# lschoenm/MerKurio

Measured on AMD Instinct MI355X. Metric: Gbases/s scanned (150bp FASTQ, 10k 31-mers); % HBM roofline at 1/2/4/8 GPUs, higher is better.
Workload: dtype u8

## Files before the change

include/merkurio_hip.h:

```cpp
#ifndef MERKURIO_HIP_H
#define MERKURIO_HIP_H

#include <stddef.h>
#include <stdint.h>

#ifdef __cplusplus
extern "C" {
#endif

#define MK_ABI_VERSION 7

#define MK_OK 0
#define MK_E_EMPTY_PATTERN (-1)
#define MK_E_INVALID_Q (-2)
#define MK_E_PATTERN_TOO_LONG (-3)
#define MK_E_NO_PATTERNS (-4)
#define MK_E_NOMEM (-5)
#define MK_E_PAIR_MISMATCH (-6)
#define MK_E_HIP (-7)
#define MK_E_CAPACITY (-8)
#define MK_E_INVALID_ARG (-9)
#define MK_E_UNSUPPORTED (-10)
#define MK_E_RCCL (-11)
#define MK_E_CORRUPT (-12)

#define MK_ALGO_AUTO 0
#define MK_ALGO_AC 1
#define MK_ALGO_BNDMQ 2

#define MK_FLAG_ASCII_CASE_INSENSITIVE 1u

#define MK_MODE_ANY 0
#define MK_MODE_HITS 1

typedef struct mk_matcher mk_matcher;

typedef struct {
    uint64_t rec;
    uint32_t pat;
    uint32_t pos;
} mk_hit;

typedef struct {
    uint64_t rec;
    uint32_t pat;
    uint32_t pos;
    uint32_t file;
    uint32_t _pad;
} mk_row;

typedef struct {
    uint64_t nb_records_tot;
    uint64_t nb_bases;
    uint64_t nb_hits_tot[2];
    uint64_t nb_records_hit[2];
    uint64_t nb_records_extracted;
} mk_counters;

int mk_abi_version(void);
const char *mk_last_error(void);
int mk_device_count(void);

int mk_read_kmers_from_text(const uint8_t *content, size_t len, uint8_t **out_bytes, uint32_t **out_off,
                            uint32_t *out_n);
int mk_parse_pattern_list(const uint8_t *in_bytes, const uint32_t *in_off, uint32_t n_in, int reverse_complement,
                          int canonical, int lowercase, int uppercase, uint8_t **out_bytes, uint32_t **out_off,
                          uint32_t *out_n);
void mk_reverse_complement(const uint8_t *in, size_t n, uint8_t *out);
void mk_canonical(const uint8_t *in, size_t n, uint8_t *out);
int mk_recommend_aho_corasick(size_t num_patterns, size_t max_len);
size_t mk_tune_q_value(size_t pattern_len);
int mk_generate_masks(const uint8_t *pattern, size_t m, uint64_t masks[256], uint64_t *accept);
void mk_free(void *p);

int mk_matcher_create(const uint8_t *pat_bytes, const uint32_t *pat_off, uint32_t n_pat, uint32_t algo, uint32_t q,
                      uint32_t flags, int32_t device, mk_matcher **out);
typedef struct {
    uint32_t struct_size;
    uint32_t force_stride;
    uint32_t force_global_filter;
    uint32_t gbloom_log2_blocks;
    uint32_t tile_run;
    uint32_t gbloom_kib;
    uint32_t length_classes;
    uint32_t force_split_len;
    uint32_t force_stride2;
    uint32_t force_q2;
} mk_matcher_options;
int mk_matcher_create_ex(const uint8_t *pat_bytes, const uint32_t *pat_off, uint32_t n_pat, uint32_t algo, uint32_t q,
                         uint32_t flags, int32_t device, const mk_matcher_options *options, mk_matcher **out);
int mk_plan_geometry(const uint32_t *pat_len, uint32_t n_pat, const mk_matcher_options *options, uint32_t *q_gram, uint32_t *stride,
                     uint32_t *in_lds, uint32_t *split_len, uint32_t *n_short, uint32_t *q_gram2, uint32_t *stride2);
void mk_matcher_destroy(mk_matcher *m);
uint32_t mk_matcher_algo(const mk_matcher *m);
uint32_t mk_matcher_num_patterns(const mk_matcher *m);
int mk_matcher_filter_info(const mk_matcher *m, uint32_t *q_gram, uint32_t *stride, uint64_t *entries,
                           uint64_t *table_bytes);
int mk_matcher_class_info(const mk_matcher *m, uint32_t *split_len, uint32_t *n_short, uint32_t *q_gram2, uint32_t *stride2);
int mk_matcher_filter_mode(const mk_matcher *m, uint32_t *in_lds, uint64_t *filter_bytes);

int mk_scan_batch(mk_matcher *m, const uint8_t *seq_bytes, const uint64_t *seq_off, uint64_t n_rec, uint32_t mode,
                  uint8_t *rec_flags, mk_hit *hits, uint64_t hits_cap, uint64_t *n_hits);

#define MK_NUM_SUMMARY 8
#define MK_SUM_HITS 0
#define MK_SUM_RECORDS_HIT 1
#define MK_SUM_RECORDS 2
#define MK_SUM_BASES 3
#define MK_SUM_CANDIDATES 4

int mk_scan_device(mk_matcher *m, const void *d_seq, uint64_t n_bytes, const void *d_seq_off, uint64_t n_rec,
                   uint32_t mode, void *d_rec_flags, void *d_hits, uint64_t hits_cap, void *d_n_hits,
                   void *d_counters, void *stream);

int mk_matcher_check_device(mk_matcher *m, void *stream);

int mk_matcher_hint_hit_density(mk_matcher *m, uint32_t records_hit_per_1000);

int mk_matcher_set_fixed_record_length(mk_matcher *m, uint32_t record_length);

int mk_matcher_hint_record_lengths(mk_matcher *m, int equal_lengths);

int mk_order_hits(const mk_matcher *m, mk_hit *hits, uint64_t n_hits);
int mk_order_hits_device(mk_matcher *m, void *d_hits, uint64_t n_hits, void *stream);
int mk_matcher_order_info(const mk_matcher *m, uint32_t *path, uint32_t *n_bins, uint32_t *max_bin);
int mk_matcher_order_stats(const mk_matcher *m, uint64_t calls[4]);

const char *mk_matcher_kernel_name(const mk_matcher *m);
int mk_matcher_launch_info(const mk_matcher *m, uint32_t *grid_blocks, uint32_t *block_threads, uint32_t *lds_bytes);
int mk_matcher_enable_timing(mk_matcher *m, uint32_t slots);
int mk_matcher_kernel_times(mk_matcher *m, float *ms, uint32_t cap, uint32_t *n_out);

int mk_extract_single(mk_matcher *m, const uint8_t *seq, const uint64_t *off, uint64_t n_rec, int logging,
                      int invert, uint8_t *keep, mk_row *rows, uint64_t rows_cap, uint64_t *n_rows,
                      mk_counters *counters, uint32_t *pattern_hit_counts);
int mk_extract_paired(mk_matcher *m, const uint8_t *seq1, const uint64_t *off1, uint64_t n_rec1,
                      const uint8_t *seq2, const uint64_t *off2, uint64_t n_rec2, int logging, int invert,
                      uint8_t *keep, mk_row *rows, uint64_t rows_cap, uint64_t *n_rows, mk_counters *counters,
                      uint32_t *pattern_hit_counts);
int mk_tag_records(mk_matcher *m, const uint8_t *seq, const uint64_t *off, uint64_t n_rec, int logging,
                   int filter_matching, int invert, uint8_t *keep, mk_row *rows, uint64_t rows_cap, uint64_t *n_rows,
                   mk_counters *counters, uint32_t *pattern_hit_counts, uint64_t *found_off, uint32_t *found_pat,
                   uint64_t found_cap);
int mk_extract_fastq_text(mk_matcher *m, const uint8_t *text, uint64_t n_text, int logging, int invert, uint64_t rec_cap,
                          uint64_t *n_rec, uint64_t *rec_start, uint8_t *keep, mk_row *rows, uint64_t rows_cap, uint64_t *n_rows,
                          mk_counters *counters, uint32_t *pattern_hit_counts, uint32_t *status);
int mk_upload_text_ahead(mk_matcher *m, const uint8_t *text, uint64_t n_text);
int mk_host_alloc(size_t bytes, void **out);
void mk_host_free(void *p);
int mk_matcher_batch_times(const mk_matcher *m, float ms[4]);

int mk_tag_value(const mk_matcher *m, const uint32_t *found_pat, uint64_t n_found, const char *existing, char *out,
                 size_t cap, size_t *out_len);

int mk_synth_reads_device(mk_matcher *m, uint64_t seed, uint64_t n_rec, uint32_t read_len, uint32_t plant_every,
                          void *d_seq, void *d_seq_off, void *stream);
int mk_synth_reads_host(const mk_matcher *m, uint64_t seed, uint64_t rec0, uint64_t n_rec, uint32_t read_len,
                        uint32_t plant_every, uint8_t *seq, uint64_t *seq_off);
int mk_synth_reads_device_range(mk_matcher *m, uint64_t seed, uint64_t rec0, uint64_t n_rec, uint32_t read_len,
                                uint32_t plant_every, void *d_seq, void *d_seq_off, void *stream);

#define MK_COMM_ID_BYTES 128
int mk_reduce_counters(mk_matcher *const *per_gpu, int n, void *const *d_counters, size_t len, uint64_t *host_sum);
int mk_reduce_prepare(mk_matcher *const *per_gpu, int n);
int mk_comm_available(void);
int mk_comm_unique_id(uint8_t id[MK_COMM_ID_BYTES]);
int mk_comm_init(mk_matcher *m, const uint8_t id[MK_COMM_ID_BYTES], int rank, int n_ranks);
int mk_comm_reduce_counters(mk_matcher *m, void *d_counters, size_t len, void *stream);
int mk_comm_size(const mk_matcher *m, int *n_ranks);
int mk_comm_destroy(mk_matcher *m);

typedef struct mk_codec mk_codec;
typedef struct mk_bgzf_member {
    uint64_t data_off;
    uint64_t out_off;
    uint32_t data_len;
    uint32_t isize;
    uint32_t crc;
    uint32_t reserved;
} mk_bgzf_member;
int mk_codec_create(int device, mk_codec **out);
void mk_codec_destroy(mk_codec *c);
uint64_t mk_bgzf_deflate_bound(uint64_t n, uint32_t block_bytes);
int mk_bgzf_deflate(mk_codec *c, const uint8_t *in, uint64_t n, uint32_t block_bytes, uint8_t *out, uint64_t out_cap, uint64_t *out_len);
int mk_bgzf_deflate_pieces(mk_codec *c, const uint8_t *const *pieces, const uint64_t *sizes, uint64_t n_pieces, uint32_t block_bytes,
                           uint8_t *out, uint64_t out_cap, uint64_t *out_len);
int mk_bgzf_inflate(mk_codec *c, const uint8_t *in, uint64_t n_in, const mk_bgzf_member *members, uint64_t n_members, uint8_t *out,
                    uint64_t out_cap, uint64_t *bad_member);
typedef struct mk_window_text {
    uint8_t *text;
    uint64_t text_cap;
    uint8_t *tail;
    uint64_t tail_cap;
    uint8_t *kept;
    uint64_t kept_cap;
    uint64_t n_text, n_used, n_tail, n_kept_bytes;
} mk_window_text;
int mk_extract_fastq_bgzf(mk_matcher *m, mk_codec *codec, const uint8_t *head, uint64_t n_head, const uint8_t *bgzf, uint64_t n_bgzf,
                          const mk_bgzf_member *members, uint64_t n_members, int last, mk_window_text *io, int logging, int invert,
                          uint64_t rec_cap, uint64_t *n_rec, uint64_t *rec_start, uint8_t *keep, mk_row *rows, uint64_t rows_cap,
                          uint64_t *n_rows, mk_counters *c, uint32_t *pattern_hit_counts, uint32_t *status);
#define MK_TEXT_FASTQ 0
#define MK_TEXT_FASTA 1
typedef struct mk_window_source {
    const uint8_t *head;
    uint64_t n_head;
    const uint8_t *text;
    uint64_t n_text;
    const uint8_t *bgzf;
    uint64_t n_bgzf;
    const mk_bgzf_member *members;
    uint64_t n_members;
    const void *device_text;
    uint64_t n_device_text;
    uint32_t ends_at_record;
    uint32_t reserved;
    uint64_t *rec_start;
    uint8_t *tail;
    uint64_t tail_cap;
    uint8_t *kept;
    uint64_t kept_cap;
    uint8_t *all;
    uint64_t all_cap;
    uint64_t n_window, n_used, n_tail, n_kept_bytes, n_rec_seen;
} mk_window_source;
int mk_extract_window(mk_matcher *m, mk_codec *codec, uint32_t format, uint32_t n_sources, mk_window_source *sources, int logging, int invert,
                      uint64_t rec_cap, uint64_t *n_rec, uint8_t *keep, mk_row *rows, uint64_t rows_cap, uint64_t *n_rows, mk_counters *counters,
                      uint32_t *pattern_hit_counts, uint32_t *status);

int mk_gzip_inflate_device(mk_codec *c, const uint8_t *gz, uint64_t n, uint64_t *text_bytes, uint32_t *taken);
int mk_gzip_text_read(mk_codec *c, uint64_t offset, uint8_t *out, uint64_t len);
const void *mk_gzip_text_device(const mk_codec *c, uint64_t *text_bytes);
int mk_gzip_text_release(mk_codec *c);
int mk_gzip_info(const mk_codec *c, uint32_t *segments, float ms[5]);

typedef struct mk_bam_window {
    const uint8_t *head;
    uint64_t n_head;
    const uint8_t *bgzf;
    uint64_t n_bgzf;
    const mk_bgzf_member *members;
    uint64_t n_members;
    uint32_t last;
    uint32_t filter_matching, invert;
    uint8_t tag[2];
    uint8_t reserved[2];
    uint32_t block_bytes;
    uint8_t *tail;
    uint64_t tail_cap;
    uint8_t *out;
    uint64_t out_cap;
    mk_row *rows;
    uint64_t rows_cap;
    uint64_t *row_name;
    uint8_t *names;
    uint64_t names_cap;
    void (*on_tail)(void *ctx, const uint8_t *tail, uint64_t n_tail);
    void *on_tail_ctx;
    uint64_t n_window, n_used, n_tail, n_rec, n_kept, out_text_bytes, out_len, n_rows, n_names_bytes;
    float ms[8];
} mk_bam_window;
int mk_tag_bam_window(mk_matcher *m, mk_codec *codec, mk_bam_window *w, int logging, mk_counters *counters, uint32_t *pattern_hit_counts,
                      uint32_t *status);
int mk_matcher_set_bam_piece(mk_matcher *m, uint32_t piece_bytes);

typedef struct mk_sam_window {
    const uint8_t *head;
    uint64_t n_head;
    const uint8_t *text;
    uint64_t n_text;
    uint32_t last;
    uint32_t filter_matching, invert;
    uint8_t tag[2];
    uint8_t reserved[2];
    uint8_t *tail;
    uint64_t tail_cap;
    uint8_t *out;
    uint64_t out_cap;
    mk_row *rows;
    uint64_t rows_cap;
    uint64_t *row_name;
    uint8_t *names;
    uint64_t names_cap;
    uint64_t n_window, n_used, n_tail, n_rec, n_kept, out_len, n_rows, n_names_bytes;
    float ms[8];
} mk_sam_window;
int mk_tag_sam_window(mk_matcher *m, mk_sam_window *w, int logging, mk_counters *counters, uint32_t *pattern_hit_counts, uint32_t *status);

typedef struct mk_sam_bam_window {
    const uint8_t *head;
    uint64_t n_head;
    const uint8_t *text;
    uint64_t n_text;
    uint32_t last;
    uint32_t filter_matching, invert;
    uint8_t tag[2];
    uint8_t reserved[2];
    const uint8_t *ref_names;
    const uint64_t *ref_off;
    uint64_t n_refs;
    uint32_t block_bytes;
    uint32_t reserved2;
    uint8_t *tail;
    uint64_t tail_cap;
    uint8_t *out;
    uint64_t out_cap;
    mk_row *rows;
    uint64_t rows_cap;
    uint64_t *row_name;
    uint8_t *names;
    uint64_t names_cap;
    uint64_t n_window, n_used, n_tail, n_rec, n_kept, out_text_bytes, out_len, n_rows, n_names_bytes;
    float ms[8];
} mk_sam_bam_window;
int mk_tag_sam_bam_window(mk_matcher *m, mk_codec *codec, mk_sam_bam_window *w, int logging, mk_counters *counters, uint32_t *pattern_hit_counts,
                          uint32_t *status);

typedef struct mk_bam_sam_window {
    const uint8_t *head;
    uint64_t n_head;
    const uint8_t *bgzf;
    uint64_t n_bgzf;
    const mk_bgzf_member *members;
    uint64_t n_members;
    uint32_t last;
    uint32_t filter_matching, invert;
    uint8_t tag[2];
    uint8_t reserved[2];
    const uint8_t *ref_names;
    const uint64_t *ref_off;
    uint64_t n_refs;
    uint8_t *tail;
    uint64_t tail_cap;
    uint8_t *out;
    uint64_t out_cap;
    mk_row *rows;
    uint64_t rows_cap;
    uint64_t *row_name;
    uint8_t *names;
    uint64_t names_cap;
    void (*on_tail)(void *ctx, const uint8_t *tail, uint64_t n_tail);
    void *on_tail_ctx;
    uint64_t n_window, n_used, n_tail, n_rec, n_kept, out_len, n_rows, n_names_bytes;
    float ms[8];
} mk_bam_sam_window;
int mk_tag_bam_sam_window(mk_matcher *m, mk_codec *codec, mk_bam_sam_window *w, int logging, mk_counters *counters, uint32_t *pattern_hit_counts,
                          uint32_t *status);

int mk_bgzf_members(const uint8_t *in, uint64_t n, mk_bgzf_member *members, uint64_t cap, uint64_t *n_members, uint64_t *consumed,
                    uint64_t *text_bytes);
const uint8_t *mk_bgzf_eof(void);
int mk_codec_set_pass_limits(mk_codec *c, uint64_t deflate_members, uint64_t inflate_text_bytes);
int mk_codec_set_inflate_kernel(mk_codec *c, int which);
int mk_codec_set_gzip_chunk(mk_codec *c, uint64_t chunk_bytes);
int mk_codec_times(const mk_codec *c, float ms[3]);

#ifdef __cplusplus
}
#endif
#endif
```

merkurio_amd/build.py:

```python
import os
import subprocess
import sys
from concurrent.futures import ThreadPoolExecutor

HERE = os.path.dirname(os.path.abspath(__file__))
CSRC = os.path.join(HERE, "csrc")
LIB_DIR = os.path.join(HERE, "lib")
LIB_PATH = os.path.join(LIB_DIR, "libmerkurio_hip.so")
CLI_PATH = os.path.join(LIB_DIR, "merkurio")

N_VARIANT_TUS = 17
HOST_SOURCES = ["matcher.cpp", "host_patterns.cpp", "host_loops.cpp", "reduce.cpp"]
HIPCC = os.environ.get("HIPCC", "/opt/rocm/bin/hipcc")
FLAGS = ["--offload-arch=gfx950", "-O3", "-std=c++17", "-fPIC", "-Wall", "-Wno-unused-result"]
FLAGS += os.environ.get("MERKURIO_HIPCC_FLAGS", "").split()
JOBS = int(os.environ.get("MERKURIO_BUILD_JOBS", str(min(8, os.cpu_count() or 1))))


def _stale(target, deps):
    if not os.path.exists(target):
        return True
    t = os.path.getmtime(target)
    return any(os.path.getmtime(d) > t for d in deps)


def _headers():
    hs = [os.path.join(CSRC, f) for f in os.listdir(CSRC) if f.endswith((".h", ".hpp"))]
    hs += [os.path.join(CSRC, "codec", f) for f in os.listdir(os.path.join(CSRC, "codec")) if f.endswith((".h", ".hpp"))]
    hs.append(os.path.join(os.path.dirname(HERE), "include", "merkurio_hip.h"))
    return hs


def _units():
    units = [("scan_tu%d.o" % n, "scan_variants.hip", ["-DMK_TU=%d" % n]) for n in range(N_VARIANT_TUS)]
    units.append(("scan_kernel.o", "scan_kernel.hip", []))
    units.append(("order_hits.o", "order_hits.hip", []))
    units.append(("order_hits_fallback.o", "order_hits_fallback.hip", []))
    units.append(("sets.o", "sets.hip", []))
    units.append(("build_tables.o", "build_tables.hip", []))
    units.append(("ingest.o", "ingest.hip", []))
    units.append(("bam.o", "bam.hip", []))
    units.append(("sam.o", "sam.hip", []))
    units.append(("codec_bgzf_deflate.o", "codec/bgzf_deflate.hip", []))
    units.append(("codec_bgzf_inflate.o", "codec/bgzf_inflate.hip", []))
    units.append(("codec_bgzf_inflate_wave.o", "codec/bgzf_inflate_wave.hip", []))
    units.append(("codec_gzip_inflate.o", "codec/gzip_inflate.hip", []))
    units.append(("codec_gzip_segments_wave.o", "codec/gzip_segments_wave.hip", []))
    units.append(("codec_host.o", "codec/codec_host.cpp", []))
    units += [(s.replace(".cpp", ".o"), s, []) for s in HOST_SOURCES if os.path.exists(os.path.join(CSRC, s))]
    return units


def _deps():
    srcs = [os.path.join(CSRC, f) for f in os.listdir(CSRC) if os.path.isfile(os.path.join(CSRC, f))]
    srcs += [os.path.join(CSRC, "codec", f) for f in os.listdir(os.path.join(CSRC, "codec"))]
    return srcs + _headers()


def _parse_resource_remarks(stderr):
    import re
    rows, cur, rest = [], None, []
    for line in stderr.splitlines():
        if "[-Rpass-analysis=kernel-resource-usage]" not in line:
            rest.append(line)
            continue
        m = re.search(r"remark:\s+(.*?)\s*\[-Rpass", line)
        if not m:
            continue
        k, _, v = m.group(1).partition(":")
        k, v = k.strip(), v.strip()
        if k == "Function Name":
            cur = {"name": v}
            rows.append(cur)
        elif cur is not None:
            cur[k] = v
    out = []
    for r in rows:
        name = r["name"]
        for tool in ("c++filt", "/opt/rocm/lib/llvm/bin/llvm-cxxfilt"):
            try:
                name = subprocess.run([tool, name], capture_output=True, text=True).stdout.strip() or name
                break
            except OSError:
                continue
        out.append((name, r.get("VGPRs", "?"), r.get("AGPRs", "?"), r.get("TotalSGPRs", r.get("SGPRs", "?")),
                    r.get("ScratchSize [bytes/lane]", "?"), r.get("LDS Size [bytes/block]", "?"), r.get("Occupancy [waves/SIMD]", "?")))
    return out, "\n".join(rest) + ("\n" if rest else "")


def isa_resources(obj_dir, out_file, strict=True):
    rows = []
    for f in sorted(os.listdir(obj_dir)):
        if f.endswith(".isa.txt"):
            with open(os.path.join(obj_dir, f)) as fh:
                rows += [line.rstrip("\n").split("\t") for line in fh if line.strip()]
    if not rows:
        return None
    rows.sort(key=lambda r: r[0])
    with open(out_file, "w") as f:
        f.write("# kernel\tVGPRs\tAGPRs\tSGPRs\tscratch bytes/lane\tLDS bytes/block (static)\twaves/SIMD\n")
        for r in rows:
            f.write("\t".join(r) + "\n")
    spilled = [r[0] for r in rows if r[4] not in ("0", "?") and "rocprim" not in r[0]]
    if spilled and strict:
        raise RuntimeError("kernels with scratch memory (register spills): " + "; ".join(spilled))
    if spilled:
        print("note: kernels with scratch memory in this tagged build: " + "; ".join(spilled), file=sys.stderr)
    return out_file


def _compile_lib(out_path, extra_flags, obj_dir, force, verbose):
    os.makedirs(obj_dir, exist_ok=True)
    headers = _headers()
    jobs = []
    objs = []
    for obj, src, fl in _units():
        o = os.path.join(obj_dir, obj)
        s = os.path.join(CSRC, src)
        objs.append(o)
        if force or _stale(o, [s] + headers):
            jobs.append([HIPCC, *FLAGS, *extra_flags, *fl, "-c", "-o", o, s])

    def run(cmd):
        if verbose:
            print(" ".join(cmd), flush=True)
        if cmd[-1].endswith(".hip") and "-c" in cmd:
            r = subprocess.run(cmd + ["-Rpass-analysis=kernel-resource-usage"], stderr=subprocess.PIPE, text=True)
            obj = cmd[cmd.index("-o") + 1]
            rows, rest = _parse_resource_remarks(r.stderr)
            if rest.strip():
                sys.stderr.write(rest)
            if r.returncode:
                raise subprocess.CalledProcessError(r.returncode, cmd)
            with open(obj + ".isa.txt", "w") as f:
                for row in rows:
                    f.write("\t".join(str(x) for x in row) + "\n")
            return
        subprocess.run(cmd, check=True)

    if jobs:
        with ThreadPoolExecutor(max(1, JOBS)) as ex:
            list(ex.map(run, jobs))
    for f in os.listdir(obj_dir):
        if (f.endswith(".o") or f.endswith(".isa.txt")) and os.path.join(obj_dir, f.replace(".isa.txt", "")) not in objs:
            os.remove(os.path.join(obj_dir, f))
    isa_resources(obj_dir, os.path.join(os.path.dirname(out_path), "isa_resources" + os.path.basename(out_path)[len("libmerkurio_hip"):-3] + ".txt"),
                  strict=not extra_flags)
    if jobs or force or _stale(out_path, objs):
        tmp = out_path + ".tmp.%d" % os.getpid()
        run([HIPCC, "--offload-arch=gfx950", "-shared", "-o", tmp, *objs, "-ldl", "-lpthread"])
        os.replace(tmp, out_path)
    return out_path


def build_lib(force=False, verbose=False):
    import fcntl
    os.makedirs(LIB_DIR, exist_ok=True)
    if not force and not _stale(LIB_PATH, _deps()):
        return LIB_PATH
    with open(os.path.join(LIB_DIR, ".build.lock"), "w") as lock:
        fcntl.flock(lock, fcntl.LOCK_EX)
        if force or _stale(LIB_PATH, _deps()):
            _compile_lib(LIB_PATH, [], os.path.join(LIB_DIR, "obj"), force, verbose)
    return LIB_PATH


def build_tagged(tag, flags, force=False, verbose=False, only_scan=True):
    out = os.path.join(LIB_DIR, "libmerkurio_hip_%s.so" % tag)
    return _compile_lib(out, list(flags), os.path.join(LIB_DIR, "obj_" + tag), force, verbose)


def build_cli(force=False, verbose=False):
    srcs = [os.path.join(CSRC, "cli", f) for f in sorted(os.listdir(os.path.join(CSRC, "cli")))
            if f.endswith(".cpp")] if os.path.isdir(os.path.join(CSRC, "cli")) else []
    if not srcs:
        return None
    deps = srcs + [os.path.join(CSRC, "cli", f) for f in os.listdir(os.path.join(CSRC, "cli"))] + [LIB_PATH]
    if not force and not _stale(CLI_PATH, deps):
        return CLI_PATH
    obj_dir = os.path.join(LIB_DIR, "obj_cli")
    os.makedirs(obj_dir, exist_ok=True)
    cli_hdrs = [os.path.join(CSRC, "cli", f) for f in os.listdir(os.path.join(CSRC, "cli")) if f.endswith(".hpp")] + _headers()
    jobs, objs = [], []
    for s in srcs:
        o = os.path.join(obj_dir, os.path.basename(s).replace(".cpp", ".o"))
        objs.append(o)
        if force or _stale(o, [s] + cli_hdrs):
            jobs.append([HIPCC, "--offload-arch=gfx950", "-O2", "-std=c++17", "-Wall", "-Wno-unused-result", "-c", "-o", o, s])

    def run(cmd):
        if verbose:
            print(" ".join(cmd), flush=True)
        subprocess.run(cmd, check=True)

    with ThreadPoolExecutor(max(1, JOBS)) as ex:
        list(ex.map(run, jobs))
    run([HIPCC, "-o", CLI_PATH, *objs, "-L" + LIB_DIR, "-lmerkurio_hip", "-lz", "-ldl", "-lpthread", "-Wl,-rpath,$ORIGIN"])
    return CLI_PATH


def build_all(force=False, verbose=False):
    lib = build_lib(force, verbose)
    cli = build_cli(force, verbose)
    return lib, cli


if __name__ == "__main__":
    if "--tag" in sys.argv:
        tag = sys.argv[sys.argv.index("--tag") + 1]
        fl = sys.argv[sys.argv.index("--flags") + 1].split() if "--flags" in sys.argv else []
        print(build_tagged(tag, fl, force="--force" in sys.argv, verbose=True))
    else:
        print(build_all(force="--force" in sys.argv, verbose=True))
```

merkurio_amd/csrc/matcher.cpp:

```cpp
#include <hip/hip_runtime.h>

#include <algorithm>
#include <chrono>
#include <cmath>
#include <cstdarg>
#include <cstdio>
#include <cstdlib>
#include <cstring>
#include <memory>
#include <string>
#include <vector>

#include "host_common.h"
#include "matcher_internal.h"
#include "scan_kernel.h"

namespace mk {

thread_local char g_last_error[512] = "";

int fail(int code, const char *fmt, ...) {
    va_list ap;
    va_start(ap, fmt);
    vsnprintf(g_last_error, sizeof(g_last_error), fmt, ap);
    va_end(ap);
    return code;
}

int hip_fail(hipError_t e, const char *what) {
    (void)hipGetLastError();
    return fail(e == hipErrorOutOfMemory ? MK_E_NOMEM : MK_E_HIP, "%s failed: %s", what, hipGetErrorString(e));
}

#define MK_HIP(call)                                       \
    do {                                                   \
        hipError_t e_ = (call);                            \
        if (e_ != hipSuccess) return hip_fail(e_, #call);  \
    } while (0)

constexpr uint64_t kMaxLdsEntries = 98304;
constexpr double kMCandPerLaunch = 15000.0;
static double bloom_fp(double entries) {
    const double lo = 1.0 - exp(-entries / (kBloomBlocks * 32.0)), hi = 1.0 - exp(-2.0 * entries / (kBloomBlocks * 32.0));
    return lo * hi * hi;
}
static double hashed_cost(uint64_t n, uint32_t S, uint32_t q, double per_mcand) {
    const double per_base = std::min(1.0 / S, (double)n / pow(4.0, (double)std::min(q, 30u))) + bloom_fp((double)n * S) / S;
    return 0.42 * (16.0 / S) + kMCandPerLaunch * per_mcand * per_base;
}
static void choose_geometry(uint32_t lmin, uint64_t n_pat, const mk_matcher_options &opt, uint32_t *q, uint32_t *S,
                            uint32_t *gblocks) {
    const int forced = (int)opt.force_stride;
    const bool force_global = opt.force_global_filter != 0;
    *gblocks = 0;
    if (n_pat <= kMaxLdsEntries && !force_global) {
        *q = std::min<uint32_t>(32, lmin);
        *S = 1;
        double best = 1e300;
        for (uint32_t s : {16u, 8u, 4u, 2u, 1u}) {
            if (s > lmin) continue;
            const uint32_t qq = std::min<uint32_t>(32, lmin - s + 1);
            if (forced) {
                if ((int)s != forced) continue;
                *q = qq;
                *S = s;
                return;
            }
            if (s > 1 && n_pat * s > kMaxLdsEntries) continue;
            if (s > 1 && qq < 16 && (double)n_pat * s > 2.0 * pow(4.0, (double)qq)) continue;
            const double c = hashed_cost(n_pat, s, qq, 0.0152);
            if (c < best) {
                best = c;
                *q = qq;
                *S = s;
            }
        }
        return;
    }
    *q = std::min<uint32_t>(32, lmin);
    *S = 1;
    bool chosen = false;
    for (uint32_t s : {16u, 8u, 4u, 2u}) {
        if (s > lmin) continue;
        const uint32_t qq = std::min<uint32_t>(32, lmin - s + 1);
        if (forced ? (int)s != forced : (qq < 14 || n_pat * s > (8ull << 19))) continue;
        *q = qq;
        *S = s;
        chosen = true;
        break;
    }
    if (!chosen && !forced)
        for (uint32_t s : {16u, 8u, 4u, 2u}) {
            if (s > lmin) continue;
            const uint32_t qq = std::min<uint32_t>(32, lmin - s + 1);
            if (qq < 16 || n_pat * s * 4 > (1ull << 25)) continue;
            *q = qq;
            *S = s;
            break;
        }
    uint64_t blocks = std::min<uint64_t>(std::max<uint64_t>(n_pat * *S / 8, 1ull << 17), 3ull << 17);
    if (opt.gbloom_log2_blocks) blocks = 1ull << opt.gbloom_log2_blocks;
    if (opt.gbloom_kib) blocks = (uint64_t)opt.gbloom_kib * 128;
    *gblocks = (uint32_t)blocks;
}

struct ClassPlan {
    uint32_t split = 0;
    uint32_t S2 = 0, q2 = 0;
    uint32_t lmin_main = 0;
    uint64_t n_main = 0, n_short = 0;
    double cost = 0;
};
static double main_cost(uint32_t lmin, uint64_t n, const mk_matcher_options &opt, bool two_class) {
    uint32_t q, S, gb;
    choose_geometry(lmin, n, opt, &q, &S, &gb);
    return hashed_cost(n, S, q, two_class ? 0.025 : 0.0152);
}
static double short_cost(uint32_t S2, uint32_t q2, uint64_t n) {
    const double per_sample = std::min(1.0, (double)n * S2 / pow(4.0, (double)q2));
    return (q2 <= kShortByteMaxQ ? 0.075 : 0.15) * (16.0 / S2) + kMCandPerLaunch * 0.025 * per_sample / S2;
}
static ClassPlan plan_classes(std::vector<uint32_t> lens, const mk_matcher_options &opt) {
    ClassPlan best;
    const uint64_t n = lens.size();
    const auto mm = std::minmax_element(lens.begin(), lens.end());
    best.n_main = n;
    best.lmin_main = *mm.first;
    if (opt.length_classes == 1 || *mm.first == *mm.second) return best;
    if (opt.force_global_filter || n > kMaxLdsEntries) {
        constexpr uint32_t kGfMinLen = 15;
        if (*mm.first >= kGfMinLen || *mm.second < kGfMinLen || (opt.force_stride && opt.length_classes != 2 && !opt.force_split_len)) return best;
        uint32_t split = 0xFFFFFFFFu;
        uint64_t n_short = 0;
        for (uint32_t l : lens) {
            if (l < kGfMinLen)
                ++n_short;
            else
                split = std::min(split, l);
        }
        if (opt.force_split_len) {
            split = opt.force_split_len;
            n_short = 0;
            for (uint32_t l : lens) n_short += l < split;
            if (n_short == 0 || n_short == n) return best;
        }
        uint32_t q, S, gb;
        choose_geometry(split, n - n_short, opt, &q, &S, &gb);
        if (S < 2) return best;
        for (uint32_t s2 : {8u, 4u, 2u, 1u}) {
            if (s2 > *mm.first || (opt.force_stride2 && s2 != opt.force_stride2)) continue;
            const uint32_t qmax = std::min<uint32_t>(kShortMaxQ, *mm.first - s2 + 1);
            for (uint32_t q2 : {qmax, std::min(qmax, kShortByteMaxQ)}) {
                if (opt.force_q2 && q2 != std::min<uint32_t>(opt.force_q2, qmax)) continue;
                const double c = short_cost(s2, q2, n_short);
                if (best.split == 0 || c < best.cost) {
                    best.split = split;
                    best.S2 = s2;
                    best.q2 = q2;
                    best.lmin_main = split;
                    best.n_main = n - n_short;
                    best.n_short = n_short;
                    best.cost = c;
                }
            }
        }
        return best;
    }
    std::sort(lens.begin(), lens.end());
    if (opt.force_stride && opt.length_classes != 2 && !opt.force_split_len) return best;
    best.cost = main_cost(lens[0], n, opt, false);
    const double single = best.cost;
    for (uint64_t i = 1; i < n; ++i) {
        if (lens[i] == lens[i - 1]) continue;
        const uint32_t split = lens[i];
        if (opt.force_split_len && split != opt.force_split_len) continue;
        if (lens[0] > 64 && !opt.force_split_len) break;
        {
            uint32_t q, S, gb;
            choose_geometry(split, n - i, opt, &q, &S, &gb);
            if (S < 2) continue;
        }
        const double mc = main_cost(split, n - i, opt, true);
        for (uint32_t s2 : {8u, 4u, 2u, 1u}) {
            if (s2 > lens[0] || (opt.force_stride2 && s2 != opt.force_stride2)) continue;
            const uint32_t qmax = std::min<uint32_t>(kShortMaxQ, lens[0] - s2 + 1);
            for (uint32_t q2 : {qmax, std::min(qmax, kShortByteMaxQ)}) {
                if (opt.force_q2 && q2 != std::min<uint32_t>(opt.force_q2, qmax)) continue;
                if (!opt.force_stride2 && !opt.force_q2 && s2 > 1 && (double)i * s2 > 2.0 * pow(4.0, (double)q2)) continue;
                const double c = mc + short_cost(s2, q2, i);
                const bool forced = opt.length_classes == 2 || opt.force_split_len;
                if ((best.split == 0 && (forced || c < 0.9 * single)) || (best.split != 0 && c < best.cost)) {
                    best.split = split;
                    best.S2 = s2;
                    best.q2 = q2;
                    best.lmin_main = split;
                    best.n_main = n - i;
                    best.n_short = i;
                    best.cost = c;
                }
            }
        }
    }
    return best;
}

}

using namespace mk;

thread_local double mk::g_free_ms = 0;
thread_local double mk::g_alloc_ms = 0;

int mk::ensure_device(void **p, size_t *cap, size_t need) {
    if (need <= *cap) return MK_OK;
    const auto t0 = std::chrono::steady_clock::now();
    auto ms_since = [](std::chrono::steady_clock::time_point a) { return std::chrono::duration<double, std::milli>(std::chrono::steady_clock::now() - a).count(); };
    double free_ms = 0;
    if (*p) {
        (void)hipFree(*p);
        free_ms = ms_since(t0);
        g_free_ms += free_ms;
    }
    *p = nullptr;
    *cap = 0;
    size_t want = need + (need < (64u << 20) ? need / 4 : need / 16) + 4096;
    hipError_t e = hipMalloc(p, want);
    g_alloc_ms += ms_since(t0);
#ifdef MK_ALLOC_LOG
    fprintf(stderr, "[alloc] %8.1f MiB: hipFree %7.2f ms, hipMalloc %7.2f ms\n", want / 1048576.0, free_ms, ms_since(t0) - free_ms);
#endif
    if (e != hipSuccess) return hip_fail(e, "hipMalloc");
    *cap = want;
    return MK_OK;
}

static int ensure(void **p, size_t *cap, size_t need) { return ensure_device(p, cap, need); }

static int read_options(const mk_matcher_options *options, mk_matcher_options *out) {
    mk_matcher_options opt;
    memset(&opt, 0, sizeof(opt));
    if (options) {
        if (options->struct_size < sizeof(uint32_t) || options->struct_size > 4096)
            return fail(MK_E_INVALID_ARG, "mk_matcher_options.struct_size %u is not plausible", options->struct_size);
        memcpy(&opt, options, std::min<size_t>(options->struct_size, sizeof(opt)));
        const uint32_t fs = opt.force_stride;
        if (fs != 0 && fs != 1 && fs != 2 && fs != 4 && fs != 8 && fs != 16)
            return fail(MK_E_INVALID_ARG, "force_stride %u: must be 0, 1, 2, 4, 8 or 16", fs);
        if (opt.gbloom_log2_blocks != 0 && (opt.gbloom_log2_blocks < 10 || opt.gbloom_log2_blocks > 25))
            return fail(MK_E_INVALID_ARG, "gbloom_log2_blocks %u out of range (10..25)", opt.gbloom_log2_blocks);
        if (opt.tile_run > 8) return fail(MK_E_INVALID_ARG, "tile_run %u out of range (0..8)", opt.tile_run);
        if (opt.gbloom_kib > (1u << 18)) return fail(MK_E_INVALID_ARG, "gbloom_kib %u out of range (<= 256 MiB)", opt.gbloom_kib);
        if (opt.length_classes > 2) return fail(MK_E_INVALID_ARG, "length_classes %u: must be 0 (rule), 1 or 2", opt.length_classes);
        const uint32_t f2 = opt.force_stride2;
        if (f2 != 0 && f2 != 1 && f2 != 2 && f2 != 4 && f2 != 8)
            return fail(MK_E_INVALID_ARG, "force_stride2 %u: must be 0, 1, 2, 4 or 8", f2);
        if (opt.force_q2 > kShortMaxQ) return fail(MK_E_INVALID_ARG, "force_q2 %u: must be 0..%u", opt.force_q2, kShortMaxQ);
    }
    *out = opt;
    return MK_OK;
}

extern "C" {

int mk_abi_version(void) { return MK_ABI_VERSION; }
const char *mk_last_error(void) { return g_last_error; }

int mk_device_count(void) {
    int n = 0;
    if (hipGetDeviceCount(&n) != hipSuccess) return 0;
    return n;
}

void mk_free(void *p) { free(p); }

int mk_plan_geometry(const uint32_t *pat_len, uint32_t n_pat, const mk_matcher_options *options, uint32_t *q_gram, uint32_t *stride,
                     uint32_t *in_lds, uint32_t *split_len, uint32_t *n_short, uint32_t *q_gram2, uint32_t *stride2) {
    if (!pat_len || n_pat == 0) return fail(MK_E_NO_PATTERNS, "No k-mers found in file or provided sequence.");
    mk_matcher_options opt;
    int rc = read_options(options, &opt);
    if (rc) return rc;
    MK_ABI_BEGIN
    std::vector<uint32_t> lens(pat_len, pat_len + n_pat);
    if (*std::min_element(lens.begin(), lens.end()) == 0) return fail(MK_E_EMPTY_PATTERN, "Pattern is empty.");
    const ClassPlan plan = plan_classes(std::move(lens), opt);
    uint32_t q = 0, S = 1, gb = 0;
    choose_geometry(plan.lmin_main, plan.n_main, opt, &q, &S, &gb);
    if (q_gram) *q_gram = q;
    if (stride) *stride = S;
    if (in_lds) *in_lds = gb ? 0 : 1;
    if (split_len) *split_len = plan.split;
    if (n_short) *n_short = (uint32_t)plan.n_short;
    if (q_gram2) *q_gram2 = plan.q2;
    if (stride2) *stride2 = plan.S2;
    return MK_OK;
    MK_ABI_END
}

int mk_matcher_create(const uint8_t *pat_bytes, const uint32_t *pat_off, uint32_t n_pat, uint32_t algo, uint32_t q,
                      uint32_t flags, int32_t device, mk_matcher **out) {
    return mk_matcher_create_ex(pat_bytes, pat_off, n_pat, algo, q, flags, device, nullptr, out);
}

int mk_matcher_create_ex(const uint8_t *pat_bytes, const uint32_t *pat_off, uint32_t n_pat, uint32_t algo, uint32_t q,
                         uint32_t flags, int32_t device, const mk_matcher_options *options, mk_matcher **out) {
    if (!out) return fail(MK_E_INVALID_ARG, "out is null");
    *out = nullptr;
    mk_matcher_options opt;
    int rc_opt = read_options(options, &opt);
    if (rc_opt) return rc_opt;
    MK_ABI_BEGIN
    if (n_pat == 0 || !pat_off || !pat_bytes) return fail(MK_E_NO_PATTERNS, "No k-mers found in file or provided sequence.");
    if (algo > MK_ALGO_BNDMQ) return fail(MK_E_INVALID_ARG, "unknown algo %u", algo);
    if (n_pat > kMaxPatterns) return fail(MK_E_UNSUPPORTED, "too many patterns (%u)", n_pat);
    const bool ci = flags & MK_FLAG_ASCII_CASE_INSENSITIVE;
    uint32_t lmin = 0xFFFFFFFFu, lmax = 0;
    for (uint32_t i = 0; i < n_pat; ++i) {
        if (pat_off[i + 1] < pat_off[i]) return fail(MK_E_INVALID_ARG, "pattern offsets not monotone");
        uint32_t len = pat_off[i + 1] - pat_off[i];
        lmin = std::min(lmin, len);
        lmax = std::max(lmax, len);
    }
    uint32_t use = algo;
    if (ci)
        use = MK_ALGO_AC;
    else if (algo == MK_ALGO_AUTO)
        use = (q == 0 && mk_recommend_aho_corasick(n_pat, lmax)) ? MK_ALGO_AC : MK_ALGO_BNDMQ;
    if (use == MK_ALGO_BNDMQ) {
        for (uint32_t i = 0; i < n_pat; ++i) {
            size_t len = pat_off[i + 1] - pat_off[i];
            size_t qq = q ? q : mk_tune_q_value(len);
            if (!q && len >= 65) return fail(MK_E_PATTERN_TOO_LONG, "Pattern length is too long for BNDMq.");
            if (len == 0) return fail(MK_E_EMPTY_PATTERN, "Pattern is empty.");
            if (qq == 0 || qq > len)
                return fail(MK_E_INVALID_Q, "Invalid q-gram length: %zu. Must be between 1 and pattern length.", qq);
            if (len > 64)
                return fail(MK_E_PATTERN_TOO_LONG,
                            "Pattern length %zu is too large for this architecture when using BNDM (max 64).", len);
        }
    } else if (lmin == 0) {
        return fail(MK_E_EMPTY_PATTERN, "Pattern is empty.");
    }

    int ndev = 0;
    if (hipGetDeviceCount(&ndev) != hipSuccess || ndev <= 0)
        return fail(MK_E_HIP, "no HIP device available: the MI355X scan path has no CPU fallback");
    if (device < 0 || device >= ndev) return fail(MK_E_INVALID_ARG, "device %d out of range (%d devices)", device, ndev);
    MK_HIP(hipSetDevice(device));

    struct Deleter {
        void operator()(mk_matcher *p) const { mk_matcher_destroy(p); }
    };
    std::unique_ptr<mk_matcher, Deleter> owner(new mk_matcher());
    mk_matcher *m = owner.get();
    m->device = device;
    m->algo = use;
    m->flags = flags;
    m->n_pat = n_pat;
    m->pat_bytes.assign(pat_bytes, pat_bytes + pat_off[n_pat]);
    m->pat_off.assign(pat_off, pat_off + n_pat + 1);
    hipDeviceProp_t prop;
    if (hipGetDeviceProperties(&prop, device) == hipSuccess && prop.multiProcessorCount > 0)
        m->num_cus = prop.multiProcessorCount;

    m->uniform_len = (lmin == lmax) ? lmin : 0;
    m->tile_run = opt.tile_run;
    ClassPlan plan;
    {
        std::vector<uint32_t> lens(n_pat);
        for (uint32_t i = 0; i < n_pat; ++i) lens[i] = pat_off[i + 1] - pat_off[i];
        plan = plan_classes(std::move(lens), opt);
    }
    if ((opt.length_classes == 2 || opt.force_split_len) && !plan.split)
        return fail(MK_E_INVALID_ARG, "the pattern set cannot be split into two length classes as the options ask "
                                      "(split length %u, stride %u, shortest pattern %u, longest %u)",
                    opt.force_split_len, opt.force_stride2, lmin, lmax);
    m->split_len = plan.split;
    m->S2 = plan.S2;
    m->q2 = plan.q2;
    m->n_short = (uint32_t)plan.n_short;
    choose_geometry(plan.lmin_main, plan.n_main, opt, &m->q, &m->S, &m->gbloom_blocks);
    if (opt.force_stride && m->S != opt.force_stride)
        return fail(MK_E_INVALID_ARG, "force_stride %u is longer than the shortest pattern (%u)", opt.force_stride, plan.lmin_main);
    const uint32_t q_f = m->q, S = m->S;
    m->entries = plan.n_main * S + plan.n_short * plan.S2;
    uint64_t slots = 64;
    while (slots < (m->gbloom_blocks ? 4 : 2) * m->entries) slots <<= 1;
    if (slots > (1ull << 27) && m->gbloom_blocks) {
        slots = 64;
        while (slots < 2 * m->entries) slots <<= 1;
    }
    if (slots > (1ull << 27))
        return fail(MK_E_UNSUPPORTED, "pattern set too large (%llu table entries)", (unsigned long long)m->entries);
    m->table_slots = (uint32_t)slots;
    const bool two = plan.split != 0;
    const bool gf_ctx = m->gbloom_blocks != 0 && gf_has_ctx(S, q_f) && !two;
    const size_t bloom_words = m->gbloom_blocks ? (size_t)m->gbloom_blocks * 2 : (size_t)kBloomWords;
    MK_HIP(hipStreamCreateWithFlags(&m->stream, hipStreamNonBlocking));
    MK_HIP(hipMalloc((void **)&m->d_bloom, bloom_words * sizeof(uint32_t)));
    MK_HIP(hipMalloc((void **)&m->d_table, slots * sizeof(TableEntry)));
    MK_HIP(hipMalloc((void **)&m->d_pat_bytes, m->pat_bytes.size() + 16));
    MK_HIP(hipMalloc((void **)&m->d_pat_off, (n_pat + 1) * sizeof(uint32_t)));
    MK_HIP(hipMalloc((void **)&m->d_nhits, sizeof(unsigned long long)));
    MK_HIP(hipMalloc((void **)&m->d_error, 16));
    MK_HIP(hipMemset(m->d_error, 0, 16));
    MK_HIP(hipMalloc((void **)&m->d_stage, (size_t)m->num_cus * (kBlockThreads / 64) * kHitStage * sizeof(mk_hit)));
    MK_HIP(hipMalloc((void **)&m->d_flag_list, (size_t)m->num_cus * (kBlockThreads / 64) * kFlagListCap * sizeof(uint32_t)));
    MK_HIP(hipMalloc((void **)&m->d_flag_counts, (size_t)m->num_cus * (kBlockThreads / 64) * sizeof(uint32_t)));
    MK_HIP(hipMemcpy(m->d_pat_bytes, m->pat_bytes.data(), m->pat_bytes.size(), hipMemcpyHostToDevice));
    MK_HIP(hipMemsetAsync(m->d_pat_bytes + m->pat_bytes.size(), 0, 16, m->stream));
    MK_HIP(hipMemcpy(m->d_pat_off, m->pat_off.data(), (n_pat + 1) * sizeof(uint32_t), hipMemcpyHostToDevice));
    MK_HIP(hipMemsetAsync(m->d_bloom, 0, bloom_words * sizeof(uint32_t), m->stream));
    if (two) {
        MK_HIP(hipMalloc((void **)&m->d_short_table, kShortBitmapWords * sizeof(uint32_t)));
        MK_HIP(hipMemsetAsync(m->d_short_table, 0, kShortBitmapWords * sizeof(uint32_t), m->stream));
    }
    {
        BuildParams B;
        memset(&B, 0, sizeof(B));
        B.pat_bytes = m->d_pat_bytes;
        B.pat_off = m->d_pat_off;
        B.n_pat = n_pat;
        B.S = S;
        B.q = q_f;
        B.split = plan.split;
        B.S2 = plan.S2;
        B.q2 = plan.q2;
        B.gbloom_blocks = m->gbloom_blocks;
        B.gf_ctx = gf_ctx ? 1 : 0;
        B.bloom = m->d_bloom;
        B.table = m->d_table;
        B.bucket_mask = m->table_slots / kBucketEntries - 1;
        B.short_table = m->d_short_table;
        launch_build_tables(B, slots, m->stream);
        MK_HIP(hipGetLastError());
        MK_HIP(hipStreamSynchronize(m->stream));
    }
    if (use == MK_ALGO_AC && !m->uniform_len) {
        std::vector<uint32_t> unrank(n_pat), rank(n_pat);
        if (lmax <= (1u << 20)) {
            std::vector<uint32_t> start((size_t)lmax + 2, 0);
            for (uint32_t i = 0; i < n_pat; ++i) start[lmax - (pat_off[i + 1] - pat_off[i]) + 1]++;
            for (uint32_t l = 0; l <= lmax; ++l) start[l + 1] += start[l];
            for (uint32_t i = 0; i < n_pat; ++i) unrank[start[lmax - (pat_off[i + 1] - pat_off[i])]++] = i;
        } else {
            for (uint32_t i = 0; i < n_pat; ++i) unrank[i] = i;
            std::stable_sort(unrank.begin(), unrank.end(), [pat_off](uint32_t a, uint32_t b) {
                return pat_off[a + 1] - pat_off[a] > pat_off[b + 1] - pat_off[b];
            });
        }
        for (uint32_t r = 0; r < n_pat; ++r) rank[unrank[r]] = r;
        MK_HIP(hipMalloc((void **)&m->d_pat_rank, n_pat * sizeof(uint32_t)));
        MK_HIP(hipMalloc((void **)&m->d_pat_unrank, n_pat * sizeof(uint32_t)));
        MK_HIP(hipMemcpy(m->d_pat_rank, rank.data(), n_pat * sizeof(uint32_t), hipMemcpyHostToDevice));
        MK_HIP(hipMemcpy(m->d_pat_unrank, unrank.data(), n_pat * sizeof(uint32_t), hipMemcpyHostToDevice));
    }
    *out = owner.release();
    return MK_OK;
    MK_ABI_END
}

void mk_matcher_destroy(mk_matcher *m) {
    if (!m) return;
    (void)hipSetDevice(m->device);
    if (m->comm) (void)mk_comm_destroy(m);
    if (m->stream) (void)hipStreamDestroy(m->stream);
    if (m->stream_ahead) {
        (void)hipStreamSynchronize(m->stream_ahead);
        (void)hipStreamDestroy(m->stream_ahead);
        for (auto &a : m->ahead)
            if (a.ev) (void)hipEventDestroy(a.ev);
    }
    for (auto e : m->ev_start) (void)hipEventDestroy(e);
    for (auto e : m->ev_stop) (void)hipEventDestroy(e);
    for (void *p : {(void *)m->d_bloom, (void *)m->d_table, (void *)m->d_pat_bytes, (void *)m->d_pat_off,
                    (void *)m->d_seq, (void *)m->d_off, (void *)m->d_flags, (void *)m->d_hits, (void *)m->d_nhits,
                    (void *)m->d_stage, (void *)m->d_rec_index, (void *)m->d_flag_list, (void *)m->d_flag_counts, m->d_sort_tmp,
                    (void *)m->d_pat_rank, (void *)m->d_pat_unrank, (void *)m->d_error, m->d_aux, m->d_pair, (void *)m->d_short_table, m->d_refs, m->txt[0].d_text, m->txt[0].d_ing_a, m->txt[0].d_ing_b, m->txt[1].d_text, m->txt[1].d_ing_a, m->txt[1].d_ing_b, m->txt[0].d_fa_seq, m->txt[1].d_fa_seq, (void *)m->d_flags2, m->ahead[0].d, m->ahead[1].d, m->ahead[2].d, m->ahead[3].d})
        if (p) (void)hipFree(p);
    delete m;
}

uint32_t mk_matcher_algo(const mk_matcher *m) { return m ? m->algo : 0; }
uint32_t mk_matcher_num_patterns(const mk_matcher *m) { return m ? m->n_pat : 0; }
const char *mk_matcher_kernel_name(const mk_matcher *m) { return m ? m->kernel_name : ""; }

int mk_matcher_filter_info(const mk_matcher *m, uint32_t *q_gram, uint32_t *stride, uint64_t *entries,
                           uint64_t *table_bytes) {
    if (!m) return fail(MK_E_INVALID_ARG, "null matcher");
    if (q_gram) *q_gram = m->q;
    if (stride) *stride = m->S;
    if (entries) *entries = m->entries;
    if (table_bytes) *table_bytes = (uint64_t)m->table_slots * sizeof(TableEntry);
    return MK_OK;
}

int mk_matcher_class_info(const mk_matcher *m, uint32_t *split_len, uint32_t *n_short, uint32_t *q_gram2, uint32_t *stride2) {
    if (!m) return fail(MK_E_INVALID_ARG, "null matcher");
    if (split_len) *split_len = m->split_len;
    if (n_short) *n_short = m->n_short;
    if (q_gram2) *q_gram2 = m->q2;
    if (stride2) *stride2 = m->S2;
    return MK_OK;
}

int mk_matcher_filter_mode(const mk_matcher *m, uint32_t *in_lds, uint64_t *filter_bytes) {
    if (!m) return fail(MK_E_INVALID_ARG, "null matcher");
    if (in_lds) *in_lds = m->gbloom_blocks ? 0 : 1;
    if (filter_bytes) *filter_bytes = m->gbloom_blocks ? (uint64_t)m->gbloom_blocks * 8 : (uint64_t)kBloomBytes;
    return MK_OK;
}

int mk_scan_device(mk_matcher *m, const void *d_seq, uint64_t n_bytes, const void *d_seq_off, uint64_t n_rec,
                   uint32_t mode, void *d_rec_flags, void *d_hits, uint64_t hits_cap, void *d_n_hits,
                   void *d_counters, void *stream) {
    if (!m) return fail(MK_E_INVALID_ARG, "null matcher");
    if (mode > MK_MODE_HITS) return fail(MK_E_INVALID_ARG, "unknown mode %u", mode);
    if (((uintptr_t)d_seq & 15) != 0) return fail(MK_E_INVALID_ARG, "d_seq must be 16-byte aligned");
    if (((uintptr_t)d_rec_flags & 3) != 0) return fail(MK_E_INVALID_ARG, "d_rec_flags must be 4-byte aligned");
    const uint32_t rec_len = m->batch_rec_len ? m->batch_rec_len : m->fixed_rec_len;
    if (rec_len && n_bytes != n_rec * (uint64_t)rec_len)
        return fail(MK_E_INVALID_ARG, "fixed record length %u: %llu records are not %llu bytes", rec_len, (unsigned long long)n_rec,
                    (unsigned long long)n_bytes);
    if (!d_n_hits || !d_rec_flags || (!d_seq_off && n_rec && !rec_len)) return fail(MK_E_INVALID_ARG, "null device buffer");
    if (mode == MK_MODE_HITS && !d_hits && hits_cap) return fail(MK_E_INVALID_ARG, "d_hits is null");
    hipStream_t st = (hipStream_t)stream;
    MK_HIP(hipSetDevice(m->device));
    launch_clear((uint32_t *)d_rec_flags, (n_rec + 3) / 4, (unsigned long long *)d_n_hits, st);
    MK_HIP(hipGetLastError());
    if (mode == MK_MODE_HITS) MK_HIP(hipMemsetAsync(m->d_error, 0, sizeof(uint32_t), st));
    m->last_n_rec = n_rec;
    if (n_rec == 0 || n_bytes == 0) return MK_OK;
    ScanParams p;
    memset(&p, 0, sizeof(p));
    p.seq = (const uint8_t *)d_seq;
    p.n_bytes = n_bytes;
    p.rec_off = (const uint64_t *)d_seq_off;
    p.n_rec = n_rec;
    const uint64_t tile_bytes = (uint64_t)kTileChunks * kChunkBytes;
    const uint64_t n_tiles = (n_bytes + tile_bytes - 1) / tile_bytes;
    p.bloom = m->d_bloom;
    p.gbloom_blocks = m->gbloom_blocks;
    p.table = m->d_table;
    p.table_mask = m->table_slots / kBucketEntries - 1;
    p.pat_bytes = m->d_pat_bytes;
    p.pat_off = m->d_pat_off;
    p.n_pat = m->n_pat;
    p.q = m->q;
    const uint64_t kmask = m->q >= 32 ? ~0ull : ((1ull << (2 * m->q)) - 1);
    p.key_mask_lo = (uint32_t)kmask;
    p.key_mask_hi = (uint32_t)(kmask >> 32);
    p.case_insensitive = (m->flags & MK_FLAG_ASCII_CASE_INSENSITIVE) ? 1 : 0;
    p.s2 = m->split_len ? m->S2 : 0;
    p.s2_log2 = m->S2 >= 8 ? 3 : m->S2 >= 4 ? 2 : m->S2 >= 2 ? 1 : 0;
    p.key2_mask = (1u << (2 * m->q2)) - 1u;
    p.short_bytes = m->q2 <= kShortByteMaxQ;
    p.short_bitmap = m->d_short_table;
    p.uniform_len = m->uniform_len;
    p.rec_flags32 = (uint32_t *)d_rec_flags;
    p.hits = (mk_hit *)d_hits;
    p.hits_cap = (mode == MK_MODE_HITS) ? hits_cap : 0;
    p.n_hits = (unsigned long long *)d_n_hits;
    p.counters = (unsigned long long *)d_counters;
    p.error_word = m->d_error;
    const uint64_t waves_per_block = kBlockThreads / 64;
    uint64_t blocks = (n_tiles + waves_per_block - 1) / waves_per_block;
    if (blocks > (uint64_t)m->num_cus) blocks = m->num_cus;
    p.stage = m->d_stage;
    p.rec_per_byte = (double)n_rec / (double)n_bytes;
    const uint64_t tiles_per_wave = n_tiles / (blocks * waves_per_block);
    p.tile_run = m->tile_run ? m->tile_run : tiles_per_wave >= 16 ? 4 : tiles_per_wave >= 8 ? 2 : 1;
    p.rec_index = nullptr;
    p.rec_len = rec_len;
    p.inv_rec_len = rec_len ? 1.0 / (double)rec_len : 0.0;
    if (m->ragged && !rec_len && n_rec < (1ull << 32)) {
        int rc_i = ensure((void **)&m->d_rec_index, &m->d_rec_index_cap, ((n_bytes >> kRecIndexShift) + 2) * sizeof(uint32_t));
        if (rc_i) return rc_i;
        launch_rec_index(p.rec_off, n_rec, n_bytes, m->d_rec_index, st);
        p.rec_index = m->d_rec_index;
    }
    const size_t slots = m->ev_start.size();
    const size_t slot = slots ? (size_t)(m->timed_launches % slots) : 0;
    if (slots) MK_HIP(hipEventRecord(m->ev_start[slot], st));
    const uint32_t kDensePerMille = mode == MK_MODE_HITS ? 95 : 145;
    const bool plain_loads = m->hit_density_pm >= kDensePerMille && !m->split_len;
    const int flavour = plain_loads ? 0 : 1;
    const bool listed = !(plain_loads && m->gbloom_blocks == 0) && mode != MK_MODE_HITS && n_rec < (1ull << 32);
    p.flag_list = listed ? m->d_flag_list : nullptr;
    p.flag_counts = m->d_flag_counts;
    p.flag_cap = kFlagListCap;
    const char *name = launch_scan(p, (int)m->S, m->q > 16, mode == MK_MODE_HITS, m->gbloom_blocks != 0, flavour, (int)blocks, st);
    if (!name) return fail(MK_E_UNSUPPORTED, "no kernel for stride %u", m->S);
    if (slots) {
        MK_HIP(hipEventRecord(m->ev_stop[slot], st));
        m->timed_launches++;
    }
    if (listed)
        launch_flag_scatter(m->d_flag_list, m->d_flag_counts, kFlagListCap, (uint32_t)(blocks * waves_per_block), (uint8_t *)d_rec_flags, st);
    if (d_counters) {
        launch_count_flags(p, st);
        if (mode == MK_MODE_HITS && p.hits && p.hits_cap) launch_hist_hits(p, m->num_cus, st);
    }
    m->kernel_name = name;
    m->last_grid = (int)blocks;
    MK_HIP(hipGetLastError());
    return MK_OK;
}

static int take_device_errors(mk_matcher *m, hipStream_t st) {
    uint32_t w = 0;
    MK_HIP(hipMemcpyAsync(&w, m->d_error, sizeof(w), hipMemcpyDeviceToHost, st));
    MK_HIP(hipStreamSynchronize(st));
    if (!w) return MK_OK;
    MK_HIP(hipMemsetAsync(m->d_error, 0, sizeof(w), st));
    return fail(MK_E_UNSUPPORTED, "an occurrence lies 4 GiB or more into its record: a single record must be shorter than 4 GiB "
                                  "(mk_hit.pos is 32 bits); the tuples of that scan are not usable");
}

int mk_matcher_check_device(mk_matcher *m, void *stream) {
    if (!m) return fail(MK_E_INVALID_ARG, "null matcher");
    MK_HIP(hipSetDevice(m->device));
    return take_device_errors(m, (hipStream_t)stream);
}

int mk_matcher_hint_hit_density(mk_matcher *m, uint32_t records_hit_per_1000) {
    if (!m) return fail(MK_E_INVALID_ARG, "null matcher");
    m->hit_density_pm = records_hit_per_1000 > 1000 ? 1000 : records_hit_per_1000;
    return MK_OK;
}

int mk_matcher_set_fixed_record_length(mk_matcher *m, uint32_t record_length) {
    if (!m) return fail(MK_E_INVALID_ARG, "null matcher");
    m->fixed_rec_len = record_length;
    return MK_OK;
}

int mk_matcher_hint_record_lengths(mk_matcher *m, int equal_lengths) {
    if (!m) return fail(MK_E_INVALID_ARG, "null matcher");
    m->ragged = !equal_lengths;
    return MK_OK;
}

int mk_matcher_enable_timing(mk_matcher *m, uint32_t slots) {
    if (!m) return fail(MK_E_INVALID_ARG, "null matcher");
    MK_ABI_BEGIN
    MK_HIP(hipSetDevice(m->device));
    for (auto e : m->ev_start) (void)hipEventDestroy(e);
    for (auto e : m->ev_stop) (void)hipEventDestroy(e);
    m->ev_start.assign(slots, nullptr);
    m->ev_stop.assign(slots, nullptr);
    m->timed_launches = 0;
    for (uint32_t i = 0; i < slots; ++i) {
        MK_HIP(hipEventCreate(&m->ev_start[i]));
        MK_HIP(hipEventCreate(&m->ev_stop[i]));
    }
    return MK_OK;
    MK_ABI_END
}

int mk_matcher_kernel_times(mk_matcher *m, float *ms, uint32_t cap, uint32_t *n_out) {
    if (!m || !n_out) return fail(MK_E_INVALID_ARG, "null argument");
    const uint64_t slots = m->ev_start.size();
    const uint64_t n = std::min<uint64_t>(m->timed_launches, slots);
    *n_out = (uint32_t)n;
    if (n > cap) return fail(MK_E_CAPACITY, "need room for %llu timings", (unsigned long long)n);
    MK_HIP(hipSetDevice(m->device));
    const uint64_t first = m->timed_launches - n;
    for (uint64_t i = 0; i < n; ++i) {
        const size_t slot = (size_t)((first + i) % slots);
        MK_HIP(hipEventSynchronize(m->ev_stop[slot]));
        MK_HIP(hipEventElapsedTime(&ms[i], m->ev_start[slot], m->ev_stop[slot]));
    }
    m->timed_launches = 0;
    return MK_OK;
}

int mk_matcher_launch_info(const mk_matcher *m, uint32_t *grid_blocks, uint32_t *block_threads, uint32_t *lds_bytes) {
    if (!m) return fail(MK_E_INVALID_ARG, "null matcher");
    if (grid_blocks) *grid_blocks = (uint32_t)m->last_grid;
    if (block_threads) *block_threads = kBlockThreads;
    if (lds_bytes) *lds_bytes = scan_lds_bytes();
    return MK_OK;
}

static uint32_t bits_of(uint64_t v) { return v ? 64u - (uint32_t)__builtin_clzll(v) : 0u; }

static int order_library(mk_matcher *m, mk_hit *d_hits, uint64_t n, bool ac, hipStream_t st) {
    size_t need = 0;
    MK_HIP(order_hits_library(d_hits, n, ac, m->d_pat_off, m->uniform_len, nullptr, &need, st));
    int rc = ensure(&m->d_sort_tmp, &m->d_sort_tmp_cap, need ? need : 16);
    if (rc) return rc;
    MK_HIP(order_hits_library(d_hits, n, ac, m->d_pat_off, m->uniform_len, m->d_sort_tmp, &need, st));
    m->order_path = 3;
    return MK_OK;
}

int mk_order_hits_device(mk_matcher *m, void *d_hits, uint64_t n_hits, void *stream) {
    if (!m) return fail(MK_E_INVALID_ARG, "null matcher");
    return mk::order_hits_on_device(m, d_hits, n_hits, m->algo == MK_ALGO_AC, m->last_n_rec, stream);
}

}

static int order_hits_on_device_impl(mk_matcher *m, void *d_hits, uint64_t n_hits, bool ac_order, uint64_t rec_bound, void *stream);
int mk::order_hits_on_device(mk_matcher *m, void *d_hits, uint64_t n_hits, bool ac_order, uint64_t rec_bound, void *stream) {
    const int rc = order_hits_on_device_impl(m, d_hits, n_hits, ac_order, rec_bound, stream);
    if (rc == MK_OK) ++m->order_path_calls[m->order_path & 3];
    return rc;
}
static int order_hits_on_device_impl(mk_matcher *m, void *d_hits, uint64_t n_hits, bool ac_order, uint64_t rec_bound, void *stream) {
    using namespace mk;
    m->order_path = 0;
    if (n_hits < 2) return MK_OK;
    if (!d_hits) return fail(MK_E_INVALID_ARG, "null buffer");
    if (((uintptr_t)d_hits & 15) != 0) return fail(MK_E_INVALID_ARG, "d_hits must be 16-byte aligned");
    MK_ABI_BEGIN
    MK_HIP(hipSetDevice(m->device));
    hipStream_t st = (hipStream_t)stream;
    mk_hit *hits = (mk_hit *)d_hits;
    const uint64_t n = n_hits;
    if (n >= (1ull << 32)) return order_library(m, hits, n, ac_order, st);
    if (!m->order_prepared) {
        MK_HIP(order_kernels_prepare());
        m->order_prepared = true;
    }
    uint32_t log_bins = 0;
    while (log_bins < 15 && ((uint64_t)2048 << log_bins) < n) ++log_bins;
    const size_t head = 64 + (size_t)(4 * kOrderMaxBins + 16) * sizeof(uint32_t);
    int rc = ensure(&m->d_sort_tmp, &m->d_sort_tmp_cap, head + n * sizeof(uint64_t));
    if (rc) return rc;
    OrderScratch S;
    S.stats = (unsigned long long *)m->d_sort_tmp;
    S.g_cnt = (uint32_t *)((char *)m->d_sort_tmp + 64);
    S.bin_start = S.g_cnt + kOrderMaxBins;
    S.cursor = S.bin_start + kOrderMaxBins + 8;
    S.big_list = S.cursor + kOrderMaxBins;
    S.keys = (uint64_t *)((char *)m->d_sort_tmp + head);
    OrderKey L;
    memset(&L, 0, sizeof(L));
    L.pat_off = m->d_pat_off;
    L.uniform_len = m->uniform_len;
    L.rank = ac_order ? m->d_pat_rank : nullptr;
    L.unrank = ac_order ? m->d_pat_unrank : nullptr;
    L.ac = ac_order ? 1 : 0;
    if (!rec_bound) rec_bound = 1ull << 32;
    unsigned long long stats[6] = {0, 0, 0, 0, 0, 0};
    uint32_t s = 0;
    for (int attempt = 0; attempt < 2; ++attempt) {
        s = bits_of(rec_bound - 1) > log_bins ? bits_of(rec_bound - 1) - log_bins : 0;
        L.bits_a = 0;
        L.bits_b = 1;
        L.b_hi = 0;
        L.b_lo = 63;
        L.shift = s;
        L.n_bins = 1u << log_bins;
        MK_HIP(hipMemsetAsync(m->d_sort_tmp, 0, 64 + (size_t)L.n_bins * sizeof(uint32_t), st));
        launch_order_hist(hits, n, L, S, m->num_cus, st);
        MK_HIP(hipGetLastError());
        MK_HIP(hipMemcpyAsync(stats, S.stats, sizeof(stats), hipMemcpyDeviceToHost, st));
        uint32_t err_word = 0;
        MK_HIP(hipMemcpyAsync(&err_word, m->d_error, sizeof(err_word), hipMemcpyDeviceToHost, st));
        MK_HIP(hipStreamSynchronize(st));
        if (err_word) return take_device_errors(m, st);
        const bool beyond = (stats[0] >> s) >= L.n_bins;
        const bool loose = stats[3] > kOrderLeafMax && bits_of(stats[0]) < bits_of(rec_bound - 1);
        if (!beyond && !loose) break;
        rec_bound = stats[0] + 1;
    }
    uint32_t bits_rec = bits_of(stats[0]);
    const uint32_t bits_a = std::max(1u, bits_of(stats[1])), bits_b = std::max(1u, bits_of(stats[2]));
    if (bits_rec + bits_a + bits_b > 64) return order_library(m, hits, n, ac_order, st);
    if (s + bits_a > 63) return order_library(m, hits, n, ac_order, st);
    L.bits_a = bits_a;
    L.bits_b = bits_b;
    L.b_hi = 0;
    L.b_lo = bits_b;
    m->order_path = 1;
    if (stats[3] > kOrderLeafMax || (stats[0] >> s) >= L.n_bins) {
        L.rec_base = ~stats[4];
        bits_rec = bits_of(stats[0] - L.rec_base);
        const uint32_t total = bits_rec + bits_a + bits_b;
        const uint32_t lb = std::min(15u, std::max(log_bins + 3, total > 14 ? total - 14 : 0u));
        const uint32_t drop = total > lb ? total - lb : 0;
        if (drop >= bits_b) {
            L.b_hi = 0;
            L.b_lo = bits_b;
            L.shift = drop - bits_b;
        } else {
            L.b_hi = bits_b - drop;
            L.b_lo = drop;
            L.shift = 0;
        }
        L.n_bins = 1u << std::min(lb, total);
        MK_HIP(hipMemsetAsync(m->d_sort_tmp, 0, 64 + (size_t)L.n_bins * sizeof(uint32_t), st));
        launch_order_hist(hits, n, L, S, m->num_cus, st);
        MK_HIP(hipGetLastError());
        MK_HIP(hipMemcpyAsync(stats, S.stats, sizeof(stats), hipMemcpyDeviceToHost, st));
        MK_HIP(hipStreamSynchronize(st));
        if (stats[3] > kOrderLeafMax) return order_library(m, hits, n, ac_order, st);
        m->order_path = 2;
    } else {
        L.shift = s + bits_a;
    }
    m->order_bins = L.n_bins;
    m->order_max_bin = (uint32_t)stats[3];
    launch_order_scatter_leaf(hits, n, L, S, (uint32_t)stats[3], (uint32_t)stats[5], m->num_cus, st);
    MK_HIP(hipGetLastError());
    return MK_OK;
    MK_ABI_END
}

extern "C" {

int mk_matcher_order_stats(const mk_matcher *m, uint64_t calls[4]) {
    if (!m || !calls) return fail(MK_E_INVALID_ARG, "null argument");
    for (int i = 0; i < 4; ++i) calls[i] = m->order_path_calls[i];
    return MK_OK;
}

int mk_matcher_order_info(const mk_matcher *m, uint32_t *path, uint32_t *n_bins, uint32_t *max_bin) {
    if (!m) return fail(MK_E_INVALID_ARG, "null matcher");
    if (path) *path = m->order_path;
    if (n_bins) *n_bins = m->order_bins;
    if (max_bin) *max_bin = m->order_max_bin;
    return MK_OK;
}

int mk_order_hits(const mk_matcher *m, mk_hit *hits, uint64_t n_hits) {
    if (!m) return fail(MK_E_INVALID_ARG, "null matcher");
    if (m->algo == MK_ALGO_AC) {
        const uint32_t *off = m->pat_off.data();
        std::sort(hits, hits + n_hits, [off](const mk_hit &a, const mk_hit &b) {
            if (a.rec != b.rec) return a.rec < b.rec;
            uint64_t ea = (uint64_t)a.pos + (off[a.pat + 1] - off[a.pat]);
            uint64_t eb = (uint64_t)b.pos + (off[b.pat + 1] - off[b.pat]);
            if (ea != eb) return ea < eb;
            if (a.pos != b.pos) return a.pos < b.pos;
            return a.pat < b.pat;
        });
    } else {
        std::sort(hits, hits + n_hits, [](const mk_hit &a, const mk_hit &b) {
            if (a.rec != b.rec) return a.rec < b.rec;
            if (a.pat != b.pat) return a.pat < b.pat;
            return a.pos < b.pos;
        });
    }
    return MK_OK;
}

}

namespace mk {

int batch_check(const uint8_t *seq_bytes, const uint64_t *seq_off, uint64_t n_rec, uint64_t *n_bytes) {
    if (!seq_off) return fail(MK_E_INVALID_ARG, "null buffer");
    *n_bytes = seq_off[n_rec] - seq_off[0];
    if (*n_bytes && !seq_bytes) return fail(MK_E_INVALID_ARG, "null sequence buffer");
    if (*n_bytes >= (1ull << 32))
        for (uint64_t i = 0; i < n_rec; ++i)
            if (seq_off[i + 1] - seq_off[i] >= (1ull << 32))
                return fail(MK_E_UNSUPPORTED, "record %llu is %llu bytes long: a single record must be shorter than 4 GiB",
                            (unsigned long long)i, (unsigned long long)(seq_off[i + 1] - seq_off[i]));
    return MK_OK;
}

int batch_upload(mk_matcher *m, const uint8_t *seq_bytes, const uint64_t *seq_off, uint64_t n_rec, uint64_t n_bytes, uint32_t *batch_len) {
    MK_HIP(hipSetDevice(m->device));
    int rc;
    if ((rc = ensure((void **)&m->d_seq, &m->d_seq_cap, n_bytes + 64))) return rc;
    if ((rc = ensure((void **)&m->d_off, &m->d_off_cap, (n_rec + 1) * sizeof(uint64_t)))) return rc;
    if ((rc = ensure((void **)&m->d_flags, &m->d_flags_cap, n_rec + 8))) return rc;
    const uint64_t base = seq_off[0];
    const uint64_t len0 = seq_off[1] - seq_off[0];
    bool equal = true;
    for (uint64_t i = 1; i < n_rec && equal; ++i) equal = seq_off[i + 1] - seq_off[i] == len0;
    m->ragged = !equal;
    *batch_len = (equal && len0 > 0 && len0 < (1ull << 32)) ? (uint32_t)len0 : 0;
    std::vector<uint64_t> rel;
    const uint64_t *off_src = seq_off;
    if (base != 0) {
        rel.resize(n_rec + 1);
        for (uint64_t i = 0; i <= n_rec; ++i) rel[i] = seq_off[i] - base;
        off_src = rel.data();
    }
    if (n_bytes) MK_HIP(hipMemcpyAsync(m->d_seq, seq_bytes + base, n_bytes, hipMemcpyHostToDevice, m->stream));
    MK_HIP(hipMemcpyAsync(m->d_off, off_src, (n_rec + 1) * sizeof(uint64_t), hipMemcpyHostToDevice, m->stream));
    if (!rel.empty()) MK_HIP(hipStreamSynchronize(m->stream));
    return MK_OK;
}

int batch_scan(mk_matcher *m, uint64_t n_bytes, uint64_t n_rec, uint32_t mode, uint32_t batch_len, uint64_t cap, uint64_t limit,
               unsigned long long *found) {
    struct BatchLen {
        mk_matcher *m;
        uint32_t saved;
        ~BatchLen() {
            m->batch_rec_len = 0;
            m->fixed_rec_len = saved;
        }
    } guard{m, m->fixed_rec_len};
    m->fixed_rec_len = 0;
// ... 105 lines not shown
```

merkurio_amd/csrc/matcher_internal.h:

```cpp
#pragma once
#include <hip/hip_runtime.h>

#include <mutex>
#include <vector>

#include "filter.hpp"
#include "scan_kernel.h"
#include "host_common.h"

struct mk_matcher {
    int device = 0;
    int num_cus = 256;
    uint32_t algo = MK_ALGO_AC;
    uint32_t flags = 0;
    uint32_t n_pat = 0;
    std::vector<uint8_t> pat_bytes;
    std::vector<uint32_t> pat_off;
    uint32_t uniform_len = 0;
    uint32_t q = 0, S = 1;
    uint32_t split_len = 0, S2 = 0, q2 = 0, n_short = 0;
    uint32_t *d_short_table = nullptr;
    uint64_t entries = 0;
    uint32_t table_slots = 0;
    uint32_t *d_bloom = nullptr;
    uint32_t gbloom_blocks = 0;
    uint32_t tile_run = 0;
    uint32_t hit_density_pm = 0;
    bool ragged = false;
    uint32_t fixed_rec_len = 0, batch_rec_len = 0;
    uint32_t *d_rec_index = nullptr;
    size_t d_rec_index_cap = 0;
    mk::TableEntry *d_table = nullptr;
    uint8_t *d_pat_bytes = nullptr;
    uint32_t *d_pat_off = nullptr;
    hipStream_t stream = nullptr;
    uint8_t *d_seq = nullptr;
    size_t d_seq_cap = 0;
    uint64_t *d_off = nullptr;
    size_t d_off_cap = 0;
    uint8_t *d_flags = nullptr;
    size_t d_flags_cap = 0;
    mk_hit *d_hits = nullptr;
    size_t d_hits_cap = 0;
    unsigned long long *d_nhits = nullptr;
    uint32_t *d_error = nullptr;
    mk_hit *d_stage = nullptr;
    uint32_t *d_flag_list = nullptr;
    uint32_t *d_flag_counts = nullptr;
    void *d_sort_tmp = nullptr;
    size_t d_sort_tmp_cap = 0;
    uint32_t *d_pat_rank = nullptr;
    uint32_t *d_pat_unrank = nullptr;
    uint64_t last_n_rec = 0;
    uint32_t order_path = 0, order_bins = 0, order_max_bin = 0;
    uint64_t order_path_calls[4] = {0, 0, 0, 0};
    bool order_prepared = false;
    void *d_aux = nullptr;
    size_t d_aux_cap = 0;
    void *d_pair = nullptr;
    size_t d_pair_cap = 0;
    struct TextSlot {
        void *d_text = nullptr, *d_ing_a = nullptr, *d_ing_b = nullptr, *d_fa_seq = nullptr;
        size_t d_text_cap = 0, d_ing_a_cap = 0, d_ing_b_cap = 0, d_fa_seq_cap = 0;
    } txt[2];
    uint32_t bam_piece = 0;
    uint8_t *d_flags2 = nullptr;
    size_t d_flags2_cap = 0;
    void *d_refs = nullptr;
    size_t d_refs_cap = 0;
    std::vector<uint8_t> refs_names;
    std::vector<uint64_t> refs_off;
    uint32_t refs_slots = 0;
    bool refs_valid = false;
    struct AheadSlot {
        void *d = nullptr;
        size_t cap = 0;
        hipEvent_t ev = nullptr;
        const uint8_t *text = nullptr;
        uint64_t n = 0;
    } ahead[4];
    hipStream_t stream_ahead = nullptr;
    std::mutex ahead_mu;
    float batch_ms[4] = {0, 0, 0, 0};
    const char *kernel_name = "";
    int last_grid = 0;
    std::vector<hipEvent_t> ev_start, ev_stop;
    uint64_t timed_launches = 0;
    void *comm = nullptr;
    int comm_rank = 0, comm_size = 0;
};

namespace mk {
int ensure_device(void **p, size_t *cap, size_t need);
extern thread_local double g_alloc_ms, g_free_ms;
int batch_check(const uint8_t *seq_bytes, const uint64_t *seq_off, uint64_t n_rec, uint64_t *n_bytes);
int batch_upload(mk_matcher *m, const uint8_t *seq_bytes, const uint64_t *seq_off, uint64_t n_rec, uint64_t n_bytes, uint32_t *batch_len);
int batch_scan(mk_matcher *m, uint64_t n_bytes, uint64_t n_rec, uint32_t mode, uint32_t batch_len, uint64_t cap, uint64_t limit,
               unsigned long long *found);
int batch_flags(mk_matcher *m, uint64_t n_rec, uint8_t *rec_flags, uint64_t *flagged_out);
int order_hits_on_device(mk_matcher *m, void *d_hits, uint64_t n_hits, bool ac_order, uint64_t rec_bound, void *stream);
int hip_fail(hipError_t e, const char *what);
}
```

merkurio_amd/csrc/scan_kernel.h:

```cpp
#pragma once
#include <hip/hip_runtime.h>
#include <stdint.h>

#include "../../include/merkurio_hip.h"
#include "filter.hpp"

namespace mk {

constexpr uint32_t kHitStage = 1024;
constexpr uint32_t kFlagListCap = 2048;

struct ScanParams {
    const uint8_t *seq;
    uint64_t n_bytes;
    const uint64_t *rec_off;
    uint64_t n_rec;
    const uint32_t *bloom;
    uint32_t gbloom_blocks;
    const TableEntry *table;
    uint32_t table_mask;
    const uint8_t *pat_bytes;
    const uint32_t *pat_off;
    uint32_t n_pat;
    uint32_t q;
    uint32_t key_mask_lo;
    uint32_t key_mask_hi;
    uint32_t s2;
    uint32_t s2_log2;
    uint32_t key2_mask;
    uint32_t short_bytes;
    const uint32_t *short_bitmap;
    uint32_t case_insensitive;
    uint32_t uniform_len;
    double rec_per_byte;
    uint32_t tile_run;
    const uint32_t *rec_index;
    uint32_t rec_len;
    double inv_rec_len;
    mk_hit *stage;
    uint32_t *rec_flags32;
    uint32_t *flag_list;
    uint32_t *flag_counts;
    uint32_t flag_cap;
    mk_hit *hits;
    uint64_t hits_cap;
    unsigned long long *n_hits;
    unsigned long long *counters;
    uint32_t *error_word;
};

const char *launch_scan(const ScanParams &p, int S, bool wide, bool emit, bool global_filter, int flavour, int grid_blocks,
                        hipStream_t stream);

template <int S, int QC, bool EMIT, bool GF, int FL, int MC = 0>
void launch_variant(const ScanParams &p, int grid_blocks, hipStream_t stream);

uint32_t scan_lds_bytes();

void launch_hist_hits(const ScanParams &p, int grid_blocks, hipStream_t stream);

constexpr uint32_t kRecIndexShift = 16;
void launch_clear(uint32_t *flags32, uint64_t n_words, unsigned long long *n_hits, hipStream_t stream);
void launch_flag_scatter(const uint32_t *flag_list, const uint32_t *flag_counts, uint32_t flag_cap, uint32_t n_waves, uint8_t *rec_flags,
                         hipStream_t stream);
void launch_rec_index(const uint64_t *rec_off, uint64_t n_rec, uint64_t n_bytes, uint32_t *rec_index, hipStream_t stream);
struct OrderKey {
    const uint32_t *pat_off;
    uint32_t uniform_len;
    const uint32_t *rank;
    const uint32_t *unrank;
    uint64_t rec_base;
    uint32_t ac;
    uint32_t bits_a;
    uint32_t bits_b;
    uint32_t b_hi;
    uint32_t b_lo;
    uint32_t shift;
    uint32_t n_bins;
};
struct OrderScratch {
    unsigned long long *stats;
    uint32_t *g_cnt;
    uint32_t *bin_start;
    uint32_t *cursor;
    uint32_t *big_list;
    uint64_t *keys;
};
constexpr uint32_t kOrderMaxBins = 32768;
constexpr uint32_t kOrderLeafMax = 16384;
constexpr uint32_t kOrderLeafSmall = 4096;
void launch_order_hist(const mk_hit *d_hits, uint64_t n, const OrderKey &L, const OrderScratch &S, int num_cus, hipStream_t st);
void launch_order_scatter_leaf(mk_hit *d_hits, uint64_t n, const OrderKey &L, const OrderScratch &S, uint32_t max_bin, uint32_t n_big,
                               int num_cus, hipStream_t st);
hipError_t order_kernels_prepare();
hipError_t order_hits_library(mk_hit *d_hits, size_t n, bool ac, const uint32_t *d_pat_off, uint32_t uniform_len, void *tmp,
                              size_t *tmp_bytes, hipStream_t stream);

void launch_pattern_sets(const mk_hit *d_hits, uint64_t n, uint64_t n_rec, uint32_t *d_found_pat, unsigned long long *d_found_off,
                         unsigned long long *d_total, void *d_tile, hipStream_t st);
void launch_count_u32(const uint32_t *d_list, uint64_t n, uint32_t *d_counts, uint32_t n_bins, hipStream_t st);
void launch_rows(const mk_hit *d_hits, uint64_t n, uint32_t file, mk_row *d_rows, hipStream_t st);
void launch_pair_mark(mk_hit *d_hits, uint64_t n, uint32_t mate, bool ac, hipStream_t st);
void launch_rows_pair(const mk_hit *d_hits, uint64_t n, bool ac, mk_row *d_rows, hipStream_t st);
void launch_count_pair_heads(const mk_hit *d_hits, uint64_t n, uint32_t *d_counts, uint32_t n_bins, hipStream_t st);

void launch_ingest_count(const uint8_t *d_text, uint64_t n, uint32_t *d_block_cnt, uint32_t *d_total, hipStream_t st);
void launch_ingest_records(const uint8_t *d_text, uint64_t n, const uint32_t *d_block_off, const uint32_t *d_total, uint32_t *d_line_start,
                           uint64_t n_rec, uint32_t *d_rec_start, uint32_t *d_seq_start, uint32_t *d_seq_len, uint32_t *d_status, hipStream_t st);
void launch_ingest_lines(const uint8_t *d_text, uint64_t n, const uint32_t *d_block_off, const uint32_t *d_total, uint32_t *d_line_start, hipStream_t st);
void launch_ingest_offsets(const uint32_t *d_seq_len, uint64_t n_rec, unsigned long long *d_tile, unsigned long long *d_off, hipStream_t st);
void launch_ingest_gather(const uint8_t *d_text, const uint32_t *d_seq_start, const uint32_t *d_seq_len, const unsigned long long *d_off,
                          uint32_t fixed_len, uint64_t n_rec, uint8_t *d_seq, hipStream_t st, uint32_t skip_from = 0xFFFFFFFFu);
void launch_ingest_select(const uint8_t *d_flags, uint32_t invert, const uint32_t *d_rec_start, uint64_t n_rec, uint32_t n_text, uint32_t *d_sel_len,
                          hipStream_t st);
void launch_ingest_fasta_count(const uint8_t *d_text, uint64_t n, const uint32_t *d_nl_block_off, const uint32_t *d_line_start,
                               unsigned long long *d_block64, hipStream_t st);
void launch_ingest_fasta_emit(const uint8_t *d_text, uint64_t n, const uint32_t *d_nl_block_off, const uint32_t *d_line_start,
                              unsigned long long *d_block64, uint8_t *d_seq, uint32_t *d_rec_start, unsigned long long *d_off, hipStream_t st);
uint32_t ingest_block_bytes();
uint32_t ingest_scan_tile();
void launch_bam_find(const uint8_t *d_text, uint64_t n, uint32_t piece, uint32_t n_pieces, uint32_t *d_start, hipStream_t st);
void launch_bam_walk_count(const uint8_t *d_text, uint64_t n, uint32_t piece, uint32_t n_pieces, const uint32_t *d_start, uint32_t *d_land,
                           uint32_t *d_count, hipStream_t st);
void launch_bam_walk_emit(const uint8_t *d_text, uint64_t n, uint32_t piece, uint32_t n_pieces, const uint32_t *d_start, const uint32_t *d_base,
                          uint32_t *d_rec_off, uint32_t *d_rec_len, uint32_t *d_seq_start, uint32_t *d_seq_len, uint32_t *d_st, hipStream_t st);
void launch_bam_unpack(const uint8_t *d_text, const uint32_t *d_seq_start, const uint32_t *d_seq_len, const unsigned long long *d_off, uint32_t fixed_len,
                       uint64_t n_rec, uint8_t *d_seq, hipStream_t st);
void launch_bam_taglen(const uint8_t *d_text, const uint32_t *d_rec_off, const uint32_t *d_rec_len, const uint32_t *d_seq_start, const uint32_t *d_seq_len,
                       const unsigned long long *d_found_off, const uint32_t *d_found_pat, const uint32_t *d_pat_off, const uint8_t *d_pat_bytes, uint64_t n_rec,
                       uint32_t filter_matching, uint32_t invert, uint32_t tag0, uint32_t tag1, uint8_t *d_keep, uint32_t *d_out_len, uint32_t *d_ex_off,
                       uint32_t *d_st, hipStream_t st);
void launch_bam_emit(const uint8_t *d_text, const uint32_t *d_rec_off, const uint32_t *d_rec_len, const uint32_t *d_out_len, const unsigned long long *d_out_off,
                     const unsigned long long *d_found_off, const uint32_t *d_found_pat, const uint8_t *d_pat_bytes, const uint32_t *d_pat_off,
                     const uint32_t *d_ex_off, uint64_t n_rec, uint32_t tag0, uint32_t tag1, uint8_t *d_out, hipStream_t st);
void launch_bam_names(const uint8_t *d_text, const uint32_t *d_rec_off, const uint8_t *d_flags, uint64_t n_rec, uint32_t *d_name_start, uint32_t *d_name_len,
                      hipStream_t st);
void launch_bam_sam_len(const uint8_t *d_text, const uint32_t *d_rec_off, const uint32_t *d_rec_len, const uint8_t *d_keep, uint64_t n_rec,
                        const uint8_t *d_ref_bytes, const uint32_t *d_ref_off, uint32_t n_refs, uint32_t *d_out_len, uint32_t *d_seq_at, uint32_t *d_st, hipStream_t st);
void launch_bam_sam_emit(const uint8_t *d_text, const uint32_t *d_rec_off, const uint32_t *d_rec_len, const uint32_t *d_seq_start, const uint32_t *d_seq_len,
                         const uint32_t *d_out_len, const unsigned long long *d_out_off, const uint32_t *d_seq_at, const unsigned long long *d_found_off,
                         const uint32_t *d_found_pat, const uint8_t *d_pat_bytes, const uint32_t *d_pat_off, const uint32_t *d_ex_off, const uint8_t *d_ref_bytes,
                         const uint32_t *d_ref_off, uint32_t n_refs, uint64_t n_rec, uint32_t tag0, uint32_t tag1, uint8_t *d_out, hipStream_t st);
struct SamTables {
    uint32_t *rec_start, *rec_len, *name_len, *seq_start, *seq_len, *aux_start;
};
void launch_sam_fields(const uint8_t *d_text, const uint32_t *d_line_start, uint64_t n_lines, uint32_t *d_is_rec, const SamTables &L, uint32_t *d_st,
                       hipStream_t st);
void launch_sam_compact(const uint32_t *d_is_rec, const unsigned long long *d_rec_index, uint64_t n_lines, const SamTables &L, const SamTables &R,
                        hipStream_t st);
void launch_sam_gather(const uint8_t *d_text, const uint32_t *d_seq_start, const uint32_t *d_seq_len, const unsigned long long *d_off, uint32_t fixed_len,
                       uint64_t n_rec, uint8_t *d_seq, hipStream_t st);
void launch_sam_names(const uint32_t *d_name_len, const uint8_t *d_flags, uint64_t n_rec, uint32_t *d_name_len_out, hipStream_t st);
void launch_sam_name_ends(const uint32_t *d_name_len_out, const unsigned long long *d_name_off, uint64_t n_rec, uint8_t *d_names, hipStream_t st);
void launch_sam_taglen(const uint8_t *d_text, const SamTables &R, const unsigned long long *d_found_off, const uint32_t *d_found_pat, const uint32_t *d_pat_off,
                       const uint8_t *d_pat_bytes, uint64_t n_rec, uint32_t filter_matching, uint32_t invert, uint32_t tag0, uint32_t tag1, uint8_t *d_keep,
                       uint32_t *d_out_len, uint32_t *d_ex_off, uint32_t *d_st, hipStream_t st);
void launch_sam_emit(const uint8_t *d_text, const SamTables &R, const uint32_t *d_out_len, const unsigned long long *d_out_off,
                     const unsigned long long *d_found_off, const uint32_t *d_found_pat, const uint8_t *d_pat_bytes, const uint32_t *d_pat_off,
                     const uint32_t *d_ex_off, uint64_t n_rec, uint32_t tag0, uint32_t tag1, uint8_t *d_out, hipStream_t st);
void launch_sam_bam_len(const uint8_t *d_text, const SamTables &R, const uint8_t *d_keep, uint64_t n_rec, uint32_t *d_out_len, uint32_t *d_n_cig, uint32_t *d_st,
                        hipStream_t st);
void launch_sam_bam_encode(const uint8_t *d_text, const SamTables &R, const uint8_t *d_keep, const uint32_t *d_out_len, const unsigned long long *d_out_off,
                           const uint32_t *d_n_cig, const unsigned long long *d_found_off, const uint32_t *d_found_pat, const uint8_t *d_pat_bytes,
                           const uint32_t *d_pat_off, const uint32_t *d_ex_off, const uint8_t *d_ref_bytes, const uint32_t *d_ref_off, const uint32_t *d_ref_table,
                           uint32_t ref_table_mask, uint64_t n_rec, uint32_t tag0, uint32_t tag1, uint8_t *d_out, hipStream_t st);

struct BuildParams {
    const uint8_t *pat_bytes;
    const uint32_t *pat_off;
    uint32_t n_pat;
    uint32_t S, q;
    uint32_t split, S2, q2;
    uint32_t gbloom_blocks;
    uint32_t gf_ctx;
    uint32_t *bloom;
    TableEntry *table;
    uint32_t bucket_mask;
    uint32_t *short_table;
};
void launch_build_tables(const BuildParams &B, uint64_t n_slots, hipStream_t st);

void launch_count_flags(const ScanParams &p, hipStream_t stream);

void launch_synth(uint64_t seed, uint64_t rec0, uint64_t n_rec, uint32_t read_len, uint32_t plant_every, const uint8_t *d_pat_bytes,
                  const uint32_t *d_pat_off, uint32_t n_pat, uint8_t *d_seq, uint64_t *d_seq_off, hipStream_t stream);

}
```

merkurio_amd/csrc/scan_kernel.hip:

```cpp
#include <algorithm>

#include "scan_kernel.h"

namespace mk {

__global__ __launch_bounds__(1024) void mk_count_flags_kernel(const uint8_t *__restrict__ flags, uint64_t n_rec,
                                                             unsigned long long *__restrict__ out) {
    const uint64_t head = std::min<uint64_t>(n_rec, (16 - ((uintptr_t)flags & 15)) & 15);
    const uint64_t n16 = (n_rec - head) / 16;
    const uint4 *__restrict__ v = reinterpret_cast<const uint4 *>(flags + head);
    unsigned long long c = 0;
    const uint64_t stride = (uint64_t)gridDim.x * blockDim.x;
    uint64_t i = (uint64_t)blockIdx.x * blockDim.x + threadIdx.x;
    for (; i + 3 * stride < n16; i += 4 * stride) {
        const uint4 a = v[i], b = v[i + stride], d = v[i + 2 * stride], e = v[i + 3 * stride];
        c += __popc(a.x) + __popc(a.y) + __popc(a.z) + __popc(a.w) + __popc(b.x) + __popc(b.y) + __popc(b.z) + __popc(b.w) +
             __popc(d.x) + __popc(d.y) + __popc(d.z) + __popc(d.w) + __popc(e.x) + __popc(e.y) + __popc(e.z) + __popc(e.w);
    }
    for (; i < n16; i += stride) {
        const uint4 a = v[i];
        c += __popc(a.x) + __popc(a.y) + __popc(a.z) + __popc(a.w);
    }
    if (blockIdx.x == 0 && threadIdx.x == 0) {
        for (uint64_t r = 0; r < head; ++r) c += flags[r] != 0;
        for (uint64_t r = head + n16 * 16; r < n_rec; ++r) c += flags[r] != 0;
    }
    __shared__ unsigned long long part[16];
    for (int o = 32; o > 0; o >>= 1) c += __shfl_down(c, o);
    if ((threadIdx.x & 63) == 0) part[threadIdx.x >> 6] = c;
    __syncthreads();
    if (threadIdx.x == 0) {
        unsigned long long t = 0;
        for (unsigned w = 0; w < blockDim.x / 64; ++w) t += part[w];
        if (t) atomicAdd(out, t);
    }
}

void launch_count_flags(const ScanParams &p, hipStream_t st) {
    const uint64_t n16 = p.n_rec / 16;
    const int blocks = (int)std::min<uint64_t>(256, std::max<uint64_t>(1, (n16 + 4095) / 4096));
    hipLaunchKernelGGL(mk_count_flags_kernel, dim3(blocks), dim3(1024), 0, st, reinterpret_cast<const uint8_t *>(p.rec_flags32),
                       p.n_rec, p.counters + p.n_pat + MK_SUM_RECORDS_HIT);
}

__global__ __launch_bounds__(1024) void mk_clear_kernel(uint32_t *__restrict__ flags32, uint64_t n_words,
                                                       unsigned long long *__restrict__ n_hits) {
    if (blockIdx.x == 0 && threadIdx.x == 0) *n_hits = 0;
    const uint64_t head = std::min<uint64_t>(n_words, ((16 - ((uintptr_t)flags32 & 15)) & 15) / 4);
    const uint64_t n16 = (n_words - head) / 4;
    uint4 *__restrict__ v = reinterpret_cast<uint4 *>(flags32 + head);
    const uint64_t stride = (uint64_t)gridDim.x * blockDim.x;
    for (uint64_t i = (uint64_t)blockIdx.x * blockDim.x + threadIdx.x; i < n16; i += stride) v[i] = make_uint4(0, 0, 0, 0);
    if (blockIdx.x == 0 && threadIdx.x < 8) {
        if (threadIdx.x < head) flags32[threadIdx.x] = 0;
        const uint64_t t = head + n16 * 4 + threadIdx.x;
        if (threadIdx.x < 4 && t < n_words) flags32[t] = 0;
    }
}

void launch_clear(uint32_t *flags32, uint64_t n_words, unsigned long long *n_hits, hipStream_t st) {
    const int blocks = (int)std::min<uint64_t>(512, std::max<uint64_t>(1, (n_words / 4 + 1023) / 1024));
    hipLaunchKernelGGL(mk_clear_kernel, dim3(blocks), dim3(1024), 0, st, flags32, n_words, n_hits);
}

__global__ __launch_bounds__(1024) void mk_flag_scatter_kernel(const uint32_t *__restrict__ list, const uint32_t *__restrict__ counts,
                                                              uint32_t cap, uint32_t n_waves, uint8_t *__restrict__ flags) {
    const uint32_t w = blockIdx.x * (blockDim.x / 64) + threadIdx.x / 64;
    if (w >= n_waves) return;
    const uint32_t n = counts[w] < cap ? counts[w] : cap;
    const uint32_t *__restrict__ l = list + (uint64_t)w * cap;
    for (uint32_t i = threadIdx.x & 63; i < n; i += 64) flags[l[i]] = 1;
}

void launch_flag_scatter(const uint32_t *flag_list, const uint32_t *flag_counts, uint32_t flag_cap, uint32_t n_waves, uint8_t *rec_flags,
                         hipStream_t st) {
    hipLaunchKernelGGL(mk_flag_scatter_kernel, dim3((n_waves + 15) / 16), dim3(1024), 0, st, flag_list, flag_counts, flag_cap, n_waves,
                       rec_flags);
}

constexpr uint32_t kHistLdsBins = 36864;
__global__ __launch_bounds__(1024) void mk_hist_hits_kernel(const mk_hit *__restrict__ hits, const unsigned long long *__restrict__ n_hits,
                                                            uint64_t cap, unsigned long long *__restrict__ counters, uint32_t n_pat) {
    __shared__ uint32_t bins[kHistLdsBins];
    const uint64_t n = std::min<uint64_t>(*n_hits, cap);
    const uint64_t per = std::max<uint64_t>(65536, (n + gridDim.x - 1) / gridDim.x);
    const uint64_t lo = (uint64_t)blockIdx.x * per;
    if (lo >= n) return;
    const uint64_t hi = std::min(n, lo + per);
    const bool in_lds = n_pat <= kHistLdsBins;
    if (in_lds) {
        for (uint32_t i = threadIdx.x; i < n_pat; i += blockDim.x) bins[i] = 0;
        __syncthreads();
    }
    for (uint64_t i = lo + threadIdx.x; i < hi; i += blockDim.x) {
        const uint32_t pat = hits[i].pat;
        if (pat >= n_pat) continue;
        if (in_lds)
            atomicAdd(&bins[pat], 1u);
        else
            atomicAdd(&counters[pat], 1ull);
    }
    if (in_lds) {
        __syncthreads();
        for (uint32_t i = threadIdx.x; i < n_pat; i += blockDim.x)
            if (bins[i]) atomicAdd(&counters[i], (unsigned long long)bins[i]);
    }
}

void launch_hist_hits(const ScanParams &p, int grid_blocks, hipStream_t st) {
    hipLaunchKernelGGL(mk_hist_hits_kernel, dim3(grid_blocks), dim3(1024), 0, st, p.hits, p.n_hits, p.hits_cap, p.counters, p.n_pat);
}

__global__ void mk_rec_index_kernel(const uint64_t *__restrict__ rec_off, uint64_t n_rec, uint64_t n_entries, uint32_t *__restrict__ out) {
    for (uint64_t k = (uint64_t)blockIdx.x * blockDim.x + threadIdx.x; k < n_entries; k += (uint64_t)gridDim.x * blockDim.x) {
        const uint64_t p = k << kRecIndexShift;
        uint64_t lo = 0, hi = n_rec;
        while (hi - lo > 1) {
            const uint64_t mid = (lo + hi) >> 1;
            if (rec_off[mid] <= p)
                lo = mid;
            else
                hi = mid;
        }
        out[k] = (uint32_t)lo;
    }
}

void launch_rec_index(const uint64_t *rec_off, uint64_t n_rec, uint64_t n_bytes, uint32_t *rec_index, hipStream_t stream) {
    const uint64_t n_entries = (n_bytes >> kRecIndexShift) + 2;
    const int blocks = (int)std::min<uint64_t>(2048, (n_entries + 255) / 256);
    hipLaunchKernelGGL(mk_rec_index_kernel, dim3(blocks), dim3(256), 0, stream, rec_off, n_rec, n_entries, rec_index);
}

__global__ void mk_add_u64_kernel(unsigned long long *__restrict__ dst, const unsigned long long *__restrict__ src, size_t len) {
    for (size_t i = (size_t)blockIdx.x * blockDim.x + threadIdx.x; i < len; i += (size_t)gridDim.x * blockDim.x) dst[i] += src[i];
}

void launch_add_u64(unsigned long long *dst, const unsigned long long *src, size_t len, hipStream_t stream) {
    const int blocks = (int)std::min<size_t>(1024, (len + 255) / 256);
    hipLaunchKernelGGL(mk_add_u64_kernel, dim3(blocks ? blocks : 1), dim3(256), 0, stream, dst, src, len);
}

template <int S, int QC, bool EMIT, bool GF, int FL = 1, int MC = 0>
static const char *launch_one(const ScanParams &p, int grid, hipStream_t st, const char *name) {
    launch_variant<S, QC, EMIT, GF, FL, MC>(p, grid, st);
    return name;
}

#define MK_VARIANT(S_, QC_, GF_)                                                                                   \
    return emit ? launch_one<S_, QC_, true, GF_>(p, grid_blocks, stream, "mk_scan_kernel<" #S_ "," #QC_ ",true," #GF_ ">") \
                : launch_one<S_, QC_, false, GF_>(p, grid_blocks, stream, "mk_scan_kernel<" #S_ "," #QC_ ",false," #GF_ ">")

#define MK_VARIANT_PLAIN(S_, QC_)                                                                                       \
    return emit ? launch_one<S_, QC_, true, false, 0>(p, grid_blocks, stream, "mk_scan_kernel<" #S_ "," #QC_ ",true,false,plain>") \
                : launch_one<S_, QC_, false, false, 0>(p, grid_blocks, stream, "mk_scan_kernel<" #S_ "," #QC_ ",false,false,plain>")
#define MK_VARIANT_MC(S_, QC_)                                                                                              \
    return emit ? launch_one<S_, QC_, true, false, 1, 1>(p, grid_blocks, stream, "mk_scan_kernel<" #S_ "," #QC_ ",true,false,2-class>") \
                : launch_one<S_, QC_, false, false, 1, 1>(p, grid_blocks, stream, "mk_scan_kernel<" #S_ "," #QC_ ",false,false,2-class>")
#define MK_VARIANT_MCS(S_, QC_)                                                                                                         \
    do {                                                                                                                                \
        if (p.short_bytes && p.s2 == 2)                                                                                                 \
            return emit ? launch_one<S_, QC_, true, false, 1, 2>(p, grid_blocks, stream, "mk_scan_kernel<" #S_ "," #QC_ ",true,false,s2=2,2-class>") \
                        : launch_one<S_, QC_, false, false, 1, 2>(p, grid_blocks, stream, "mk_scan_kernel<" #S_ "," #QC_ ",false,false,s2=2,2-class>"); \
        if (p.short_bytes && p.s2 == 4)                                                                                                 \
            return emit ? launch_one<S_, QC_, true, false, 1, 4>(p, grid_blocks, stream, "mk_scan_kernel<" #S_ "," #QC_ ",true,false,s2=4,2-class>") \
                        : launch_one<S_, QC_, false, false, 1, 4>(p, grid_blocks, stream, "mk_scan_kernel<" #S_ "," #QC_ ",false,false,s2=4,2-class>"); \
        if (p.short_bytes && p.s2 == 8)                                                                                                 \
            return emit ? launch_one<S_, QC_, true, false, 1, 8>(p, grid_blocks, stream, "mk_scan_kernel<" #S_ "," #QC_ ",true,false,s2=8,2-class>") \
                        : launch_one<S_, QC_, false, false, 1, 8>(p, grid_blocks, stream, "mk_scan_kernel<" #S_ "," #QC_ ",false,false,s2=8,2-class>"); \
        MK_VARIANT_MC(S_, QC_);                                                                                                         \
    } while (0)

const char *launch_scan(const ScanParams &p, int S, bool wide, bool emit, bool global_filter, int flavour, int grid_blocks,
                        hipStream_t stream) {
    const bool plain_loads = flavour == 0;
#define MK_VARIANT_MC_GF(S_, QC_)                                                                                          \
    return emit ? launch_one<S_, QC_, true, true, 1, 1>(p, grid_blocks, stream, "mk_scan_kernel<" #S_ "," #QC_ ",true,true,2-class>") \
                : launch_one<S_, QC_, false, true, 1, 1>(p, grid_blocks, stream, "mk_scan_kernel<" #S_ "," #QC_ ",false,true,2-class>")
    if (p.s2 && global_filter) {
        if (wide) switch (S) {
                case 2: MK_VARIANT_MC_GF(2, -1);
                case 4: MK_VARIANT_MC_GF(4, -1);
                case 8: MK_VARIANT_MC_GF(8, -1);
                case 16: MK_VARIANT_MC_GF(16, -1);
                default: return nullptr;
            }
        switch (S) {
            case 2: MK_VARIANT_MC_GF(2, 0);
            case 4: MK_VARIANT_MC_GF(4, 0);
            case 8: MK_VARIANT_MC_GF(8, 0);
            case 16: MK_VARIANT_MC_GF(16, 0);
            default: return nullptr;
        }
    }
#undef MK_VARIANT_MC_GF
    if (p.s2) {
        if (S == 16 && p.q == 16) MK_VARIANT_MCS(16, 16);
        if (S == 8 && p.q == 24) MK_VARIANT_MCS(8, 24);
        if (S == 4 && p.q == 28) MK_VARIANT_MCS(4, 28);
        if (S == 4 && p.q == 18) MK_VARIANT_MCS(4, 18);
        if (wide) switch (S) {
                case 2: MK_VARIANT_MC(2, -1);
                case 4: MK_VARIANT_MC(4, -1);
                case 8: MK_VARIANT_MC(8, -1);
                case 16: MK_VARIANT_MC(16, -1);
                default: return nullptr;
            }
        switch (S) {
            case 2: MK_VARIANT_MC(2, 0);
            case 4: MK_VARIANT_MC(4, 0);
            case 8: MK_VARIANT_MC(8, 0);
            case 16: MK_VARIANT_MC(16, 0);
            default: return nullptr;
        }
    }
    if (global_filter) {
        if (S == 8 && p.q == 14) MK_VARIANT(8, 14, true);
        if (S == 4 && p.q == 18) MK_VARIANT(4, 18, true);
        if (S == 8 && p.q == 24) MK_VARIANT(8, 24, true);
        if (wide) switch (S) {
                case 1: MK_VARIANT(1, -1, true);
                case 2: MK_VARIANT(2, -1, true);
                case 4: MK_VARIANT(4, -1, true);
                case 8: MK_VARIANT(8, -1, true);
                case 16: MK_VARIANT(16, -1, true);
                default: return nullptr;
            }
        switch (S) {
            case 1: MK_VARIANT(1, 0, true);
            case 2: MK_VARIANT(2, 0, true);
            case 4: MK_VARIANT(4, 0, true);
            case 8: MK_VARIANT(8, 0, true);
            case 16: MK_VARIANT(16, 0, true);
            default: return nullptr;
        }
    }
    if (plain_loads) {
        if (S == 16 && p.q == 16) MK_VARIANT_PLAIN(16, 16);
        if (S == 8 && p.q == 24) MK_VARIANT_PLAIN(8, 24);
        if (S == 4 && p.q == 28) MK_VARIANT_PLAIN(4, 28);
        if (S == 4 && p.q == 18) MK_VARIANT_PLAIN(4, 18);
        if (wide) switch (S) {
                case 1: MK_VARIANT_PLAIN(1, -1);
                case 2: MK_VARIANT_PLAIN(2, -1);
                case 4: MK_VARIANT_PLAIN(4, -1);
                case 8: MK_VARIANT_PLAIN(8, -1);
                case 16: MK_VARIANT_PLAIN(16, -1);
                default: return nullptr;
            }
        switch (S) {
            case 1: MK_VARIANT_PLAIN(1, 0);
            case 2: MK_VARIANT_PLAIN(2, 0);
            case 4: MK_VARIANT_PLAIN(4, 0);
            case 8: MK_VARIANT_PLAIN(8, 0);
            case 16: MK_VARIANT_PLAIN(16, 0);
            default: return nullptr;
        }
    }
    if (S == 16 && p.q == 16) MK_VARIANT(16, 16, false);
    if (S == 8 && p.q == 24) MK_VARIANT(8, 24, false);
    if (S == 4 && p.q == 28) MK_VARIANT(4, 28, false);
    if (S == 4 && p.q == 18) MK_VARIANT(4, 18, false);
    if (wide) switch (S) {
            case 1: MK_VARIANT(1, -1, false);
            case 2: MK_VARIANT(2, -1, false);
            case 4: MK_VARIANT(4, -1, false);
            case 8: MK_VARIANT(8, -1, false);
            case 16: MK_VARIANT(16, -1, false);
            default: return nullptr;
        }
    switch (S) {
        case 1: MK_VARIANT(1, 0, false);
        case 2: MK_VARIANT(2, 0, false);
        case 4: MK_VARIANT(4, 0, false);
        case 8: MK_VARIANT(8, 0, false);
        case 16: MK_VARIANT(16, 0, false);
        default: return nullptr;
    }
}
#undef MK_VARIANT
#undef MK_VARIANT_PLAIN
#undef MK_VARIANT_MC
#undef MK_VARIANT_MCS

__global__ void mk_synth_fill_kernel(uint64_t seed, uint64_t byte0, uint64_t n_bytes, uint8_t *__restrict__ seq) {
    const uint64_t n16 = (n_bytes + 15) / 16;
    const uint64_t blk0 = byte0 >> 5;
    for (uint64_t i = (uint64_t)blockIdx.x * blockDim.x + threadIdx.x; i < n16; i += (uint64_t)gridDim.x * blockDim.x) {
        const uint64_t bits = synth_block(seed, blk0 + (i >> 1)) >> (32 * (i & 1));
        uint32_t w[4];
#pragma unroll
        for (int k = 0; k < 4; ++k) {
            uint32_t v = 0;
#pragma unroll
            for (int b = 0; b < 4; ++b) v |= (uint32_t)synth_base(bits, 4 * k + b) << (8 * b);
            w[k] = v;
        }
        const uint64_t pos = i * 16;
        if (pos + 16 <= n_bytes) {
            *reinterpret_cast<uint4 *>(seq + pos) = make_uint4(w[0], w[1], w[2], w[3]);
        } else {
            for (uint64_t k = 0; pos + k < n_bytes; ++k) seq[pos + k] = (uint8_t)(w[k >> 2] >> (8 * (k & 3)));
        }
    }
}

__global__ void mk_synth_off_plant_kernel(uint64_t seed, uint64_t rec0, uint64_t n_rec, uint32_t read_len, uint32_t plant_every,
                                          const uint8_t *__restrict__ pat_bytes, const uint32_t *__restrict__ pat_off,
                                          uint32_t n_pat, uint8_t *__restrict__ seq, uint64_t *__restrict__ seq_off) {
    for (uint64_t r = (uint64_t)blockIdx.x * blockDim.x + threadIdx.x; r <= n_rec; r += (uint64_t)gridDim.x * blockDim.x) {
        seq_off[r] = r * read_len;
        if (r == n_rec || plant_every == 0) continue;
        const uint64_t gr = rec0 + r;
        const uint64_t h = synth_rec_hash(seed, gr);
        if (h % plant_every != 0) continue;
        const uint32_t pat = (uint32_t)((gr * 2654435761ull) % n_pat);
        const uint32_t a = pat_off[pat], len = pat_off[pat + 1] - a;
        if (len > read_len) continue;
        const uint32_t o = (uint32_t)((h >> 32) % (read_len - len + 1));
        for (uint32_t i = 0; i < len; ++i) seq[r * read_len + o + i] = pat_bytes[a + i];
    }
}

void launch_synth(uint64_t seed, uint64_t rec0, uint64_t n_rec, uint32_t read_len, uint32_t plant_every, const uint8_t *d_pat_bytes,
                  const uint32_t *d_pat_off, uint32_t n_pat, uint8_t *d_seq, uint64_t *d_seq_off, hipStream_t stream) {
    const uint64_t n_bytes = n_rec * read_len;
    hipLaunchKernelGGL(mk_synth_fill_kernel, dim3(2048), dim3(256), 0, stream, seed, rec0 * read_len, n_bytes, d_seq);
    hipLaunchKernelGGL(mk_synth_off_plant_kernel, dim3(2048), dim3(256), 0, stream, seed, rec0, n_rec, read_len, plant_every,
                       d_pat_bytes, d_pat_off, n_pat, d_seq, d_seq_off);
}

}
```

merkurio_amd/csrc/scan_kernel_impl.hpp:

```cpp
#pragma once
#include <algorithm>

#include "scan_kernel.h"

namespace mk {

typedef uint32_t u32x4 __attribute__((ext_vector_type(4)));

__device__ __forceinline__ uint32_t pack4_top(uint32_t d) { return (d & 0x06060606u) * 0x00820820u; }
__device__ __forceinline__ uint32_t pack16(uint4 v) {
    const uint32_t u0 = pack4_top(v.x), u1 = pack4_top(v.y), u2 = pack4_top(v.z), u3 = pack4_top(v.w);
    const uint32_t lo16 = __builtin_amdgcn_perm(u1, u0, 0x0c0c0703u);
    const uint32_t hi16 = __builtin_amdgcn_perm(u3, u2, 0x07030c0cu);
    return lo16 | hi16;
}

__device__ __forceinline__ uint4 load16(const uint8_t *__restrict__ seq, uint64_t pos, uint64_t n) {
    if (pos + 16 <= n) return *reinterpret_cast<const uint4 *>(seq + pos);
    uint32_t w[4] = {0, 0, 0, 0};
    if (pos < n) {
        uint32_t rem = (uint32_t)(n - pos);
        for (uint32_t i = 0; i < rem; ++i) w[i >> 2] |= (uint32_t)seq[pos + i] << (8 * (i & 3));
    }
    return make_uint4(w[0], w[1], w[2], w[3]);
}

struct alignas(8) CandEntry {
    uint32_t h;
    uint32_t t_lo;
};
constexpr uint32_t kRingEntries = 128;
constexpr uint32_t kHitSlots = 64;
constexpr uint32_t kLdsSumWords = 4;
constexpr uint32_t kLdsBytes = kBloomBytes + (kBlockThreads / 64) * kRingEntries * sizeof(CandEntry) +
                               (kBlockThreads / 64) * kHitSlots * 8;
constexpr uint32_t kShortBitmapBytes = kShortBitmapWords * 4;
static_assert(kLdsBytes + kShortBitmapBytes <= 160 * 1024, "one workgroup per CU");

#ifndef MK_ABLATE
#define MK_ABLATE 0
#endif

template <bool EMIT, int FL>
__device__ __forceinline__ bool resolve_one(const ScanParams &P, uint32_t pat, uint64_t p, uint32_t &n_true, mk_hit &out) {
    if constexpr ((MK_ABLATE & 16) != 0) return false;
    const uint32_t a = P.uniform_len ? pat * P.uniform_len : P.pat_off[pat];
    const uint32_t len = P.uniform_len ? P.uniform_len : P.pat_off[pat + 1] - a;
    if (p + len > P.n_bytes) return false;
    const uint8_t *__restrict__ tx = P.seq + p;
    const uint8_t *__restrict__ pt = P.pat_bytes + a;
    constexpr bool WIDE = FL != 1;
    const uint64_t n = P.n_rec;
    uint64_t rstart, rend, lo;
    if (P.rec_len) {
        lo = (uint64_t)((double)p * P.inv_rec_len);
        rstart = lo * P.rec_len;
        if (rstart > p) {
            --lo;
            rstart -= P.rec_len;
        } else if (p - rstart >= P.rec_len) {
            ++lo;
            rstart += P.rec_len;
        }
        rend = rstart + P.rec_len;
    } else {
        lo = (uint64_t)((double)p * P.rec_per_byte + 1e-6);
        if (P.rec_index) {
            const uint32_t k = (uint32_t)(p >> kRecIndexShift);
            const uint32_t r0 = P.rec_index[k], r1 = P.rec_index[k + 1];
            lo = r0 + ((((uint32_t)p & ((1u << kRecIndexShift) - 1u)) * (uint64_t)(r1 - r0 + 1)) >> kRecIndexShift);
            if (lo > r1) lo = r1;
        }
        if (lo >= n) lo = n - 1;
        if constexpr (WIDE) {
            uint64_t rpair[2];
            __builtin_memcpy(rpair, P.rec_off + lo, 16);
            rstart = rpair[0], rend = rpair[1];
        } else {
            rstart = P.rec_off[lo], rend = P.rec_off[lo + 1];
        }
    }
    if (P.case_insensitive) {
        for (uint32_t i = 0; i < len; ++i)
            if (fold_ascii(tx[i]) != fold_ascii(pt[i])) return false;
    } else {
        uint64_t diff = 0;
        if (WIDE && len >= 16) {
            const uint32_t last = len - 16;
            uint64_t x[2], y[2], u[2], v[2];
            __builtin_memcpy(x, tx, 16);
            __builtin_memcpy(y, pt, 16);
            __builtin_memcpy(u, tx + last, 16);
            __builtin_memcpy(v, pt + last, 16);
            diff = (x[0] ^ y[0]) | (x[1] ^ y[1]) | (u[0] ^ v[0]) | (u[1] ^ v[1]);
            for (uint32_t o = 16; o < last; o += 16) {
                __builtin_memcpy(x, tx + o, 16);
                __builtin_memcpy(y, pt + o, 16);
                diff |= (x[0] ^ y[0]) | (x[1] ^ y[1]);
            }
        } else if (len >= 8) {
            const uint32_t last = len - 8;
#pragma unroll
            for (uint32_t i = 0; i < 4; ++i) {
                const uint32_t o = 8 * i < last ? 8 * i : last;
                uint64_t x, y;
                __builtin_memcpy(&x, tx + o, 8);
                __builtin_memcpy(&y, pt + o, 8);
                diff |= x ^ y;
            }
            for (uint32_t o = 32; o < len; o += 8) {
                const uint32_t oo = o < last ? o : last;
                uint64_t x, y;
                __builtin_memcpy(&x, tx + oo, 8);
                __builtin_memcpy(&y, pt + oo, 8);
                diff |= x ^ y;
            }
        } else {
            for (uint32_t i = 0; i < len; ++i) diff |= (uint64_t)(tx[i] ^ pt[i]);
        }
        if (diff) return false;
    }
    if (!(rstart <= p && p < rend)) {
        uint64_t hi;
        if (rstart <= p) {
            hi = lo + 1;
            uint64_t step = 1;
            while (hi < n && P.rec_off[hi] <= p) {
                lo = hi;
                step <<= 1;
                hi = (n - hi > step) ? hi + step : n;
            }
        } else {
            hi = lo;
            uint64_t step = 1;
            lo = lo - 1;
            while (P.rec_off[lo] > p) {
                hi = lo;
                step <<= 1;
                lo = lo > step ? lo - step : 0;
            }
        }
        while (hi - lo > 1) {
            const uint64_t mid = (lo + hi) >> 1;
            if (P.rec_off[mid] <= p)
                lo = mid;
            else
                hi = mid;
        }
        rstart = P.rec_off[lo];
        rend = P.rec_off[lo + 1];
    }
    if (p + len > rend) return false;
    if constexpr ((MK_ABLATE & 32) != 0) {
        n_true++;
        return false;
    }
    n_true++;
    out.rec = lo;
    if (EMIT) {
        out.pat = pat;
        out.pos = (uint32_t)(p - rstart);
        if (p - rstart > 0xFFFFFFFFull) atomicOr(P.error_word, 1u);
    }
    return true;
}

struct HitRing {
    uint2 *q;
    uint32_t count;
    mk_hit *stage;
    uint32_t staged;
    uint32_t *flist;
    uint32_t nflag;
};

template <bool FLAGS>
__device__ __forceinline__ void flush_stage(const ScanParams &P, HitRing &hr, uint32_t lane) {
    const uint32_t n = hr.staged;
    if (n == 0) return;
    unsigned long long base = 0;
    if (lane == 0) base = atomicAdd(P.n_hits, (unsigned long long)n);
    const uint32_t blo = __builtin_amdgcn_readfirstlane((uint32_t)base);
    const uint32_t bhi = __builtin_amdgcn_readfirstlane((uint32_t)(base >> 32));
    base = ((unsigned long long)bhi << 32) | blo;
    __builtin_amdgcn_fence(__ATOMIC_RELEASE, "workgroup");
    __builtin_amdgcn_fence(__ATOMIC_ACQUIRE, "workgroup");
    for (uint32_t i = lane; i < n; i += 64) {
        const uint4 v = reinterpret_cast<const uint4 *>(hr.stage)[i];
        if (base + i < P.hits_cap) reinterpret_cast<uint4 *>(P.hits)[base + i] = v;
        if constexpr (FLAGS && (MK_ABLATE & 256) == 0)
            reinterpret_cast<uint8_t *>(P.rec_flags32)[((uint64_t)v.y << 32) | v.x] = 1;
    }
    __builtin_amdgcn_fence(__ATOMIC_RELEASE, "workgroup");
    hr.staged = 0;
}

template <bool EMIT, int FL>
__device__ __forceinline__ void drain_hits(const ScanParams &P, HitRing &hr, uint64_t newest_end, uint32_t lane, uint32_t &n_true) {
    constexpr bool WIDE = FL == 0;
    const uint32_t n = hr.count;
    __builtin_amdgcn_fence(__ATOMIC_RELEASE, "wavefront");
    __builtin_amdgcn_wave_barrier();
    const uint2 e = hr.q[lane & (kHitSlots - 1)];
    __builtin_amdgcn_wave_barrier();
    bool hit = false;
    mk_hit out;
    if (lane < n) {
        uint64_t p = (newest_end & 0xFFFFFFFF00000000ull) | e.x;
        if (p >= newest_end) p -= 1ull << 32;
        hit = resolve_one<EMIT, FL>(P, e.y, p, n_true, out);
    }
    hr.count = 0;
    const uint64_t mm = __ballot(hit);
    if (mm == 0) return;
    const uint32_t below = __builtin_amdgcn_mbcnt_hi((uint32_t)(mm >> 32), __builtin_amdgcn_mbcnt_lo((uint32_t)mm, 0u));
    const uint32_t n_hit = (uint32_t)__popcll(mm);
    if constexpr (EMIT) {
        if constexpr (WIDE && (MK_ABLATE & 256) == 0)
            if (hit) reinterpret_cast<uint8_t *>(P.rec_flags32)[out.rec] = 1;
        if (hit) hr.stage[hr.staged + below] = out;
        hr.staged += n_hit;
        if (hr.staged > kHitStage - 64) flush_stage<!WIDE>(P, hr, lane);
    } else if constexpr ((MK_ABLATE & 256) == 0) {
        if (!WIDE && hr.flist && hr.nflag + n_hit <= P.flag_cap) {
            if (hit) hr.flist[hr.nflag + below] = (uint32_t)out.rec;
            hr.nflag += n_hit;
        } else if (hit) {
            reinterpret_cast<uint8_t *>(P.rec_flags32)[out.rec] = 1;
        }
    }
}

template <bool EMIT, int CS, int FL>
__device__ __forceinline__ bool probe_round(const ScanParams &P, bool active, uint32_t fp, uint32_t ctx, uint64_t t, uint4 v0, uint4 v1,
                                            uint32_t lane, HitRing &hr, uint64_t newest_end, uint32_t &n_true) {
    const uint32_t efp[4] = {v0.x, v0.z, v1.x, v1.z};
    const uint32_t epo[4] = {v0.y, v0.w, v1.y, v1.w};
#pragma unroll
    for (int k = 0; k < 4; ++k) {
        const uint32_t e_off = epo[k] & 15u, e_pat = (epo[k] & ~kBucketOverflow) >> 4;
        uint32_t want = fp;
        if constexpr (CS > 0) want = ctx_fp(fp, ctx & ctx_mask(e_off & (uint32_t)(CS - 1), (uint32_t)CS));
        const bool match = active && epo[k] != kEmptyPat && efp[k] == want && t >= e_off;
        const uint64_t mm = (MK_ABLATE & 64) ? 0ull : __ballot(match);
        if (mm) {
            const uint32_t cnt = (uint32_t)__popcll(mm);
            if (hr.count + cnt > kHitSlots) drain_hits<EMIT, FL>(P, hr, newest_end, lane, n_true);
            if (match) {
                const uint32_t below =
                    __builtin_amdgcn_mbcnt_hi((uint32_t)(mm >> 32), __builtin_amdgcn_mbcnt_lo((uint32_t)mm, 0u));
                hr.q[hr.count + below] = make_uint2((uint32_t)(t - e_off), e_pat);
            }
            hr.count += cnt;
        }
    }
    return active && epo[0] != kEmptyPat && (epo[0] & kBucketOverflow) != 0;
}

__device__ __forceinline__ void load_bucket(const ScanParams &P, bool active, uint32_t b, uint4 &v0, uint4 &v1) {
    v0 = make_uint4(0, kEmptyPat, 0, kEmptyPat);
    v1 = v0;
    if (active) {
        const uint4 *bp = reinterpret_cast<const uint4 *>(P.table + (size_t)b * kBucketEntries);
        v0 = bp[0];
        v1 = bp[1];
    }
}

template <bool EMIT, int CS, int FL>
__device__ __forceinline__ void probe_chain(const ScanParams &P, bool active, uint32_t b, uint32_t fp, uint32_t ctx, uint64_t t,
                                            uint32_t lane, HitRing &hr, uint64_t newest_end, uint32_t &n_true) {
    while (__ballot(active)) {
        uint4 v0, v1;
        load_bucket(P, active, b, v0, v1);
        active = probe_round<EMIT, CS, FL>(P, active, fp, ctx, t, v0, v1, lane, hr, newest_end, n_true);
        b = (b + 1) & P.table_mask;
    }
}

#ifndef MK_ISSUE_AT
#define MK_ISSUE_AT 56
#endif
#ifndef MK_ISSUE_AT_DENSE
#define MK_ISSUE_AT_DENSE 16
#endif
#ifndef MK_DRAIN_AT_DENSE
#define MK_DRAIN_AT_DENSE 16
#endif

template <int S, int QC, bool CTX, int MC = 0>
struct Geo {
    static constexpr bool kFixed = QC > 0;
    static constexpr int kNS = 16 / S;
    static constexpr int kSpan = kFixed ? (kNS - 1) * S + QC + (CTX ? 7 : 0) : 48;
    static constexpr bool kNeedW1 = kSpan > 16 || MC != 0, kNeedW2 = kSpan > 32;
};

template <int S2, bool BYTES>
__device__ __forceinline__ uint32_t short_filter(const uint32_t *__restrict__ bm, uint32_t w0, uint32_t w1, uint32_t kmask) {
    uint32_t cand = 0;
#pragma unroll
    for (int j = 0; j < 16 / S2; ++j) {
        const int sh = 2 * j * S2;
        const uint32_t x = sh == 0 ? w0 : (BYTES && sh <= 20) ? (w0 >> sh) : __builtin_amdgcn_alignbit(w1, w0, sh);
        const uint32_t key = x & kmask;
        if constexpr (BYTES) {
            cand |= (uint32_t) reinterpret_cast<const uint8_t *>(bm)[key] << j;
        } else {
            const uint32_t word = bm[key >> 5];
            cand |= ((word >> (key & 31u)) & 1u) << j;
        }
    }
    return cand;
}

__device__ __forceinline__ uint32_t stream32_rt(uint32_t w0, uint32_t w1, uint32_t w2, uint32_t bit) {
    const uint32_t k = bit >> 5;
    const uint32_t a = k == 0 ? w0 : k == 1 ? w1 : w2;
    const uint32_t b = k == 0 ? w1 : k == 1 ? w2 : 0u;
    return __builtin_amdgcn_alignbit(b, a, bit & 31u);
}

__device__ __forceinline__ uint32_t stream32(uint32_t w0, uint32_t w1, uint32_t w2, int bit) {
    const int k = bit >> 5, r = bit & 31;
    const uint32_t a = k == 0 ? w0 : k == 1 ? w1 : k == 2 ? w2 : 0u;
    const uint32_t b = k == 0 ? w1 : k == 1 ? w2 : 0u;
    return r ? __builtin_amdgcn_alignbit(b, a, r) : a;
}

template <int S, int QC>
__device__ __forceinline__ uint32_t sample_hash(uint32_t w0, uint32_t w1, uint32_t w2, int sh, uint32_t mask_lo,
                                                uint32_t mask_hi) {
    constexpr uint32_t C1 = 0x9E3779u, C2 = 0x85EBCBu;
    if constexpr (QC > 0) {
        const uint32_t lo = stream32(w0, w1, w2, sh);
        if constexpr (QC <= 12) {
            return __umul24(lo & ((1u << (2 * QC)) - 1u), C1);
        } else if constexpr (QC < 16) {
            const uint32_t l = lo & ((1u << (2 * QC)) - 1u);
            return __umul24(l, C1) + __umul24(l >> 24, C2);
        } else if constexpr (QC == 16) {
            return __umul24(lo, C1) + __umul24(lo >> 24, C2);
        } else if constexpr (QC < 24) {
            const uint32_t t = stream32(w0, w1, w2, sh + 24) & ((1u << (2 * QC - 24)) - 1u);
            return __umul24(lo, C1) + __umul24(t, C2);
        } else if constexpr (QC == 24) {
            const uint32_t t = stream32(w0, w1, w2, sh + 24);
            return __umul24(lo, C1) + __umul24(t, C2);
        } else {
            const uint32_t t = stream32(w0, w1, w2, sh + 24);
            constexpr uint32_t top = QC >= 28 ? 0xFF000000u : (((1u << (2 * QC - 48)) - 1u) << 24);
            return __umul24(lo, C1) + __umul24(t, C2) + (t & top);
        }
    } else {
        const uint32_t lo = stream32(w0, w1, w2, sh) & mask_lo;
        const uint32_t hi = QC == 0 ? 0u : (stream32(w0, w1, w2, sh + 32) & mask_hi);
        const uint32_t t = __builtin_amdgcn_alignbit(hi, lo, 24);
        return __umul24(lo, C1) + __umul24(t, C2) + (t & 0xFF000000u);
    }
}

template <int S, int QC, bool EMIT, bool GF, int FL, int MC = 0>
__global__ __launch_bounds__(kBlockThreads) void mk_scan_kernel(const ScanParams P) {
    static_assert(!(MC != 0 && GF && QC > 0), "two length classes with the main filter in global memory: the runtime-q kernels only "
                                              "(the context fingerprints of the fixed-q ones cover the main class's geometry)");
    constexpr bool NTL = FL != 0;
    constexpr bool kCtx = GF && QC > 0;
    constexpr int CS = kCtx ? S : 0;
    using G = Geo<S, QC, kCtx, MC>;
    constexpr bool kPipe = kCtx && G::kNS <= 2 && (MK_ABLATE & 7) == 0;
    constexpr bool kWide = FL == 0;
    constexpr uint32_t kShortWords = MC != 0 ? kShortBitmapWords : 0;
    __shared__ __attribute__((aligned(16))) uint32_t lds_all[kShortWords + kLdsBytes / 4];
    uint32_t *const bloom = lds_all + kShortWords;
    uint32_t *lds_sums = bloom + kBloomWords;
    const uint32_t *short_bm = lds_all;
    if constexpr (!GF) {
        const uint4 *src = reinterpret_cast<const uint4 *>(P.bloom);
        uint4 *dst = reinterpret_cast<uint4 *>(bloom);
        for (uint32_t i = threadIdx.x; i < kBloomWords / 4; i += kBlockThreads) dst[i] = src[i];
    }
    if constexpr (MC != 0) {
        const uint4 *src2 = reinterpret_cast<const uint4 *>(P.short_bitmap);
        uint4 *dst2 = reinterpret_cast<uint4 *>(lds_all);
        for (uint32_t i = threadIdx.x; i < kShortBitmapWords / 4; i += kBlockThreads) dst2[i] = src2[i];
    }
    if constexpr (!GF || MC != 0) __syncthreads();
    const uint2 *__restrict__ gbloom = reinterpret_cast<const uint2 *>(P.bloom);
    const uint32_t gmask = P.gbloom_blocks;

    if (P.counters && blockIdx.x == 0 && threadIdx.x == 0) {
        atomicAdd(&P.counters[P.n_pat + MK_SUM_RECORDS], (unsigned long long)P.n_rec);
        atomicAdd(&P.counters[P.n_pat + MK_SUM_BASES], (unsigned long long)P.n_bytes);
    }
    const uint32_t lane = threadIdx.x & 63u;
    const uint32_t wave_in_block = __builtin_amdgcn_readfirstlane(threadIdx.x >> 6);
    const uint64_t wave_id = (uint64_t)blockIdx.x * (kBlockThreads / 64) + wave_in_block;
    const uint64_t n_waves = (uint64_t)gridDim.x * (kBlockThreads / 64);
    constexpr int NS = G::kNS;
    constexpr uint64_t kTileBytes = (uint64_t)kTileChunks * kChunkBytes;
    const uint32_t mask_lo = P.key_mask_lo, mask_hi = P.key_mask_hi;
    const uint8_t *__restrict__ seq = P.seq;
    const uint64_t n_bytes = P.n_bytes;
    CandEntry *ring = reinterpret_cast<CandEntry *>(bloom + kBloomWords) + wave_in_block * kRingEntries;
    uint32_t *ctx_ring = bloom + wave_in_block * kRingEntries;
    uint32_t q_head = 0, q_count = 0, n_cand = 0;
    HitRing hr;
    hr.q = reinterpret_cast<uint2 *>(bloom + kBloomWords + (kBlockThreads / 64) * kRingEntries * 2) + wave_in_block * kHitSlots;
    hr.count = 0;
    hr.stage = EMIT ? P.stage + wave_id * (uint64_t)kHitStage : nullptr;
    hr.staged = 0;
    hr.flist = (!kWide && !EMIT && P.flag_list) ? P.flag_list + wave_id * (uint64_t)P.flag_cap : nullptr;
    hr.nflag = 0;
    uint32_t n_true = 0;
    uint32_t abl_acc = 0;

    auto halo = [&](uint32_t pk_cur, uint32_t pk_nxt, uint32_t &w1, uint32_t &w2) __attribute__((always_inline)) {
        w1 = 0;
        w2 = 0;
        if constexpr (G::kNeedW1) {
            const uint32_t n0 = __builtin_amdgcn_readlane(pk_nxt, 0);
            w1 = __builtin_amdgcn_update_dpp(n0, pk_cur, 0x130, 0xf, 0xf, false);
        }
        if constexpr (G::kNeedW2) {
            const uint32_t n1 = __builtin_amdgcn_readlane(pk_nxt, 1);
            w2 = __builtin_amdgcn_update_dpp(n1, w1, 0x130, 0xf, 0xf, false);
        }
    };
    auto filter_chunk = [&](uint32_t pk_cur, uint32_t pk_nxt, uint32_t &h0, uint32_t &h1) __attribute__((always_inline)) -> uint32_t {
        const uint32_t w0 = pk_cur;
        uint32_t w1, w2;
        halo(pk_cur, pk_nxt, w1, w2);
        if constexpr ((MK_ABLATE & 4) != 0) return ((w0 ^ w1 ^ w2) == 0x12345678u) ? 1u : 0u;
        uint32_t cand = 0;
        const char *bloom_bytes = reinterpret_cast<const char *>(bloom);
#pragma unroll
        for (int j = 0; j < NS; ++j) {
            uint32_t h = sample_hash<S, QC>(w0, w1, w2, 2 * j * S, mask_lo, mask_hi);
            if (j == 0) h0 = h;
            if (j == 1) h1 = h;
            uint2 blk;
            if constexpr ((MK_ABLATE & 2) != 0) {
                blk = make_uint2(h & 0x10101010u, h);
            } else if constexpr (GF) {
                blk = gbloom[gbloom_block(h, gmask)];
                h = gbloom_bits(h);
            } else {
                blk = *reinterpret_cast<const uint2 *>(bloom_bytes + bloom_block_byte(h));
            }
            uint32_t m = (blk.x >> (h >> 27)) & (blk.y >> (h >> 22)) & (blk.y >> (h >> 17));
            if constexpr (GF) m &= blk.x >> (h >> 12);
            cand |= (m & 1u) << j;
        }
        if constexpr (MC != 0) {
            uint32_t c2;
#if defined(MK_MC_ABL) && MK_MC_ABL == 1
            c2 = 0;
#elif defined(MK_MC_ABL) && MK_MC_ABL == 2
            c2 = short_filter<4, true>(short_bm, w0, w1, P.key2_mask);
#else
            if constexpr (MC > 1) {
                c2 = short_filter<MC, true>(short_bm, w0, w1, P.key2_mask);
            } else if (P.short_bytes) {
                switch (P.s2) {
                    case 1: c2 = short_filter<1, true>(short_bm, w0, w1, P.key2_mask); break;
                    case 2: c2 = short_filter<2, true>(short_bm, w0, w1, P.key2_mask); break;
                    case 4: c2 = short_filter<4, true>(short_bm, w0, w1, P.key2_mask); break;
                    default: c2 = short_filter<8, true>(short_bm, w0, w1, P.key2_mask); break;
                }
            } else {
                switch (P.s2) {
                    case 1: c2 = short_filter<1, false>(short_bm, w0, w1, P.key2_mask); break;
                    case 2: c2 = short_filter<2, false>(short_bm, w0, w1, P.key2_mask); break;
                    case 4: c2 = short_filter<4, false>(short_bm, w0, w1, P.key2_mask); break;
                    default: c2 = short_filter<8, false>(short_bm, w0, w1, P.key2_mask); break;
                }
            }
#endif
            cand |= c2 << 16;
        }
        if constexpr ((MK_ABLATE & 1) != 0) {
            abl_acc += cand;
            cand = 0;
        }
        return cand;
    };

    bool pend_on = false;
    bool pend_active = false;
    uint32_t pend_fp = 0, pend_b = 0, pend_ctx = 0;
    uint64_t pend_t = 0;
    uint4 pend_v0 = make_uint4(0, 0, 0, 0), pend_v1 = pend_v0;
    uint64_t newest_end = 0;
    auto take_from_ring = [&](uint32_t n, bool &active, uint32_t &b, uint32_t &fp, uint32_t &ctx, uint64_t &t) __attribute__((always_inline)) {
        __builtin_amdgcn_fence(__ATOMIC_RELEASE, "wavefront");
        __builtin_amdgcn_wave_barrier();
        const CandEntry e = ring[(q_head + lane) & (kRingEntries - 1)];
        ctx = 0;
        if constexpr (kCtx) ctx = ctx_ring[(q_head + lane) & (kRingEntries - 1)];
        __builtin_amdgcn_wave_barrier();
        active = lane < n;
        b = table_bucket(e.h, P.table_mask);
        fp = e.h;
        t = (newest_end & 0xFFFFFFFF00000000ull) | e.t_lo;
        if (t >= newest_end) t -= 1ull << 32;
        q_head = (q_head + n) & (kRingEntries - 1);
        q_count -= n;
    };
    auto drain_ring = [&](uint32_t n) __attribute__((always_inline)) {
        bool active;
        uint32_t b, fp;
        uint64_t t;
        uint32_t ctx;
        take_from_ring(n, active, b, fp, ctx, t);
        probe_chain<EMIT, CS, FL>(P, active, b, fp, ctx, t, lane, hr, newest_end, n_true);
    };
    auto issue_probe = [&](uint32_t n) __attribute__((always_inline)) {
        take_from_ring(n, pend_active, pend_b, pend_fp, pend_ctx, pend_t);
        load_bucket(P, pend_active, pend_b, pend_v0, pend_v1);
        pend_on = true;
    };
    auto consume_probe = [&]() __attribute__((always_inline)) {
        const bool more = probe_round<EMIT, CS, FL>(P, pend_active, pend_fp, pend_ctx, pend_t, pend_v0, pend_v1, lane, hr, newest_end, n_true);
        if (__ballot(more))
            probe_chain<EMIT, CS, FL>(P, more, (pend_b + 1) & P.table_mask, pend_fp, pend_ctx, pend_t, lane, hr, newest_end, n_true);
        pend_on = false;
    };

    uint32_t slot_h = 0, slot_t = 0, slot_c = 0;
    bool slot_full = false;
    auto flush_slots = [&]() __attribute__((always_inline)) {
        const uint64_t full = __ballot(slot_full);
        if (!full) return;
        if (q_count > 64) drain_ring(64);
        if (slot_full) {
            const uint32_t below =
                __builtin_amdgcn_mbcnt_hi((uint32_t)(full >> 32), __builtin_amdgcn_mbcnt_lo((uint32_t)full, 0u));
            CandEntry e;
            e.h = slot_h;
            e.t_lo = slot_t;
            ring[(q_head + q_count + below) & (kRingEntries - 1)] = e;
            if constexpr (kCtx) ctx_ring[(q_head + q_count + below) & (kRingEntries - 1)] = slot_c;
        }
        q_count += (uint32_t)__popcll(full);
        n_cand += (uint32_t)__popcll(full);
        slot_full = false;
    };
    auto queue_candidates = [&](uint32_t pk_cur, uint32_t pk_nxt, uint32_t wm1, uint32_t cand, uint64_t cpos, uint32_t h0, uint32_t h1) __attribute__((always_inline)) {
        const uint32_t w0 = pk_cur;
        uint32_t w1 = 0, w2 = 0;
        if constexpr (NS > 2 || kCtx || MC != 0) halo(pk_cur, pk_nxt, w1, w2);
        newest_end = cpos + kChunkBytes;
        const uint32_t t_base = (uint32_t)cpos + lane * 16;
        do {
            if (__ballot(cand != 0 && slot_full)) flush_slots();
            if (cand != 0) {
                const uint32_t j = (uint32_t)__ffs(cand) - 1u;
                cand &= cand - 1;
                if constexpr (NS <= 2) {
                    slot_h = j ? h1 : h0;
                } else {
                    const uint32_t sh = 2u * j * S;
                    const uint32_t klo = __builtin_amdgcn_alignbit(w1, w0, sh) & mask_lo;
                    const uint32_t khi = __builtin_amdgcn_alignbit(w2, w1, sh) & mask_hi;
                    const uint32_t t = __builtin_amdgcn_alignbit(khi, klo, 24);
                    slot_h = __umul24(klo, 0x9E3779u) + __umul24(t, 0x85EBCBu) + (t & 0xFF000000u);
                }
                if constexpr (kCtx) {
                    const uint32_t pb = 2u * j * S;
                    const uint32_t prev7 = pb >= 14u ? (w0 >> (pb - 14u)) : __builtin_amdgcn_alignbit(w0, wm1, (pb + 18u) & 31u);
                    const uint32_t next7 = stream32_rt(w0, w1, w2, pb + 2u * (uint32_t)QC);
                    slot_c = (prev7 & 0x3FFFu) | ((next7 & 0x3FFFu) << 14);
                }
                slot_t = t_base + j * S;
                if constexpr (MC != 0) {
                    const uint32_t j2 = (j - 16u) << P.s2_log2;
                    const uint32_t fp2 = short_fp(__builtin_amdgcn_alignbit(w1, w0, 2u * j2) & P.key2_mask);
                    const bool is2 = j >= 16u;
                    slot_h = is2 ? fp2 : main_fp(slot_h);
                    slot_t = is2 ? t_base + j2 : slot_t;
                }
                slot_full = true;
            }
        } while (__ballot(cand != 0));
    };

    const uint64_t n_main_tiles = n_bytes >= kChunkBytes ? (n_bytes - kChunkBytes) / kTileBytes : 0;
    if (wave_id * (P.tile_run ? P.tile_run : 1u) < n_main_tiles) {
        const uint32_t run = P.tile_run ? P.tile_run : 1u;
        const uint64_t jump = (n_waves - 1) * (uint64_t)run + 1;
        uint64_t ld_tile = wave_id * run;
        uint32_t ld_run = 0;
        uint32_t ld_g = 0;
        const uint64_t last_tile = n_main_tiles - 1;
        const uint8_t *ld_ptr = seq + (ld_tile < last_tile ? ld_tile : last_tile) * kTileBytes + lane * 16;
        auto nt_load = [](const uint8_t *p) -> uint4 {
            if constexpr (NTL) {
                const u32x4 nv = __builtin_nontemporal_load(reinterpret_cast<const u32x4 *>(p));
                return make_uint4(nv.x, nv.y, nv.z, nv.w);
            } else {
                return *reinterpret_cast<const uint4 *>(p);
            }
        };
        auto load_group = [&](uint4 &a, uint4 &b, uint4 &c, uint4 &d) __attribute__((always_inline)) {
            a = nt_load(ld_ptr);
            b = nt_load(ld_ptr + kChunkBytes);
            c = nt_load(ld_ptr + 2 * kChunkBytes);
            d = nt_load(ld_ptr + 3 * kChunkBytes);
            ld_ptr += 4 * kChunkBytes;
            if (++ld_g == (uint32_t)(kTileChunks + 1) / 4) {
                ld_g = 0;
                if (++ld_run == run) {
                    ld_run = 0;
                    ld_tile += jump;
                } else {
                    ld_tile += 1;
                }
                const uint64_t t = ld_tile < last_tile ? ld_tile : last_tile;
                ld_ptr = seq + t * kTileBytes + lane * 16;
            }
        };
        uint4 r0, r1, r2, r3;
        load_group(r0, r1, r2, r3);
        uint32_t pk_prev = 0;
        uint32_t pk_pp = 0, pk_tile_prev = 0;
        bool pd_on = false;
        uint32_t pd_h0 = 0, pd_h1 = 0, pd_cur = 0, pd_nxt = 0, pd_wm1 = 0;
        uint2 pd_b0 = make_uint2(0, 0), pd_b1 = pd_b0;
        uint64_t pd_cpos = 0;
        auto test_pending = [&]() __attribute__((always_inline)) {
            auto pass = [](uint32_t h, uint2 blk) -> uint32_t {
                const uint32_t hb = gbloom_bits(h);
                return (blk.x >> (hb >> 27)) & (blk.x >> (hb >> 12)) & (blk.y >> (hb >> 22)) & (blk.y >> (hb >> 17)) & 1u;
            };
            uint32_t cand = pass(pd_h0, pd_b0);
            if constexpr (NS > 1) cand |= pass(pd_h1, pd_b1) << 1;
            if (__ballot(cand != 0)) queue_candidates(pd_cur, pd_nxt, pd_wm1, cand, pd_cpos, pd_h0, pd_h1);
        };
        uint64_t last_push_base = 0;
        uint32_t sc_run = 0;
        for (uint64_t tile = wave_id * run; tile < n_main_tiles;) {
            const uint64_t base = tile * kTileBytes;
            if constexpr (kCtx) {
                pk_tile_prev = 0;
                if (base >= 16) pk_tile_prev = pack16(*reinterpret_cast<const uint4 *>(seq + base - 16));
            }
            if (base - last_push_base >= (1ull << 30)) {
                last_push_base = base;
                flush_slots();
                if (hr.count) drain_hits<EMIT, FL>(P, hr, newest_end, lane, n_true);
                if (q_count && !pend_on) issue_probe(q_count < 64 ? q_count : 64);
            }
#pragma unroll 1
            for (int g = 0; g < (kTileChunks + 1) / 4; ++g) {
                const uint32_t p0 = pack16(r0), p1 = pack16(r1), p2 = pack16(r2), p3 = pack16(r3);
                asm volatile("" ::"v"(p0), "v"(p1), "v"(p2), "v"(p3) : "memory");
                if (pend_on) consume_probe();
                load_group(r0, r1, r2, r3);
                {
                    uint32_t q0 = p0, q1 = p1, q2 = p2;
#pragma unroll 1
                    for (int k = 0; k < 4; ++k) {
                        const int ci = 4 * g + k - 1;
                        if constexpr (kPipe) {
                            uint32_t nh0 = 0, nh1 = 0, nwm1 = 0;
                            uint2 nb0 = make_uint2(0, 0), nb1 = nb0;
                            if (ci >= 0) {
                                uint32_t w1, w2;
                                halo(pk_prev, q0, w1, w2);
                                nh0 = sample_hash<S, QC>(pk_prev, w1, w2, 0, mask_lo, mask_hi);
                                nb0 = gbloom[gbloom_block(nh0, gmask)];
                                if constexpr (NS > 1) {
                                    nh1 = sample_hash<S, QC>(pk_prev, w1, w2, 2 * S, mask_lo, mask_hi);
                                    nb1 = gbloom[gbloom_block(nh1, gmask)];
                                }
                                nwm1 = __builtin_amdgcn_update_dpp(__builtin_amdgcn_readlane(pk_pp, 63), pk_prev, 0x138, 0xf, 0xf, false);
                            }
                            if (pd_on) test_pending();
                            pd_on = ci >= 0;
                            pd_h0 = nh0;
                            pd_h1 = nh1;
                            pd_b0 = nb0;
                            pd_b1 = nb1;
                            pd_cur = pk_prev;
                            pd_nxt = q0;
                            pd_wm1 = nwm1;
                            pd_cpos = base + (uint64_t)(ci < 0 ? 0 : ci) * kChunkBytes;
                        } else if (ci >= 0) {
                            uint32_t h0 = 0, h1 = 0;
                            const uint32_t ck = filter_chunk(pk_prev, q0, h0, h1);
                            if constexpr ((MK_ABLATE & 4) != 0) n_cand += ck;
                            if (__ballot(ck != 0)) {
                                uint32_t wm1 = 0;
                                if constexpr (kCtx)
                                    wm1 = __builtin_amdgcn_update_dpp(__builtin_amdgcn_readlane(pk_pp, 63), pk_prev, 0x138, 0xf, 0xf, false);
                                queue_candidates(pk_prev, q0, wm1, ck, base + (uint64_t)ci * kChunkBytes, h0, h1);
                            }
                        }
                        if constexpr (kCtx) pk_pp = ci < 0 ? pk_tile_prev : pk_prev;
                        pk_prev = q0;
                        q0 = q1;
                        q1 = q2;
                        q2 = p3;
                    }
                }
                if constexpr ((MK_ABLATE & 8) != 0) {
                    if (q_count >= MK_ISSUE_AT) {
                        q_head = (q_head + q_count) & (kRingEntries - 1);
                        q_count = 0;
                    }
                } else if (!pend_on && q_count >= (FL == 0 ? MK_ISSUE_AT_DENSE : MK_ISSUE_AT)) {
                    issue_probe(q_count < 64 ? q_count : 64);
                }
                if constexpr (FL == 0 && MK_DRAIN_AT_DENSE <= 64) {
                    if (hr.count >= MK_DRAIN_AT_DENSE) drain_hits<EMIT, FL>(P, hr, newest_end, lane, n_true);
                }
                pk_prev = p3;
            }
            if (++sc_run == run) {
                sc_run = 0;
                tile += jump;
            } else {
                tile += 1;
            }
        }
        if constexpr (kPipe) {
            if (pd_on) test_pending();
        }
    }
    if (pend_on) consume_probe();

    {
        const uint64_t tail_rank = (wave_id + n_waves - (n_main_tiles / (P.tile_run ? P.tile_run : 1u)) % n_waves) % n_waves;
        for (uint64_t cpos = n_main_tiles * kTileBytes + tail_rank * kChunkBytes; cpos < n_bytes; cpos += n_waves * kChunkBytes) {
            const uint32_t pk_cur = pack16(load16(seq, cpos + lane * 16, n_bytes));
            const uint32_t pk_nxt = pack16(load16(seq, cpos + kChunkBytes + lane * 16, n_bytes));
            uint32_t h0 = 0, h1 = 0;
            const uint32_t ck = filter_chunk(pk_cur, pk_nxt, h0, h1);
            if constexpr ((MK_ABLATE & 4) != 0) n_cand += ck;
            if (__ballot(ck != 0)) {
                uint32_t wm1 = 0;
                if constexpr (kCtx) {
                    const uint64_t mine = cpos + lane * 16;
                    if (mine >= 16) wm1 = pack16(load16(seq, mine - 16, n_bytes));
                }
                queue_candidates(pk_cur, pk_nxt, wm1, ck, cpos, h0, h1);
            }
        }
    }

    flush_slots();
    while (q_count) drain_ring(q_count < 64 ? q_count : 64);
    if (hr.count) drain_hits<EMIT, FL>(P, hr, newest_end, lane, n_true);
    if constexpr (EMIT) flush_stage<!kWide>(P, hr, lane);
    if (hr.flist && lane == 0) P.flag_counts[wave_id] = hr.nflag;
    if ((MK_ABLATE & 1) != 0 && abl_acc == 0xFFFFFFFFu) n_cand++;
    if (P.counters) {
        __syncthreads();
        if (threadIdx.x < kLdsSumWords) lds_sums[threadIdx.x] = 0;
        __syncthreads();
        if (lane == 0 && n_cand) atomicAdd(&lds_sums[0], n_cand);
        if (n_true) atomicAdd(&lds_sums[1], n_true);
        __syncthreads();
        if (threadIdx.x == 0 && lds_sums[0]) atomicAdd(&P.counters[P.n_pat + MK_SUM_CANDIDATES], (unsigned long long)lds_sums[0]);
        if (threadIdx.x == 1 && lds_sums[1]) atomicAdd(&P.counters[P.n_pat + MK_SUM_HITS], (unsigned long long)lds_sums[1]);
    }
}

}
```

merkurio_amd/csrc/scan_variants.hip:

```cpp
#include "scan_kernel_impl.hpp"

#ifndef MK_TU
#error "compile with -DMK_TU=0..16"
#endif

namespace mk {

template <int S, int QC, bool EMIT, bool GF, int FL, int MC>
void launch_variant(const ScanParams &p, int grid_blocks, hipStream_t stream) {
    hipLaunchKernelGGL((mk_scan_kernel<S, QC, EMIT, GF, FL, MC>), dim3(grid_blocks), dim3(kBlockThreads), 0, stream, p);
}

#define MK_INST(S_, QC_, GF_)                                                                    \
    template void launch_variant<S_, QC_, false, GF_, 1, 0>(const ScanParams &, int, hipStream_t); \
    template void launch_variant<S_, QC_, true, GF_, 1, 0>(const ScanParams &, int, hipStream_t)
#define MK_INST_MC(S_, QC_, MC_)                                                                       \
    template void launch_variant<S_, QC_, false, false, 1, MC_>(const ScanParams &, int, hipStream_t); \
    template void launch_variant<S_, QC_, true, false, 1, MC_>(const ScanParams &, int, hipStream_t)
#define MK_INST_MC_GF(S_, QC_)                                                                       \
    template void launch_variant<S_, QC_, false, true, 1, 1>(const ScanParams &, int, hipStream_t); \
    template void launch_variant<S_, QC_, true, true, 1, 1>(const ScanParams &, int, hipStream_t)
#define MK_INST_PLAIN(S_, QC_, GF_)                                                               \
    template void launch_variant<S_, QC_, false, GF_, 0, 0>(const ScanParams &, int, hipStream_t); \
    template void launch_variant<S_, QC_, true, GF_, 0, 0>(const ScanParams &, int, hipStream_t)

#if MK_TU == 0
uint32_t scan_lds_bytes() { return kLdsBytes; }
MK_INST(16, 16, false);
MK_INST(8, 24, false);
MK_INST(4, 28, false);
MK_INST(4, 18, false);
#elif MK_TU == 6
MK_INST_PLAIN(16, 16, false);
MK_INST_PLAIN(8, 24, false);
MK_INST_PLAIN(4, 28, false);
MK_INST_PLAIN(4, 18, false);
#elif MK_TU == 7
MK_INST_PLAIN(1, 0, false);
MK_INST_PLAIN(2, 0, false);
MK_INST_PLAIN(4, 0, false);
MK_INST_PLAIN(8, 0, false);
MK_INST_PLAIN(16, 0, false);
#elif MK_TU == 8
MK_INST_PLAIN(1, -1, false);
MK_INST_PLAIN(2, -1, false);
MK_INST_PLAIN(4, -1, false);
MK_INST_PLAIN(8, -1, false);
MK_INST_PLAIN(16, -1, false);
#elif MK_TU == 1
MK_INST(1, 0, false);
MK_INST(2, 0, false);
MK_INST(4, 0, false);
MK_INST(8, 0, false);
MK_INST(16, 0, false);
#elif MK_TU == 2
MK_INST(1, -1, false);
MK_INST(2, -1, false);
MK_INST(4, -1, false);
MK_INST(8, -1, false);
MK_INST(16, -1, false);
#elif MK_TU == 3
MK_INST(8, 14, true);
MK_INST(4, 18, true);
MK_INST(8, 24, true);
#elif MK_TU == 4
MK_INST(1, 0, true);
MK_INST(2, 0, true);
MK_INST(4, 0, true);
MK_INST(8, 0, true);
MK_INST(16, 0, true);
#elif MK_TU == 5
MK_INST(1, -1, true);
MK_INST(2, -1, true);
MK_INST(4, -1, true);
MK_INST(8, -1, true);
MK_INST(16, -1, true);
#elif MK_TU == 9
MK_INST_MC(16, 16, 1);
MK_INST_MC(8, 24, 1);
MK_INST_MC(4, 28, 1);
MK_INST_MC(4, 18, 1);
#elif MK_TU == 10
MK_INST_MC(2, 0, 1);
MK_INST_MC(4, 0, 1);
MK_INST_MC(8, 0, 1);
MK_INST_MC(16, 0, 1);
#elif MK_TU == 11
MK_INST_MC(2, -1, 1);
MK_INST_MC(4, -1, 1);
MK_INST_MC(8, -1, 1);
MK_INST_MC(16, -1, 1);
#elif MK_TU == 12
MK_INST_MC(16, 16, 2);
MK_INST_MC(8, 24, 2);
MK_INST_MC(4, 28, 2);
MK_INST_MC(4, 18, 2);
#elif MK_TU == 13
MK_INST_MC(16, 16, 4);
MK_INST_MC(8, 24, 4);
MK_INST_MC(4, 28, 4);
MK_INST_MC(4, 18, 4);
#elif MK_TU == 14
MK_INST_MC(16, 16, 8);
MK_INST_MC(8, 24, 8);
MK_INST_MC(4, 28, 8);
MK_INST_MC(4, 18, 8);
#elif MK_TU == 15
MK_INST_MC_GF(2, 0);
MK_INST_MC_GF(4, 0);
MK_INST_MC_GF(8, 0);
MK_INST_MC_GF(16, 0);
#elif MK_TU == 16
MK_INST_MC_GF(2, -1);
MK_INST_MC_GF(4, -1);
MK_INST_MC_GF(8, -1);
MK_INST_MC_GF(16, -1);
#else
#error "unknown MK_TU"
#endif

}
```

merkurio_amd/native.py:

```python
import ctypes as C
import time
import importlib.util
import os

import numpy as np

from . import build as _build

MK_OK = 0
MK_E_EMPTY_PATTERN = -1
MK_E_INVALID_Q = -2
MK_E_PATTERN_TOO_LONG = -3
MK_E_NO_PATTERNS = -4
MK_E_NOMEM = -5
MK_E_PAIR_MISMATCH = -6
MK_E_HIP = -7
MK_E_CAPACITY = -8
MK_E_INVALID_ARG = -9
MK_E_UNSUPPORTED = -10
MK_E_RCCL = -11
MK_E_CORRUPT = -12
MK_COMM_ID_BYTES = 128

MK_ALGO_AUTO, MK_ALGO_AC, MK_ALGO_BNDMQ = 0, 1, 2
MK_FLAG_ASCII_CASE_INSENSITIVE = 1
MK_MODE_ANY, MK_MODE_HITS = 0, 1
MK_NUM_SUMMARY = 8
MK_SUM_HITS, MK_SUM_RECORDS_HIT, MK_SUM_RECORDS, MK_SUM_BASES, MK_SUM_CANDIDATES = 0, 1, 2, 3, 4

HIT_DTYPE = np.dtype([("rec", "<u8"), ("pat", "<u4"), ("pos", "<u4")])
ROW_DTYPE = np.dtype([("rec", "<u8"), ("pat", "<u4"), ("pos", "<u4"), ("file", "<u4"), ("_pad", "<u4")])

EXPORTS = [
    "mk_abi_version", "mk_last_error", "mk_device_count", "mk_read_kmers_from_text", "mk_parse_pattern_list",
    "mk_reverse_complement", "mk_canonical", "mk_recommend_aho_corasick", "mk_tune_q_value", "mk_generate_masks",
    "mk_free", "mk_matcher_create", "mk_matcher_create_ex", "mk_plan_geometry", "mk_matcher_destroy", "mk_matcher_algo", "mk_matcher_num_patterns",
    "mk_matcher_filter_info", "mk_matcher_class_info", "mk_matcher_filter_mode", "mk_scan_batch", "mk_scan_device", "mk_order_hits", "mk_order_hits_device", "mk_matcher_order_info", "mk_matcher_order_stats", "mk_matcher_kernel_name",
    "mk_matcher_launch_info", "mk_matcher_enable_timing", "mk_matcher_kernel_times", "mk_matcher_hint_hit_density", "mk_matcher_hint_record_lengths", "mk_matcher_set_fixed_record_length", "mk_matcher_check_device",
    "mk_extract_single", "mk_extract_fastq_text", "mk_upload_text_ahead", "mk_host_alloc", "mk_host_free", "mk_extract_paired", "mk_tag_records", "mk_tag_value", "mk_matcher_batch_times", "mk_synth_reads_device",
    "mk_synth_reads_host", "mk_synth_reads_device_range", "mk_reduce_counters", "mk_reduce_prepare", "mk_comm_available", "mk_comm_unique_id", "mk_comm_init",
    "mk_comm_reduce_counters", "mk_comm_size", "mk_comm_destroy",
    "mk_codec_create", "mk_codec_destroy", "mk_bgzf_deflate_bound", "mk_bgzf_deflate", "mk_bgzf_deflate_pieces", "mk_bgzf_inflate", "mk_bgzf_members", "mk_bgzf_eof",
    "mk_codec_times", "mk_codec_set_pass_limits", "mk_codec_set_inflate_kernel", "mk_codec_set_gzip_chunk", "mk_gzip_inflate_device", "mk_gzip_text_read", "mk_gzip_text_device", "mk_gzip_text_release", "mk_gzip_info", "mk_extract_fastq_bgzf", "mk_extract_window",
    "mk_tag_bam_window", "mk_matcher_set_bam_piece", "mk_tag_sam_window", "mk_tag_sam_bam_window", "mk_tag_bam_sam_window",
]


class MerkurioError(RuntimeError):
    def __init__(self, code, msg):
        super().__init__(f"[{code}] {msg}")
        self.code = code


class PatternError(MerkurioError):
    KINDS = {MK_E_EMPTY_PATTERN: "EmptyPattern", MK_E_INVALID_Q: "InvalidQGramLength",
             MK_E_PATTERN_TOO_LONG: "PatternTooLong"}

    @property
    def kind(self):
        return self.KINDS.get(self.code, "?")


class MatcherOptions(C.Structure):
    _fields_ = [("struct_size", C.c_uint32), ("force_stride", C.c_uint32), ("force_global_filter", C.c_uint32),
                ("gbloom_log2_blocks", C.c_uint32), ("tile_run", C.c_uint32), ("gbloom_kib", C.c_uint32),
                ("length_classes", C.c_uint32), ("force_split_len", C.c_uint32), ("force_stride2", C.c_uint32),
                ("force_q2", C.c_uint32)]

    def __init__(self, force_stride=0, force_global_filter=False, gbloom_log2_blocks=0, tile_run=0, gbloom_kib=0,
                 length_classes=0, force_split_len=0, force_stride2=0, force_q2=0, force_single_class=False):
        super().__init__(C.sizeof(MatcherOptions), int(force_stride), int(bool(force_global_filter)),
                         int(gbloom_log2_blocks), int(tile_run), int(gbloom_kib),
                         1 if force_single_class else int(length_classes), int(force_split_len), int(force_stride2), int(force_q2))


class WindowText(C.Structure):
    _fields_ = [("text", C.c_void_p), ("text_cap", C.c_uint64), ("tail", C.c_void_p), ("tail_cap", C.c_uint64), ("kept", C.c_void_p),
                ("kept_cap", C.c_uint64), ("n_text", C.c_uint64), ("n_used", C.c_uint64), ("n_tail", C.c_uint64), ("n_kept_bytes", C.c_uint64)]


class WindowSource(C.Structure):
    _fields_ = [("head", C.c_void_p), ("n_head", C.c_uint64), ("text", C.c_void_p), ("n_text", C.c_uint64), ("bgzf", C.c_void_p),
                ("n_bgzf", C.c_uint64), ("members", C.c_void_p), ("n_members", C.c_uint64), ("device_text", C.c_void_p), ("n_device_text", C.c_uint64), ("ends_at_record", C.c_uint32),
                ("reserved", C.c_uint32), ("rec_start", C.c_void_p), ("tail", C.c_void_p), ("tail_cap", C.c_uint64), ("kept", C.c_void_p),
                ("kept_cap", C.c_uint64), ("all", C.c_void_p), ("all_cap", C.c_uint64), ("n_window", C.c_uint64), ("n_used", C.c_uint64),
                ("n_tail", C.c_uint64), ("n_kept_bytes", C.c_uint64), ("n_rec_seen", C.c_uint64)]


MK_TEXT_FASTQ, MK_TEXT_FASTA = 0, 1


class BamWindow(C.Structure):
    _fields_ = [("head", C.c_void_p), ("n_head", C.c_uint64), ("bgzf", C.c_void_p), ("n_bgzf", C.c_uint64), ("members", C.c_void_p), ("n_members", C.c_uint64),
                ("last", C.c_uint32), ("filter_matching", C.c_uint32), ("invert", C.c_uint32), ("tag", C.c_uint8 * 2), ("reserved", C.c_uint8 * 2),
                ("block_bytes", C.c_uint32), ("tail", C.c_void_p), ("tail_cap", C.c_uint64), ("out", C.c_void_p), ("out_cap", C.c_uint64),
                ("rows", C.c_void_p), ("rows_cap", C.c_uint64), ("row_name", C.c_void_p), ("names", C.c_void_p), ("names_cap", C.c_uint64),
                ("on_tail", C.c_void_p), ("on_tail_ctx", C.c_void_p),
                ("n_window", C.c_uint64), ("n_used", C.c_uint64), ("n_tail", C.c_uint64), ("n_rec", C.c_uint64), ("n_kept", C.c_uint64),
                ("out_text_bytes", C.c_uint64), ("out_len", C.c_uint64), ("n_rows", C.c_uint64), ("n_names_bytes", C.c_uint64), ("ms", C.c_float * 8)]


class SamWindow(C.Structure):
    _fields_ = [("head", C.c_void_p), ("n_head", C.c_uint64), ("text", C.c_void_p), ("n_text", C.c_uint64),
                ("last", C.c_uint32), ("filter_matching", C.c_uint32), ("invert", C.c_uint32), ("tag", C.c_uint8 * 2), ("reserved", C.c_uint8 * 2),
                ("tail", C.c_void_p), ("tail_cap", C.c_uint64), ("out", C.c_void_p), ("out_cap", C.c_uint64),
                ("rows", C.c_void_p), ("rows_cap", C.c_uint64), ("row_name", C.c_void_p), ("names", C.c_void_p), ("names_cap", C.c_uint64),
                ("n_window", C.c_uint64), ("n_used", C.c_uint64), ("n_tail", C.c_uint64), ("n_rec", C.c_uint64), ("n_kept", C.c_uint64),
                ("out_len", C.c_uint64), ("n_rows", C.c_uint64), ("n_names_bytes", C.c_uint64), ("ms", C.c_float * 8)]


class SamBamWindow(C.Structure):
    _fields_ = [("head", C.c_void_p), ("n_head", C.c_uint64), ("text", C.c_void_p), ("n_text", C.c_uint64),
                ("last", C.c_uint32), ("filter_matching", C.c_uint32), ("invert", C.c_uint32), ("tag", C.c_uint8 * 2), ("reserved", C.c_uint8 * 2),
                ("ref_names", C.c_void_p), ("ref_off", C.c_void_p), ("n_refs", C.c_uint64), ("block_bytes", C.c_uint32), ("reserved2", C.c_uint32),
                ("tail", C.c_void_p), ("tail_cap", C.c_uint64), ("out", C.c_void_p), ("out_cap", C.c_uint64),
                ("rows", C.c_void_p), ("rows_cap", C.c_uint64), ("row_name", C.c_void_p), ("names", C.c_void_p), ("names_cap", C.c_uint64),
                ("n_window", C.c_uint64), ("n_used", C.c_uint64), ("n_tail", C.c_uint64), ("n_rec", C.c_uint64), ("n_kept", C.c_uint64),
                ("out_text_bytes", C.c_uint64), ("out_len", C.c_uint64), ("n_rows", C.c_uint64), ("n_names_bytes", C.c_uint64), ("ms", C.c_float * 8)]


class BamSamWindow(C.Structure):
    _fields_ = [("head", C.c_void_p), ("n_head", C.c_uint64), ("bgzf", C.c_void_p), ("n_bgzf", C.c_uint64), ("members", C.c_void_p), ("n_members", C.c_uint64),
                ("last", C.c_uint32), ("filter_matching", C.c_uint32), ("invert", C.c_uint32), ("tag", C.c_uint8 * 2), ("reserved", C.c_uint8 * 2),
                ("ref_names", C.c_void_p), ("ref_off", C.c_void_p), ("n_refs", C.c_uint64),
                ("tail", C.c_void_p), ("tail_cap", C.c_uint64), ("out", C.c_void_p), ("out_cap", C.c_uint64),
                ("rows", C.c_void_p), ("rows_cap", C.c_uint64), ("row_name", C.c_void_p), ("names", C.c_void_p), ("names_cap", C.c_uint64),
                ("on_tail", C.c_void_p), ("on_tail_ctx", C.c_void_p),
                ("n_window", C.c_uint64), ("n_used", C.c_uint64), ("n_tail", C.c_uint64), ("n_rec", C.c_uint64), ("n_kept", C.c_uint64),
                ("out_len", C.c_uint64), ("n_rows", C.c_uint64), ("n_names_bytes", C.c_uint64), ("ms", C.c_float * 8)]


class Counters(C.Structure):
    _fields_ = [("nb_records_tot", C.c_uint64), ("nb_bases", C.c_uint64), ("nb_hits_tot", C.c_uint64 * 2),
                ("nb_records_hit", C.c_uint64 * 2), ("nb_records_extracted", C.c_uint64)]

    def as_dict(self, counts):
        return {"records": self.nb_records_tot, "bases": self.nb_bases,
                "hits": (self.nb_hits_tot[0], self.nb_hits_tot[1]),
                "records_hit": (self.nb_records_hit[0], self.nb_records_hit[1]),
                "extracted": self.nb_records_extracted, "pattern_hit_counts": counts.tolist()}


_lib = None


def lib_path():
    return _build.LIB_PATH


def _bind_to_torch_hip_runtime():
    if os.environ.get("MERKURIO_SYSTEM_HIP") == "1":
        return None
    try:
        spec = importlib.util.find_spec("torch")
    except (ImportError, ValueError):
        spec = None
    if not spec or not spec.submodule_search_locations:
        return None
    path = os.path.join(list(spec.submodule_search_locations)[0], "lib", "libamdhip64.so")
    if not os.path.exists(path):
        return None
    return C.CDLL(path, mode=C.RTLD_GLOBAL)


def load(build_if_missing=True):
    global _lib
    if _lib is not None:
        return _lib
    _bind_to_torch_hip_runtime()
    path = os.environ.get("MERKURIO_LIB_PATH") or _build.LIB_PATH
    if path == _build.LIB_PATH and build_if_missing and (
            not os.path.exists(path) or os.environ.get("MERKURIO_REBUILD") == "1"):
        _build.build_lib()
    if not os.path.exists(path):
        raise MerkurioError(MK_E_HIP, f"{path} is missing: run `python -m merkurio_amd.build`")
    L = C.CDLL(path)
    L.mk_last_error.restype = C.c_char_p
    L.mk_matcher_kernel_name.restype = C.c_char_p
    L.mk_matcher_kernel_name.argtypes = [C.c_void_p]
    L.mk_tune_q_value.restype = C.c_size_t
    L.mk_tune_q_value.argtypes = [C.c_size_t]
    L.mk_recommend_aho_corasick.argtypes = [C.c_size_t, C.c_size_t]
    L.mk_free.argtypes = [C.c_void_p]
    L.mk_matcher_destroy.argtypes = [C.c_void_p]
    L.mk_matcher_algo.argtypes = [C.c_void_p]
    L.mk_matcher_algo.restype = C.c_uint32
    L.mk_matcher_num_patterns.argtypes = [C.c_void_p]
    L.mk_matcher_num_patterns.restype = C.c_uint32
    L.mk_matcher_create.argtypes = [C.c_void_p, C.c_void_p, C.c_uint32, C.c_uint32, C.c_uint32, C.c_uint32, C.c_int32,
                                    C.POINTER(C.c_void_p)]
    L.mk_matcher_create_ex.argtypes = [C.c_void_p, C.c_void_p, C.c_uint32, C.c_uint32, C.c_uint32, C.c_uint32, C.c_int32,
                                       C.POINTER(MatcherOptions), C.POINTER(C.c_void_p)]
    L.mk_synth_reads_device_range.argtypes = [C.c_void_p, C.c_uint64, C.c_uint64, C.c_uint64, C.c_uint32, C.c_uint32,
                                              C.c_void_p, C.c_void_p, C.c_void_p]
    L.mk_reduce_counters.argtypes = [C.POINTER(C.c_void_p), C.c_int, C.POINTER(C.c_void_p), C.c_size_t, C.c_void_p]
    L.mk_reduce_prepare.argtypes = [C.POINTER(C.c_void_p), C.c_int]
    L.mk_comm_unique_id.argtypes = [C.c_void_p]
    L.mk_comm_init.argtypes = [C.c_void_p, C.c_void_p, C.c_int, C.c_int]
    L.mk_comm_reduce_counters.argtypes = [C.c_void_p, C.c_void_p, C.c_size_t, C.c_void_p]
    L.mk_comm_destroy.argtypes = [C.c_void_p]
    L.mk_comm_size.argtypes = [C.c_void_p, C.POINTER(C.c_int)]
    L.mk_scan_batch.argtypes = [C.c_void_p, C.c_void_p, C.c_void_p, C.c_uint64, C.c_uint32, C.c_void_p, C.c_void_p,
                                C.c_uint64, C.POINTER(C.c_uint64)]
    L.mk_scan_device.argtypes = [C.c_void_p, C.c_void_p, C.c_uint64, C.c_void_p, C.c_uint64, C.c_uint32, C.c_void_p,
                                 C.c_void_p, C.c_uint64, C.c_void_p, C.c_void_p, C.c_void_p]
    L.mk_order_hits.argtypes = [C.c_void_p, C.c_void_p, C.c_uint64]
    L.mk_order_hits_device.argtypes = [C.c_void_p, C.c_void_p, C.c_uint64, C.c_void_p]
    L.mk_matcher_order_info.argtypes = [C.c_void_p, C.POINTER(C.c_uint32), C.POINTER(C.c_uint32), C.POINTER(C.c_uint32)]
    L.mk_matcher_launch_info.argtypes = [C.c_void_p, C.POINTER(C.c_uint32), C.POINTER(C.c_uint32), C.POINTER(C.c_uint32)]
    L.mk_matcher_enable_timing.argtypes = [C.c_void_p, C.c_uint32]
    L.mk_matcher_hint_hit_density.argtypes = [C.c_void_p, C.c_uint32]
    L.mk_matcher_hint_record_lengths.argtypes = [C.c_void_p, C.c_int]
    L.mk_matcher_set_fixed_record_length.argtypes = [C.c_void_p, C.c_uint32]
    L.mk_matcher_check_device.argtypes = [C.c_void_p, C.c_void_p]
    L.mk_matcher_batch_times.argtypes = [C.c_void_p, C.POINTER(C.c_float)]
    L.mk_matcher_kernel_times.argtypes = [C.c_void_p, C.c_void_p, C.c_uint32, C.POINTER(C.c_uint32)]
    L.mk_matcher_filter_info.argtypes = [C.c_void_p, C.POINTER(C.c_uint32), C.POINTER(C.c_uint32),
                                         C.POINTER(C.c_uint64), C.POINTER(C.c_uint64)]
    L.mk_matcher_filter_mode.argtypes = [C.c_void_p, C.POINTER(C.c_uint32), C.POINTER(C.c_uint64)]
    L.mk_plan_geometry.argtypes = [C.c_void_p, C.c_uint32, C.POINTER(MatcherOptions)] + [C.POINTER(C.c_uint32)] * 7
    L.mk_matcher_class_info.argtypes = [C.c_void_p, C.POINTER(C.c_uint32), C.POINTER(C.c_uint32), C.POINTER(C.c_uint32),
                                        C.POINTER(C.c_uint32)]
    L.mk_extract_single.argtypes = [C.c_void_p, C.c_void_p, C.c_void_p, C.c_uint64, C.c_int, C.c_int, C.c_void_p,
                                    C.c_void_p, C.c_uint64, C.POINTER(C.c_uint64), C.POINTER(Counters), C.c_void_p]
    L.mk_extract_fastq_text.argtypes = [C.c_void_p, C.c_void_p, C.c_uint64, C.c_int, C.c_int, C.c_uint64, C.POINTER(C.c_uint64), C.c_void_p,
                                        C.c_void_p, C.c_void_p, C.c_uint64, C.POINTER(C.c_uint64), C.POINTER(Counters), C.c_void_p,
                                        C.POINTER(C.c_uint32)]
    L.mk_upload_text_ahead.argtypes = [C.c_void_p, C.c_void_p, C.c_uint64]
    L.mk_host_alloc.argtypes = [C.c_size_t, C.POINTER(C.c_void_p)]
    L.mk_host_free.argtypes = [C.c_void_p]
    L.mk_host_free.restype = None
    L.mk_codec_create.argtypes = [C.c_int, C.POINTER(C.c_void_p)]
    L.mk_codec_destroy.argtypes = [C.c_void_p]
    L.mk_codec_destroy.restype = None
    L.mk_bgzf_deflate_bound.argtypes = [C.c_uint64, C.c_uint32]
    L.mk_bgzf_deflate_bound.restype = C.c_uint64
    L.mk_bgzf_deflate.argtypes = [C.c_void_p, C.c_void_p, C.c_uint64, C.c_uint32, C.c_void_p, C.c_uint64, C.POINTER(C.c_uint64)]
    L.mk_bgzf_deflate_pieces.argtypes = [C.c_void_p, C.c_void_p, C.c_void_p, C.c_uint64, C.c_uint32, C.c_void_p, C.c_uint64, C.POINTER(C.c_uint64)]
    L.mk_bgzf_inflate.argtypes = [C.c_void_p, C.c_void_p, C.c_uint64, C.c_void_p, C.c_uint64, C.c_void_p, C.c_uint64, C.POINTER(C.c_uint64)]
    L.mk_bgzf_members.argtypes = [C.c_void_p, C.c_uint64, C.c_void_p, C.c_uint64, C.POINTER(C.c_uint64), C.POINTER(C.c_uint64),
                                  C.POINTER(C.c_uint64)]
    L.mk_bgzf_eof.restype = C.POINTER(C.c_uint8 * 28)
    L.mk_codec_times.argtypes = [C.c_void_p, C.POINTER(C.c_float)]
    L.mk_codec_set_pass_limits.argtypes = [C.c_void_p, C.c_uint64, C.c_uint64]
    L.mk_codec_set_gzip_chunk.argtypes = [C.c_void_p, C.c_uint64]
    L.mk_codec_set_inflate_kernel.argtypes = [C.c_void_p, C.c_int]
    L.mk_gzip_inflate_device.argtypes = [C.c_void_p, C.c_void_p, C.c_uint64, C.POINTER(C.c_uint64), C.POINTER(C.c_uint32)]
    L.mk_gzip_text_read.argtypes = [C.c_void_p, C.c_uint64, C.c_void_p, C.c_uint64]
    L.mk_gzip_text_device.argtypes = [C.c_void_p, C.POINTER(C.c_uint64)]
    L.mk_gzip_text_device.restype = C.c_void_p
    L.mk_gzip_text_release.argtypes = [C.c_void_p]
    L.mk_gzip_info.argtypes = [C.c_void_p, C.POINTER(C.c_uint32), C.POINTER(C.c_float)]
    L.mk_extract_fastq_bgzf.argtypes = [C.c_void_p, C.c_void_p, C.c_void_p, C.c_uint64, C.c_void_p, C.c_uint64, C.c_void_p, C.c_uint64, C.c_int,
                                        C.POINTER(WindowText), C.c_int, C.c_int, C.c_uint64, C.POINTER(C.c_uint64), C.c_void_p, C.c_void_p, C.c_void_p,
                                        C.c_uint64, C.POINTER(C.c_uint64), C.POINTER(Counters), C.c_void_p, C.POINTER(C.c_uint32)]
    L.mk_extract_window.argtypes = [C.c_void_p, C.c_void_p, C.c_uint32, C.c_uint32, C.c_void_p, C.c_int, C.c_int, C.c_uint64, C.POINTER(C.c_uint64),
                                    C.c_void_p, C.c_void_p, C.c_uint64, C.POINTER(C.c_uint64), C.c_void_p, C.c_void_p, C.POINTER(C.c_uint32)]
    L.mk_matcher_order_stats.argtypes = [C.c_void_p, C.POINTER(C.c_uint64)]
    L.mk_tag_bam_window.argtypes = [C.c_void_p, C.c_void_p, C.POINTER(BamWindow), C.c_int, C.POINTER(Counters), C.c_void_p, C.POINTER(C.c_uint32)]
    L.mk_matcher_set_bam_piece.argtypes = [C.c_void_p, C.c_uint32]
    L.mk_tag_sam_window.argtypes = [C.c_void_p, C.POINTER(SamWindow), C.c_int, C.POINTER(Counters), C.c_void_p, C.POINTER(C.c_uint32)]
    L.mk_tag_sam_bam_window.argtypes = [C.c_void_p, C.c_void_p, C.POINTER(SamBamWindow), C.c_int, C.POINTER(Counters), C.c_void_p, C.POINTER(C.c_uint32)]
    L.mk_tag_bam_sam_window.argtypes = [C.c_void_p, C.c_void_p, C.POINTER(BamSamWindow), C.c_int, C.POINTER(Counters), C.c_void_p, C.POINTER(C.c_uint32)]
    L.mk_extract_paired.argtypes = [C.c_void_p, C.c_void_p, C.c_void_p, C.c_uint64, C.c_void_p, C.c_void_p, C.c_uint64,
                                    C.c_int, C.c_int, C.c_void_p, C.c_void_p, C.c_uint64, C.POINTER(C.c_uint64),
                                    C.POINTER(Counters), C.c_void_p]
    L.mk_tag_records.argtypes = [C.c_void_p, C.c_void_p, C.c_void_p, C.c_uint64, C.c_int, C.c_int, C.c_int, C.c_void_p,
                                 C.c_void_p, C.c_uint64, C.POINTER(C.c_uint64), C.POINTER(Counters), C.c_void_p,
                                 C.c_void_p, C.c_void_p, C.c_uint64]
    L.mk_tag_value.argtypes = [C.c_void_p, C.c_void_p, C.c_uint64, C.c_char_p, C.c_char_p, C.c_size_t,
                               C.POINTER(C.c_size_t)]
    L.mk_synth_reads_device.argtypes = [C.c_void_p, C.c_uint64, C.c_uint64, C.c_uint32, C.c_uint32, C.c_void_p,
                                        C.c_void_p, C.c_void_p]
    L.mk_synth_reads_host.argtypes = [C.c_void_p, C.c_uint64, C.c_uint64, C.c_uint64, C.c_uint32, C.c_uint32,
                                      C.c_void_p, C.c_void_p]
    L.mk_read_kmers_from_text.argtypes = [C.c_void_p, C.c_size_t, C.POINTER(C.c_void_p), C.POINTER(C.c_void_p),
                                          C.POINTER(C.c_uint32)]
    L.mk_parse_pattern_list.argtypes = [C.c_void_p, C.c_void_p, C.c_uint32, C.c_int, C.c_int, C.c_int, C.c_int,
                                        C.POINTER(C.c_void_p), C.POINTER(C.c_void_p), C.POINTER(C.c_uint32)]
    L.mk_reverse_complement.argtypes = [C.c_void_p, C.c_size_t, C.c_void_p]
    L.mk_canonical.argtypes = [C.c_void_p, C.c_size_t, C.c_void_p]
    L.mk_generate_masks.argtypes = [C.c_void_p, C.c_size_t, C.c_void_p, C.POINTER(C.c_uint64)]
    _lib = L
    return L


def _check(rc):
    if rc == MK_OK:
        return
    msg = load().mk_last_error().decode(errors="replace")
    if rc in PatternError.KINDS:
        raise PatternError(rc, msg)
    raise MerkurioError(rc, msg)


def device_count():
    return load().mk_device_count()


def pack_list(items):
    items = [bytes(x) for x in items]
    off = np.zeros(len(items) + 1, dtype=np.uint32)
    if items:
        off[1:] = np.cumsum([len(x) for x in items])
    data = np.frombuffer(b"".join(items) + b"\0", dtype=np.uint8).copy()
    return data, off


def pack_records(seqs):
    seqs = [bytes(x) for x in seqs]
    off = np.zeros(len(seqs) + 1, dtype=np.uint64)
    if seqs:
        off[1:] = np.cumsum([len(x) for x in seqs], dtype=np.uint64)
    data = np.frombuffer(b"".join(seqs) + b"\0", dtype=np.uint8).copy()
    return data, off


def _take_list(pb, po, n):
    L = load()
    off = np.ctypeslib.as_array(C.cast(po, C.POINTER(C.c_uint32)), shape=(n.value + 1,)).copy()
    total = int(off[-1])
    data = C.string_at(pb, total) if total else b""
    L.mk_free(pb)
    L.mk_free(po)
    return [data[off[i]:off[i + 1]] for i in range(n.value)]


def read_kmers_from_text(content: bytes):
    pb, po, n = C.c_void_p(), C.c_void_p(), C.c_uint32()
    buf = np.frombuffer(bytes(content) + b"\0", dtype=np.uint8)
    _check(load().mk_read_kmers_from_text(buf.ctypes.data, len(content), C.byref(pb), C.byref(po), C.byref(n)))
    return _take_list(pb, po, n)


def read_kmers_from_file(path):
    with open(path, "rb") as f:
        return read_kmers_from_text(f.read())


def parse_pattern_list(kmer_file=None, kmer_seq=None, reverse_complement=False, canonical=False, lowercase=False,
                       uppercase=False):
    if kmer_file is not None:
        raw = read_kmers_from_file(kmer_file)
    elif kmer_seq is not None:
        raw = [s.encode() if isinstance(s, str) else bytes(s) for s in kmer_seq]
    else:
        raise MerkurioError(MK_E_NO_PATTERNS, "No k-mer sequence provided.")
    data, off = pack_list(raw)
    pb, po, n = C.c_void_p(), C.c_void_p(), C.c_uint32()
    _check(load().mk_parse_pattern_list(data.ctypes.data, off.ctypes.data, len(raw), int(reverse_complement),
                                        int(canonical), int(lowercase), int(uppercase), C.byref(pb), C.byref(po),
                                        C.byref(n)))
    return _take_list(pb, po, n)


def reverse_complement(s: bytes) -> bytes:
    src = np.frombuffer(bytes(s) + b"\0", dtype=np.uint8)
    out = np.zeros(len(s) + 1, dtype=np.uint8)
    load().mk_reverse_complement(src.ctypes.data, len(s), out.ctypes.data)
    return out[:len(s)].tobytes()


def canonical(s: bytes) -> bytes:
    src = np.frombuffer(bytes(s) + b"\0", dtype=np.uint8)
    out = np.zeros(len(s) + 1, dtype=np.uint8)
    load().mk_canonical(src.ctypes.data, len(s), out.ctypes.data)
    return out[:len(s)].tobytes()


def recommend_aho_corasick(pattern_list) -> bool:
    return bool(load().mk_recommend_aho_corasick(len(pattern_list), max(len(p) for p in pattern_list)))


def tune_q_value(pattern) -> int:
    q = load().mk_tune_q_value(len(pattern))
    if q == 0:
# ... 599 lines not shown
```

Measured before the change: 6239.

## Fuse flag scatter into scan kernel and add optional two-group-deep load prefetch

Removes the separate flag-scatter kernel launch and its per-wave count buffer; each wave now writes its listed record flags directly at the end of the scan kernel after a workgroup fence. It also adds a depth-2 kernel variant that keeps two load groups in flight, selectable through a new force_depth option. Depth defaults to 1, so by default only the fused scatter and an added waitcnt in drain_hits take effect. The fused scatter saves a launch and a global round trip, at the cost of a tail loop inside the scan kernel.

```diff
diff --git a/include/merkurio_hip.h b/include/merkurio_hip.h
--- a/include/merkurio_hip.h
+++ b/include/merkurio_hip.h
@@ -86,6 +86,7 @@
     uint32_t force_split_len;
     uint32_t force_stride2;
     uint32_t force_q2;
+    uint32_t force_depth;
 } mk_matcher_options;
 int mk_matcher_create_ex(const uint8_t *pat_bytes, const uint32_t *pat_off, uint32_t n_pat, uint32_t algo, uint32_t q,
                          uint32_t flags, int32_t device, const mk_matcher_options *options, mk_matcher **out);
diff --git a/merkurio_amd/build.py b/merkurio_amd/build.py
--- a/merkurio_amd/build.py
+++ b/merkurio_amd/build.py
@@ -9,7 +9,7 @@
 LIB_PATH = os.path.join(LIB_DIR, "libmerkurio_hip.so")
 CLI_PATH = os.path.join(LIB_DIR, "merkurio")
 
-N_VARIANT_TUS = 17
+N_VARIANT_TUS = 19
 HOST_SOURCES = ["matcher.cpp", "host_patterns.cpp", "host_loops.cpp", "reduce.cpp"]
 HIPCC = os.environ.get("HIPCC", "/opt/rocm/bin/hipcc")
 FLAGS = ["--offload-arch=gfx950", "-O3", "-std=c++17", "-fPIC", "-Wall", "-Wno-unused-result"]
diff --git a/merkurio_amd/csrc/matcher.cpp b/merkurio_amd/csrc/matcher.cpp
--- a/merkurio_amd/csrc/matcher.cpp
+++ b/merkurio_amd/csrc/matcher.cpp
@@ -249,6 +249,7 @@
         if (opt.gbloom_log2_blocks != 0 && (opt.gbloom_log2_blocks < 10 || opt.gbloom_log2_blocks > 25))
             return fail(MK_E_INVALID_ARG, "gbloom_log2_blocks %u out of range (10..25)", opt.gbloom_log2_blocks);
         if (opt.tile_run > 8) return fail(MK_E_INVALID_ARG, "tile_run %u out of range (0..8)", opt.tile_run);
+        if (opt.force_depth > 2) return fail(MK_E_INVALID_ARG, "force_depth %u: must be 0 (rule), 1 or 2", opt.force_depth);
         if (opt.gbloom_kib > (1u << 18)) return fail(MK_E_INVALID_ARG, "gbloom_kib %u out of range (<= 256 MiB)", opt.gbloom_kib);
         if (opt.length_classes > 2) return fail(MK_E_INVALID_ARG, "length_classes %u: must be 0 (rule), 1 or 2", opt.length_classes);
         const uint32_t f2 = opt.force_stride2;
@@ -364,6 +365,7 @@
 
     m->uniform_len = (lmin == lmax) ? lmin : 0;
     m->tile_run = opt.tile_run;
+    m->force_depth = opt.force_depth;
     ClassPlan plan;
     {
         std::vector<uint32_t> lens(n_pat);
@@ -405,7 +407,6 @@
     MK_HIP(hipMemset(m->d_error, 0, 16));
     MK_HIP(hipMalloc((void **)&m->d_stage, (size_t)m->num_cus * (kBlockThreads / 64) * kHitStage * sizeof(mk_hit)));
     MK_HIP(hipMalloc((void **)&m->d_flag_list, (size_t)m->num_cus * (kBlockThreads / 64) * kFlagListCap * sizeof(uint32_t)));
-    MK_HIP(hipMalloc((void **)&m->d_flag_counts, (size_t)m->num_cus * (kBlockThreads / 64) * sizeof(uint32_t)));
     MK_HIP(hipMemcpy(m->d_pat_bytes, m->pat_bytes.data(), m->pat_bytes.size(), hipMemcpyHostToDevice));
     MK_HIP(hipMemsetAsync(m->d_pat_bytes + m->pat_bytes.size(), 0, 16, m->stream));
     MK_HIP(hipMemcpy(m->d_pat_off, m->pat_off.data(), (n_pat + 1) * sizeof(uint32_t), hipMemcpyHostToDevice));
@@ -474,7 +475,7 @@
     for (auto e : m->ev_stop) (void)hipEventDestroy(e);
     for (void *p : {(void *)m->d_bloom, (void *)m->d_table, (void *)m->d_pat_bytes, (void *)m->d_pat_off,
                     (void *)m->d_seq, (void *)m->d_off, (void *)m->d_flags, (void *)m->d_hits, (void *)m->d_nhits,
-                    (void *)m->d_stage, (void *)m->d_rec_index, (void *)m->d_flag_list, (void *)m->d_flag_counts, m->d_sort_tmp,
+                    (void *)m->d_stage, (void *)m->d_rec_index, (void *)m->d_flag_list, m->d_sort_tmp,
                     (void *)m->d_pat_rank, (void *)m->d_pat_unrank, (void *)m->d_error, m->d_aux, m->d_pair, (void *)m->d_short_table, m->d_refs, m->txt[0].d_text, m->txt[0].d_ing_a, m->txt[0].d_ing_b, m->txt[1].d_text, m->txt[1].d_ing_a, m->txt[1].d_ing_b, m->txt[0].d_fa_seq, m->txt[1].d_fa_seq, (void *)m->d_flags2, m->ahead[0].d, m->ahead[1].d, m->ahead[2].d, m->ahead[3].d})
         if (p) (void)hipFree(p);
     delete m;
@@ -569,6 +570,7 @@
     p.rec_per_byte = (double)n_rec / (double)n_bytes;
     const uint64_t tiles_per_wave = n_tiles / (blocks * waves_per_block);
     p.tile_run = m->tile_run ? m->tile_run : tiles_per_wave >= 16 ? 4 : tiles_per_wave >= 8 ? 2 : 1;
+    const int depth = m->force_depth ? (int)m->force_depth : 1;
     p.rec_index = nullptr;
     p.rec_len = rec_len;
     p.inv_rec_len = rec_len ? 1.0 / (double)rec_len : 0.0;
@@ -586,16 +588,13 @@
     const int flavour = plain_loads ? 0 : 1;
     const bool listed = !(plain_loads && m->gbloom_blocks == 0) && mode != MK_MODE_HITS && n_rec < (1ull << 32);
     p.flag_list = listed ? m->d_flag_list : nullptr;
-    p.flag_counts = m->d_flag_counts;
     p.flag_cap = kFlagListCap;
-    const char *name = launch_scan(p, (int)m->S, m->q > 16, mode == MK_MODE_HITS, m->gbloom_blocks != 0, flavour, (int)blocks, st);
+    const char *name = launch_scan(p, (int)m->S, m->q > 16, mode == MK_MODE_HITS, m->gbloom_blocks != 0, flavour, depth, (int)blocks, st);
     if (!name) return fail(MK_E_UNSUPPORTED, "no kernel for stride %u", m->S);
     if (slots) {
         MK_HIP(hipEventRecord(m->ev_stop[slot], st));
         m->timed_launches++;
     }
-    if (listed)
-        launch_flag_scatter(m->d_flag_list, m->d_flag_counts, kFlagListCap, (uint32_t)(blocks * waves_per_block), (uint8_t *)d_rec_flags, st);
     if (d_counters) {
         launch_count_flags(p, st);
         if (mode == MK_MODE_HITS && p.hits && p.hits_cap) launch_hist_hits(p, m->num_cus, st);
diff --git a/merkurio_amd/csrc/matcher_internal.h b/merkurio_amd/csrc/matcher_internal.h
--- a/merkurio_amd/csrc/matcher_internal.h
+++ b/merkurio_amd/csrc/matcher_internal.h
@@ -25,6 +25,7 @@
     uint32_t *d_bloom = nullptr;
     uint32_t gbloom_blocks = 0;
     uint32_t tile_run = 0;
+    uint32_t force_depth = 0;
     uint32_t hit_density_pm = 0;
     bool ragged = false;
     uint32_t fixed_rec_len = 0, batch_rec_len = 0;
@@ -46,7 +47,6 @@
     uint32_t *d_error = nullptr;
     mk_hit *d_stage = nullptr;
     uint32_t *d_flag_list = nullptr;
-    uint32_t *d_flag_counts = nullptr;
     void *d_sort_tmp = nullptr;
     size_t d_sort_tmp_cap = 0;
     uint32_t *d_pat_rank = nullptr;
diff --git a/merkurio_amd/csrc/scan_kernel.h b/merkurio_amd/csrc/scan_kernel.h
--- a/merkurio_amd/csrc/scan_kernel.h
+++ b/merkurio_amd/csrc/scan_kernel.h
@@ -40,7 +40,6 @@
     mk_hit *stage;
     uint32_t *rec_flags32;
     uint32_t *flag_list;
-    uint32_t *flag_counts;
     uint32_t flag_cap;
     mk_hit *hits;
     uint64_t hits_cap;
@@ -49,10 +48,13 @@
     uint32_t *error_word;
 };
 
-const char *launch_scan(const ScanParams &p, int S, bool wide, bool emit, bool global_filter, int flavour, int grid_blocks,
+const char *launch_scan(const ScanParams &p, int S, bool wide, bool emit, bool global_filter, int flavour, int depth, int grid_blocks,
                         hipStream_t stream);
 
-template <int S, int QC, bool EMIT, bool GF, int FL, int MC = 0>
+template <int S, int QC, bool EMIT, bool GF, int FL, int MC>
+constexpr bool kDepth2 = QC > 0 && !GF && MC == 0 && !(EMIT && FL == 0);
+
+template <int S, int QC, bool EMIT, bool GF, int FL, int MC = 0, int DEPTH = 1>
 void launch_variant(const ScanParams &p, int grid_blocks, hipStream_t stream);
 
 uint32_t scan_lds_bytes();
@@ -61,8 +63,6 @@
 
 constexpr uint32_t kRecIndexShift = 16;
 void launch_clear(uint32_t *flags32, uint64_t n_words, unsigned long long *n_hits, hipStream_t stream);
-void launch_flag_scatter(const uint32_t *flag_list, const uint32_t *flag_counts, uint32_t flag_cap, uint32_t n_waves, uint8_t *rec_flags,
-                         hipStream_t stream);
 void launch_rec_index(const uint64_t *rec_off, uint64_t n_rec, uint64_t n_bytes, uint32_t *rec_index, hipStream_t stream);
 struct OrderKey {
     const uint32_t *pat_off;
diff --git a/merkurio_amd/csrc/scan_kernel.hip b/merkurio_amd/csrc/scan_kernel.hip
--- a/merkurio_amd/csrc/scan_kernel.hip
+++ b/merkurio_amd/csrc/scan_kernel.hip
@@ -61,21 +61,6 @@
 void launch_clear(uint32_t *flags32, uint64_t n_words, unsigned long long *n_hits, hipStream_t st) {
     const int blocks = (int)std::min<uint64_t>(512, std::max<uint64_t>(1, (n_words / 4 + 1023) / 1024));
     hipLaunchKernelGGL(mk_clear_kernel, dim3(blocks), dim3(1024), 0, st, flags32, n_words, n_hits);
-}
-
-__global__ __launch_bounds__(1024) void mk_flag_scatter_kernel(const uint32_t *__restrict__ list, const uint32_t *__restrict__ counts,
-                                                              uint32_t cap, uint32_t n_waves, uint8_t *__restrict__ flags) {
-    const uint32_t w = blockIdx.x * (blockDim.x / 64) + threadIdx.x / 64;
-    if (w >= n_waves) return;
-    const uint32_t n = counts[w] < cap ? counts[w] : cap;
-    const uint32_t *__restrict__ l = list + (uint64_t)w * cap;
-    for (uint32_t i = threadIdx.x & 63; i < n; i += 64) flags[l[i]] = 1;
-}
-
-void launch_flag_scatter(const uint32_t *flag_list, const uint32_t *flag_counts, uint32_t flag_cap, uint32_t n_waves, uint8_t *rec_flags,
-                         hipStream_t st) {
-    hipLaunchKernelGGL(mk_flag_scatter_kernel, dim3((n_waves + 15) / 16), dim3(1024), 0, st, flag_list, flag_counts, flag_cap, n_waves,
-                       rec_flags);
 }
 
 constexpr uint32_t kHistLdsBins = 36864;
@@ -142,18 +127,24 @@
 }
 
 template <int S, int QC, bool EMIT, bool GF, int FL = 1, int MC = 0>
-static const char *launch_one(const ScanParams &p, int grid, hipStream_t st, const char *name) {
-    launch_variant<S, QC, EMIT, GF, FL, MC>(p, grid, st);
+static const char *launch_one(const ScanParams &p, int grid, hipStream_t st, const char *name, int depth = 1) {
+    if constexpr (kDepth2<S, QC, EMIT, GF, FL, MC>) {
+        if (depth == 2) {
+            launch_variant<S, QC, EMIT, GF, FL, MC, 2>(p, grid, st);
+            return name;
+        }
+    }
+    launch_variant<S, QC, EMIT, GF, FL, MC, 1>(p, grid, st);
     return name;
 }
 
 #define MK_VARIANT(S_, QC_, GF_)                                                                                   \
-    return emit ? launch_one<S_, QC_, true, GF_>(p, grid_blocks, stream, "mk_scan_kernel<" #S_ "," #QC_ ",true," #GF_ ">") \
-                : launch_one<S_, QC_, false, GF_>(p, grid_blocks, stream, "mk_scan_kernel<" #S_ "," #QC_ ",false," #GF_ ">")
+    return emit ? launch_one<S_, QC_, true, GF_>(p, grid_blocks, stream, "mk_scan_kernel<" #S_ "," #QC_ ",true," #GF_ ">", depth) \
+                : launch_one<S_, QC_, false, GF_>(p, grid_blocks, stream, "mk_scan_kernel<" #S_ "," #QC_ ",false," #GF_ ">", depth)
 
 #define MK_VARIANT_PLAIN(S_, QC_)                                                                                       \
-    return emit ? launch_one<S_, QC_, true, false, 0>(p, grid_blocks, stream, "mk_scan_kernel<" #S_ "," #QC_ ",true,false,plain>") \
-                : launch_one<S_, QC_, false, false, 0>(p, grid_blocks, stream, "mk_scan_kernel<" #S_ "," #QC_ ",false,false,plain>")
+    return emit ? launch_one<S_, QC_, true, false, 0>(p, grid_blocks, stream, "mk_scan_kernel<" #S_ "," #QC_ ",true,false,plain>", depth) \
+                : launch_one<S_, QC_, false, false, 0>(p, grid_blocks, stream, "mk_scan_kernel<" #S_ "," #QC_ ",false,false,plain>", depth)
 #define MK_VARIANT_MC(S_, QC_)                                                                                              \
     return emit ? launch_one<S_, QC_, true, false, 1, 1>(p, grid_blocks, stream, "mk_scan_kernel<" #S_ "," #QC_ ",true,false,2-class>") \
                 : launch_one<S_, QC_, false, false, 1, 1>(p, grid_blocks, stream, "mk_scan_kernel<" #S_ "," #QC_ ",false,false,2-class>")
@@ -171,7 +162,7 @@
         MK_VARIANT_MC(S_, QC_);                                                                                                         \
     } while (0)
 
-const char *launch_scan(const ScanParams &p, int S, bool wide, bool emit, bool global_filter, int flavour, int grid_blocks,
+const char *launch_scan(const ScanParams &p, int S, bool wide, bool emit, bool global_filter, int flavour, int depth, int grid_blocks,
                         hipStream_t stream) {
     const bool plain_loads = flavour == 0;
 #define MK_VARIANT_MC_GF(S_, QC_)                                                                                          \
diff --git a/merkurio_amd/csrc/scan_kernel_impl.hpp b/merkurio_amd/csrc/scan_kernel_impl.hpp
--- a/merkurio_amd/csrc/scan_kernel_impl.hpp
+++ b/merkurio_amd/csrc/scan_kernel_impl.hpp
@@ -210,6 +210,7 @@
         if (p >= newest_end) p -= 1ull << 32;
         hit = resolve_one<EMIT, FL>(P, e.y, p, n_true, out);
     }
+    __builtin_amdgcn_s_waitcnt(0x0F70);
     hr.count = 0;
     const uint64_t mm = __ballot(hit);
     if (mm == 0) return;
@@ -360,8 +361,9 @@
     }
 }
 
-template <int S, int QC, bool EMIT, bool GF, int FL, int MC = 0>
+template <int S, int QC, bool EMIT, bool GF, int FL, int MC = 0, int kDepth = 1>
 __global__ __launch_bounds__(kBlockThreads) void mk_scan_kernel(const ScanParams P) {
+    static_assert(kDepth == 1 || (kDepth == 2 && !GF && MC == 0 && QC > 0), "two load groups ahead: compile-time q, filter in LDS, one class");
     static_assert(!(MC != 0 && GF && QC > 0), "two length classes with the main filter in global memory: the runtime-q kernels only "
                                               "(the context fingerprints of the fixed-q ones cover the main class's geometry)");
     constexpr bool NTL = FL != 0;
@@ -622,6 +624,8 @@
         };
         uint4 r0, r1, r2, r3;
         load_group(r0, r1, r2, r3);
+        uint4 r4 = make_uint4(0, 0, 0, 0), r5 = r4, r6 = r4, r7 = r4;
+        if constexpr (kDepth == 2) load_group(r4, r5, r6, r7);
         uint32_t pk_prev = 0;
         uint32_t pk_pp = 0, pk_tile_prev = 0;
         bool pd_on = false;
@@ -651,12 +655,7 @@
                 if (hr.count) drain_hits<EMIT, FL>(P, hr, newest_end, lane, n_true);
                 if (q_count && !pend_on) issue_probe(q_count < 64 ? q_count : 64);
             }
-#pragma unroll 1
-            for (int g = 0; g < (kTileChunks + 1) / 4; ++g) {
-                const uint32_t p0 = pack16(r0), p1 = pack16(r1), p2 = pack16(r2), p3 = pack16(r3);
-                asm volatile("" ::"v"(p0), "v"(p1), "v"(p2), "v"(p3) : "memory");
-                if (pend_on) consume_probe();
-                load_group(r0, r1, r2, r3);
+            auto scan_group = [&](uint32_t p0, uint32_t p1, uint32_t p2, uint32_t p3, int g) __attribute__((always_inline)) {
                 {
                     uint32_t q0 = p0, q1 = p1, q2 = p2;
 #pragma unroll 1
@@ -704,18 +703,53 @@
                         q2 = p3;
                     }
                 }
+            };
+            auto end_group = [&](bool may_issue) __attribute__((always_inline)) {
                 if constexpr ((MK_ABLATE & 8) != 0) {
                     if (q_count >= MK_ISSUE_AT) {
                         q_head = (q_head + q_count) & (kRingEntries - 1);
                         q_count = 0;
                     }
-                } else if (!pend_on && q_count >= (FL == 0 ? MK_ISSUE_AT_DENSE : MK_ISSUE_AT)) {
+                } else if (may_issue && !pend_on && q_count >= (FL == 0 ? MK_ISSUE_AT_DENSE : MK_ISSUE_AT)) {
                     issue_probe(q_count < 64 ? q_count : 64);
                 }
                 if constexpr (FL == 0 && MK_DRAIN_AT_DENSE <= 64) {
                     if (hr.count >= MK_DRAIN_AT_DENSE) drain_hits<EMIT, FL>(P, hr, newest_end, lane, n_true);
                 }
-                pk_prev = p3;
+            };
+            if constexpr (kDepth == 1) {
+#pragma unroll 1
+                for (int g = 0; g < (kTileChunks + 1) / 4; ++g) {
+                    const uint32_t p0 = pack16(r0), p1 = pack16(r1), p2 = pack16(r2), p3 = pack16(r3);
+                    asm volatile("" ::"v"(p0), "v"(p1), "v"(p2), "v"(p3) : "memory");
+                    if (pend_on) consume_probe();
+                    load_group(r0, r1, r2, r3);
+                    scan_group(p0, p1, p2, p3, g);
+                    end_group(true);
+                    pk_prev = p3;
+                }
+            } else {
+                static_assert((kTileChunks + 1) / 4 % 2 == 0, "a tile is an even number of groups");
+#pragma unroll 1
+                for (int g = 0; g < (kTileChunks + 1) / 4; g += 2) {
+                    {
+                        const uint32_t p0 = pack16(r0), p1 = pack16(r1), p2 = pack16(r2), p3 = pack16(r3);
+                        asm volatile("" ::"v"(p0), "v"(p1), "v"(p2), "v"(p3) : "memory");
+                        load_group(r0, r1, r2, r3);
+                        scan_group(p0, p1, p2, p3, g);
+                        end_group(false);
+                        pk_prev = p3;
+                    }
+                    {
+                        const uint32_t p0 = pack16(r4), p1 = pack16(r5), p2 = pack16(r6), p3 = pack16(r7);
+                        asm volatile("" ::"v"(p0), "v"(p1), "v"(p2), "v"(p3) : "memory");
+                        if (pend_on) consume_probe();
+                        load_group(r4, r5, r6, r7);
+                        scan_group(p0, p1, p2, p3, g + 1);
+                        end_group(true);
+                        pk_prev = p3;
+                    }
+                }
             }
             if (++sc_run == run) {
                 sc_run = 0;
@@ -753,7 +787,12 @@
     while (q_count) drain_ring(q_count < 64 ? q_count : 64);
     if (hr.count) drain_hits<EMIT, FL>(P, hr, newest_end, lane, n_true);
     if constexpr (EMIT) flush_stage<!kWide>(P, hr, lane);
-    if (hr.flist && lane == 0) P.flag_counts[wave_id] = hr.nflag;
+    if (hr.flist && hr.nflag) {
+        __builtin_amdgcn_fence(__ATOMIC_RELEASE, "workgroup");
+        __builtin_amdgcn_fence(__ATOMIC_ACQUIRE, "workgroup");
+        const uint32_t n_listed = hr.nflag < P.flag_cap ? hr.nflag : P.flag_cap;
+        for (uint32_t i = lane; i < n_listed; i += 64) reinterpret_cast<uint8_t *>(P.rec_flags32)[hr.flist[i]] = 1;
+    }
     if ((MK_ABLATE & 1) != 0 && abl_acc == 0xFFFFFFFFu) n_cand++;
     if (P.counters) {
         __syncthreads();
diff --git a/merkurio_amd/csrc/scan_variants.hip b/merkurio_amd/csrc/scan_variants.hip
--- a/merkurio_amd/csrc/scan_variants.hip
+++ b/merkurio_amd/csrc/scan_variants.hip
@@ -1,28 +1,30 @@
 #include "scan_kernel_impl.hpp"
 
 #ifndef MK_TU
-#error "compile with -DMK_TU=0..16"
+#error "compile with -DMK_TU=0..18"
 #endif
 
 namespace mk {
 
-template <int S, int QC, bool EMIT, bool GF, int FL, int MC>
+template <int S, int QC, bool EMIT, bool GF, int FL, int MC, int DEPTH>
 void launch_variant(const ScanParams &p, int grid_blocks, hipStream_t stream) {
-    hipLaunchKernelGGL((mk_scan_kernel<S, QC, EMIT, GF, FL, MC>), dim3(grid_blocks), dim3(kBlockThreads), 0, stream, p);
+    hipLaunchKernelGGL((mk_scan_kernel<S, QC, EMIT, GF, FL, MC, DEPTH>), dim3(grid_blocks), dim3(kBlockThreads), 0, stream, p);
 }
 
 #define MK_INST(S_, QC_, GF_)                                                                    \
-    template void launch_variant<S_, QC_, false, GF_, 1, 0>(const ScanParams &, int, hipStream_t); \
-    template void launch_variant<S_, QC_, true, GF_, 1, 0>(const ScanParams &, int, hipStream_t)
+    template void launch_variant<S_, QC_, false, GF_, 1, 0, 1>(const ScanParams &, int, hipStream_t); \
+    template void launch_variant<S_, QC_, true, GF_, 1, 0, 1>(const ScanParams &, int, hipStream_t)
 #define MK_INST_MC(S_, QC_, MC_)                                                                       \
-    template void launch_variant<S_, QC_, false, false, 1, MC_>(const ScanParams &, int, hipStream_t); \
-    template void launch_variant<S_, QC_, true, false, 1, MC_>(const ScanParams &, int, hipStream_t)
+    template void launch_variant<S_, QC_, false, false, 1, MC_, 1>(const ScanParams &, int, hipStream_t); \
+    template void launch_variant<S_, QC_, true, false, 1, MC_, 1>(const ScanParams &, int, hipStream_t)
 #define MK_INST_MC_GF(S_, QC_)                                                                       \
-    template void launch_variant<S_, QC_, false, true, 1, 1>(const ScanParams &, int, hipStream_t); \
-    template void launch_variant<S_, QC_, true, true, 1, 1>(const ScanParams &, int, hipStream_t)
+    template void launch_variant<S_, QC_, false, true, 1, 1, 1>(const ScanParams &, int, hipStream_t); \
+    template void launch_variant<S_, QC_, true, true, 1, 1, 1>(const ScanParams &, int, hipStream_t)
 #define MK_INST_PLAIN(S_, QC_, GF_)                                                               \
-    template void launch_variant<S_, QC_, false, GF_, 0, 0>(const ScanParams &, int, hipStream_t); \
-    template void launch_variant<S_, QC_, true, GF_, 0, 0>(const ScanParams &, int, hipStream_t)
+    template void launch_variant<S_, QC_, false, GF_, 0, 0, 1>(const ScanParams &, int, hipStream_t); \
+    template void launch_variant<S_, QC_, true, GF_, 0, 0, 1>(const ScanParams &, int, hipStream_t)
+#define MK_INST_DEPTH2(S_, QC_, EMIT_, FL_) \
+    template void launch_variant<S_, QC_, EMIT_, false, FL_, 0, 2>(const ScanParams &, int, hipStream_t)
 
 #if MK_TU == 0
 uint32_t scan_lds_bytes() { return kLdsBytes; }
@@ -115,6 +117,20 @@
 MK_INST_MC_GF(4, -1);
 MK_INST_MC_GF(8, -1);
 MK_INST_MC_GF(16, -1);
+#elif MK_TU == 17
+MK_INST_DEPTH2(16, 16, false, 1);
+MK_INST_DEPTH2(8, 24, false, 1);
+MK_INST_DEPTH2(4, 28, false, 1);
+MK_INST_DEPTH2(4, 18, false, 1);
+MK_INST_DEPTH2(16, 16, true, 1);
+MK_INST_DEPTH2(8, 24, true, 1);
+MK_INST_DEPTH2(4, 28, true, 1);
+MK_INST_DEPTH2(4, 18, true, 1);
+#elif MK_TU == 18
+MK_INST_DEPTH2(16, 16, false, 0);
+MK_INST_DEPTH2(8, 24, false, 0);
+MK_INST_DEPTH2(4, 28, false, 0);
+MK_INST_DEPTH2(4, 18, false, 0);
 #else
 #error "unknown MK_TU"
 #endif
diff --git a/merkurio_amd/native.py b/merkurio_amd/native.py
--- a/merkurio_amd/native.py
+++ b/merkurio_amd/native.py
@@ -65,13 +65,14 @@
     _fields_ = [("struct_size", C.c_uint32), ("force_stride", C.c_uint32), ("force_global_filter", C.c_uint32),
                 ("gbloom_log2_blocks", C.c_uint32), ("tile_run", C.c_uint32), ("gbloom_kib", C.c_uint32),
                 ("length_classes", C.c_uint32), ("force_split_len", C.c_uint32), ("force_stride2", C.c_uint32),
-                ("force_q2", C.c_uint32)]
+                ("force_q2", C.c_uint32), ("force_depth", C.c_uint32)]
 
     def __init__(self, force_stride=0, force_global_filter=False, gbloom_log2_blocks=0, tile_run=0, gbloom_kib=0,
-                 length_classes=0, force_split_len=0, force_stride2=0, force_q2=0, force_single_class=False):
+                 length_classes=0, force_split_len=0, force_stride2=0, force_q2=0, force_single_class=False, force_depth=0):
         super().__init__(C.sizeof(MatcherOptions), int(force_stride), int(bool(force_global_filter)),
                          int(gbloom_log2_blocks), int(tile_run), int(gbloom_kib),
-                         1 if force_single_class else int(length_classes), int(force_split_len), int(force_stride2), int(force_q2))
+                         1 if force_single_class else int(length_classes), int(force_split_len), int(force_stride2), int(force_q2),
+                         int(force_depth))
 
 
 class WindowText(C.Structure):
```

New measurement: 6096. 0.977x the previous value.
